# kelseyicotton/rawaudiovae_kelsey

Measured on NVIDIA B200. Metric: train frames/sec (fwd+bwd+Adam), higher is better.
Workload: dtype bf16

## Files before the change

rawaudiovae_kelsey_b200/csrc/capi.cu:

```cuda
#include <cmath>
#include <cstdlib>
#include <dlfcn.h>
#include <cstring>
#include <map>
#include <new>
#include <utility>
#include <vector>

#include "../../include/rvae_b200.h"
#include "common.h"

namespace rvae {
const char* last_error();
}

using namespace rvae;

struct NcclId {
  char internal[128];
};
struct NcclApi {
  void* handle;
  int (*GetUniqueId)(NcclId*);
  int (*CommInitRank)(void** comm, int nranks, NcclId id, int rank);
// ... 243 lines not shown
}
int rvae_dp_status(rvae_ctx* ctx, unsigned int* status) {
  RVAE_REQUIRE(ctx && status, RVAE_ERR_INVALID, "dp_status: null argument");
  *status = 0;
  if (!ctx->p2p_ready) return RVAE_OK;
  RVAE_CUDA(cudaMemcpy(status, ctx->p2p.status, sizeof(unsigned int), cudaMemcpyDeviceToHost));
  return RVAE_OK;
}
int rvae_ctx_num_sms(const rvae_ctx* ctx) { return ctx ? ctx->c.num_sms : 0; }
uint64_t rvae_ctx_launch_count(const rvae_ctx* ctx) { return ctx ? ctx->c.launches : 0; }

#define CTX_OR_FAIL(ctx) RVAE_REQUIRE((ctx) != nullptr, RVAE_ERR_INVALID, "null rvae_ctx")

int rvae_debug_set_aux_trace(rvae_ctx* ctx, void* buf, int launches) {
  CTX_OR_FAIL(ctx);
  ctx->c.aux_trace = reinterpret_cast<unsigned long long*>(buf);
  ctx->c.aux_cap = buf ? launches : 0;
  ctx->c.aux_seq = 0;
  return RVAE_OK;
}

int rvae_debug_set_trace(rvae_ctx* ctx, void* buf, int launches) {
  CTX_OR_FAIL(ctx);
  RVAE_REQUIRE(launches >= 1, RVAE_ERR_INVALID, "debug_set_trace: launches=%d", launches);
  ctx->c.trace_launches = launches;
  ctx->c.trace_seq = 0;
  static_assert(RVAE_TRACE_WORDS_PER_CTA == kTraceCtaWords && RVAE_TRACE_HEADER_WORDS == kTraceHeader &&
                    RVAE_TRACE_TILES == kTraceTiles && RVAE_TRACE_EVENTS == kTraceEvents,
                "trace layout");
  ctx->c.trace = reinterpret_cast<unsigned long long*>(buf);
  return RVAE_OK;
}

int rvae_frame_gather(rvae_ctx* ctx, const void* audio, int audio_is_i16, int64_t n_samples,
                      const int64_t* frame_idx, int64_t first_frame, int64_t n_frames, int hop, int S, void* out_hi,
                      void* out_lo, float* out_f32, void* stream) {
  CTX_OR_FAIL(ctx);
  return launch_frame_gather(&ctx->c, audio, audio_is_i16, n_samples, frame_idx, first_frame, n_frames, hop, S, S,
                             BF(out_hi), BF(out_lo), out_f32, S_(stream));
}
int rvae_overlap_add(rvae_ctx* ctx, const float* frames, int64_t n_frames, int S, int hop, float* out, int64_t t_begin,
                     int64_t n_out, void* stream) {
  CTX_OR_FAIL(ctx);
  return launch_overlap_add(&ctx->c, frames, n_frames, S, hop, out, t_begin, n_out, S_(stream));
}
int rvae_randn(rvae_ctx* ctx, float* out, int64_t n, uint64_t seed, uint64_t offset, int64_t elem_base,
               void* stream) {
  CTX_OR_FAIL(ctx);
  RVAE_REQUIRE(elem_base >= 0, RVAE_ERR_INVALID, "randn: elem_base %lld", (long long)elem_base);
  if (elem_base % 4 != 0) return launch_randn_rows(&ctx->c, out, 1, n, n, seed, offset, nullptr, elem_base, S_(stream));
  return launch_randn(&ctx->c, out, n, seed, offset, nullptr, elem_base, S_(stream));
}
int rvae_lerp_reparameterize(rvae_ctx* ctx, const float* mu_a, const float* logvar_a, const float* mu_b,
                             const float* logvar_b, const void* alpha, int alpha_is_f64, const float* eps,
                             int64_t rows, int L, float* z, float* mu_out, float* logvar_out, void* stream) {
  CTX_OR_FAIL(ctx);
  return launch_lerp_reparam(&ctx->c, mu_a, logvar_a, mu_b, logvar_b, alpha, alpha_is_f64, eps, rows, L, L, z, nullptr,
                             nullptr, mu_out, logvar_out, S_(stream));
}
int rvae_split_bf16(rvae_ctx* ctx, const float* src, int64_t n, void* hi, void* lo, void* stream) {
  CTX_OR_FAIL(ctx);
  return launch_split_bf16(&ctx->c, src, n, BF(hi), BF(lo), S_(stream));
}
int rvae_reparameterize(rvae_ctx* ctx, const float* mu, const float* logvar, const float* eps, int64_t n, float* z,
                        void* stream) {
  CTX_OR_FAIL(ctx);
  return launch_reparam(&ctx->c, mu, logvar, eps, n, z, S_(stream));
}
int rvae_loss_fwd(rvae_ctx* ctx, const float* xhat, const float* x, const float* mu, const float* logvar, int64_t B,
                  int S, int L, float beta, double* acc, float* loss_out, void* stream) {
  CTX_OR_FAIL(ctx);
  return launch_loss_fwd(&ctx->c, xhat, x, mu, logvar, B, S, L, beta, acc, loss_out, S_(stream));
}
int rvae_frame_loss(rvae_ctx* ctx, const float* xhat, int ld_xhat, const float* mu, const float* logvar, int ld_lat,
                    int64_t rows, int S, int L, const void* audio, int audio_is_i16, int64_t n_samples,
                    int64_t first_frame, int hop, float* rec_out, float* kl_out, void* stream) {
  RVAE_REQUIRE(xhat && mu && logvar && audio && rec_out && kl_out, RVAE_ERR_INVALID, "frame_loss: null buffer");
  RVAE_REQUIRE(rows > 0 && S > 0 && L > 0, RVAE_ERR_INVALID, "frame_loss: rows %lld, S %d, L %d (need > 0)",
               (long long)rows, S, L);
  RVAE_REQUIRE(ld_xhat >= S && ld_lat >= L, RVAE_ERR_INVALID, "frame_loss: row pitch ld_xhat %d < S %d or ld_lat %d < L %d",
               ld_xhat, S, ld_lat, L);
  RVAE_REQUIRE(hop > 0 && n_samples >= 0 && first_frame >= 0, RVAE_ERR_INVALID,
               "frame_loss: hop %d, n_samples %lld, first_frame %lld (need hop > 0, n_samples >= 0, first_frame >= 0)",
               hop, (long long)n_samples, (long long)first_frame);
  CTX_OR_FAIL(ctx);
  return launch_frame_loss(&ctx->c, xhat, ld_xhat, mu, logvar, ld_lat, rows, S, L, audio, audio_is_i16, n_samples,
                           first_frame, hop, rec_out, kl_out, S_(stream));
}
int rvae_loss_bwd(rvae_ctx* ctx, const float* xhat, const float* x, const float* mu, const float* logvar, int64_t B,
                  int S, int L, float beta, const float* grad_out, float* g_xhat, float* g_mu, float* g_logvar,
                  void* stream) {
  CTX_OR_FAIL(ctx);
  return launch_loss_bwd(&ctx->c, xhat, x, mu, logvar, B, S, L, beta, grad_out, g_xhat, g_mu, g_logvar, S_(stream));
}
int rvae_tanh_bwd(rvae_ctx* ctx, const float* g_xhat, const float* xhat, int64_t n, void* da_hi, void* da_lo,
                  void* stream) {
  CTX_OR_FAIL(ctx);
  return launch_tanh_bwd(&ctx->c, g_xhat, xhat, n, BF(da_hi), BF(da_lo), S_(stream));
}
int rvae_colsum(rvae_ctx* ctx, const void* hi, const void* lo, int64_t M, int N, int ld, float* out, int accumulate,
                void* stream) {
  CTX_OR_FAIL(ctx);
  return launch_colsum(&ctx->c, BF(hi), BF(lo), M, N, ld, out, accumulate, S_(stream));
}
int rvae_step_inc(rvae_ctx* ctx, float* step, void* stream) {
  CTX_OR_FAIL(ctx);
  return launch_step_inc(&ctx->c, step, S_(stream));
}
int rvae_adam_step(rvae_ctx* ctx, float* p, const float* g, float* m, float* v, int64_t n, double lr, double beta1,
                   double beta2, double eps, double weight_decay, float grad_scale, const float* step, void* shadow_hi,
                   void* shadow_lo, void* stream) {
  CTX_OR_FAIL(ctx);
  return launch_adam(&ctx->c, p, const_cast<float*>(g), m, v, n, lr, beta1, beta2, eps, weight_decay, grad_scale, step,
                     BF(shadow_hi), BF(shadow_lo), 0, S_(stream));
}
size_t rvae_param_histogram_bytes(int n_segs, int n_edges) { return param_histogram_bytes(n_segs, n_edges); }
int rvae_param_histogram(rvae_ctx* ctx, const float* params, const int64_t* seg_offsets_host,
                         const int64_t* seg_lengths_host, int n_segs, const double* edges_host, int n_edges,
                         void* record, void* stream) {
  CTX_OR_FAIL(ctx);
  return launch_param_histogram(&ctx->c, params, seg_offsets_host, seg_lengths_host, n_segs, edges_host, n_edges,
                                record, S_(stream));
}
int rvae_param_histogram_rows(rvae_ctx* ctx, const float* params, const int64_t* seg_offsets_host,
                              const int64_t* seg_rows_host, const int64_t* seg_cols_host, const int64_t* seg_pitch_host,
                              int n_segs, const double* edges_host, int n_edges, void* record, void* stream) {
  CTX_OR_FAIL(ctx);
  return launch_param_histogram_rows(&ctx->c, params, seg_offsets_host, seg_rows_host, seg_cols_host, seg_pitch_host,
                                     n_segs, edges_host, n_edges, record, S_(stream));
}

static GemmDesc desc_base(int epi, int M, int N, int K) {
  GemmDesc d;
  memset(&d, 0, sizeof(d));
  d.epi = epi; d.M = M; d.N = N; d.K = K;
  return d;
}
static Operand op(const void* hi, const void* lo, int major, int ld) {
  Operand o;
  o.hi = BF(hi); o.lo = BF(lo); o.major = major; o.ld = ld; o.cols = 0;
  return o;
}

int rvae_linear_act_fwd(rvae_ctx* ctx, const void* x_hi, const void* x_lo, const void* w_hi, const void* w_lo,
                        const float* bias, int M, int N, int K, int act, void* y_hi, void* y_lo, float* y_f32,
                        void* stream) {
  CTX_OR_FAIL(ctx);
  RVAE_REQUIRE(y_hi || y_f32, RVAE_ERR_INVALID, "linear_act_fwd: no output buffer");
  GemmDesc d = desc_base(EPI_LINEAR, M, N, K);
  d.A = op(x_hi, x_lo, MAJOR_K, K);
  d.B = op(w_hi, w_lo, MAJOR_K, K);
  d.args.bias = bias; d.args.act = act; d.args.ldo = N;
  d.args.out_hi = BF(y_hi); d.args.out_lo = BF(y_lo); d.args.out_f32 = y_f32;
  return gemm_launch(&ctx->c, d, S_(stream));
}

int rvae_encode_head_fwd(rvae_ctx* ctx, const void* h_hi, const void* h_lo, const void* w2_hi, const void* w2_lo,
                         const float* b2, int M, int L, int K, const float* eps, float* mu, float* logvar, void* z_hi,
                         void* z_lo, double* kl_acc, void* stream) {
  CTX_OR_FAIL(ctx);
  RVAE_REQUIRE(b2 && mu && logvar, RVAE_ERR_INVALID, "encode_head_fwd: null buffer");
  GemmDesc d = desc_base(EPI_HEAD, M, 2 * L, K);
  d.head_L = L;
  d.A = op(h_hi, h_lo, MAJOR_K, K);
  d.B = op(w2_hi, w2_lo, MAJOR_K, K);
  d.args.bias = b2; d.args.in0 = eps; d.args.out_f32 = mu; d.args.out_f32_b = logvar;
  d.args.out_hi = BF(z_hi); d.args.out_lo = BF(z_lo);
  d.args.loss_acc = kl_acc; d.args.L = L; d.args.ldo = L;
  return gemm_launch(&ctx->c, d, S_(stream));
}

int rvae_out_tanh_mse_fwd(rvae_ctx* ctx, const void* h_hi, const void* h_lo, const void* w4_hi, const void* w4_lo,
                          const float* b4, int M, int S, int K, const void* x_hi, const void* x_lo, int tanh_approx,
                          float* xhat, void* da_hi, void* da_lo, float grad_scale, double* mse_acc, float* bias_grad,
                          void* stream) {
  CTX_OR_FAIL(ctx);
  RVAE_REQUIRE(b4 && x_hi, RVAE_ERR_INVALID, "out_tanh_mse_fwd: null buffer");
  GemmDesc d = desc_base(EPI_OUT, M, S, K);
  d.A = op(h_hi, h_lo, MAJOR_K, K);
  d.B = op(w4_hi, w4_lo, MAJOR_K, K);
  d.args.bias = b4; d.args.in0 = x_hi; d.args.in1 = x_lo; d.args.out_f32 = xhat;
  d.args.out_hi = BF(da_hi); d.args.out_lo = BF(da_lo);
  d.args.act = tanh_approx ? ACT_TANH_APPROX : ACT_TANH;
  d.args.c0 = grad_scale; d.args.loss_acc = mse_acc; d.args.ldo = S; d.args.colsum = bias_grad;
  return gemm_launch(&ctx->c, d, S_(stream));
}

int rvae_dgrad_relu(rvae_ctx* ctx, const void* dy_hi, const void* dy_lo, const void* w_hi, const void* w_lo, int M,
                    int N, int Kd, const void* mask, void* dx_hi, void* dx_lo, float* bias_grad, void* stream) {
  CTX_OR_FAIL(ctx);
  RVAE_REQUIRE(dx_hi, RVAE_ERR_INVALID, "dgrad_relu: null output");
  GemmDesc d = desc_base(EPI_DRELU, M, N, Kd);
  d.A = op(dy_hi, dy_lo, MAJOR_K, Kd);
  d.B = op(w_hi, w_lo, MAJOR_MN, N);
  d.args.in0 = mask; d.args.out_hi = BF(dx_hi); d.args.out_lo = BF(dx_lo); d.args.ldo = N;
  d.args.colsum = bias_grad;
  return gemm_launch(&ctx->c, d, S_(stream));
}

int rvae_dgrad_latent(rvae_ctx* ctx, const void* da3_hi, const void* da3_lo, const void* w3_hi, const void* w3_lo,
                      int M, int L, int H, const float* eps, const float* logvar, const float* mu,
                      const float* g_mu_ext, const float* g_logvar_ext, float kl_grad_scale, float* dz_scratch,
                      void* dml_hi, void* dml_lo, float* bias_grad, void* stream) {
  CTX_OR_FAIL(ctx);
  RVAE_REQUIRE(eps && logvar && dz_scratch && dml_hi, RVAE_ERR_INVALID, "dgrad_latent: null buffer");
  RVAE_CUDA(cudaMemsetAsync(dz_scratch, 0, sizeof(float) * (size_t)M * L, S_(stream)));
  GemmDesc d = desc_base(EPI_REDUCE, M, L, H);
  d.A = op(da3_hi, da3_lo, MAJOR_K, H);
  d.B = op(w3_hi, w3_lo, MAJOR_MN, L);
  d.args.out_f32 = dz_scratch; d.args.ldo = L; d.args.accumulate = 1;
  RVAE_CHECK(gemm_launch(&ctx->c, d, S_(stream)));
  return launch_latent_bwd(&ctx->c, dz_scratch, eps, logvar, mu, g_mu_ext, g_logvar_ext, kl_grad_value(kl_grad_scale), M, L,
                           BF(dml_hi), BF(dml_lo), bias_grad, 0, nullptr, S_(stream));
}

int rvae_wgrad(rvae_ctx* ctx, const void* dy_hi, const void* dy_lo, const void* x_hi, const void* x_lo, int B, int M,
               int N, float* dW, int accumulate, int k_splits, void* stream) {
  CTX_OR_FAIL(ctx);
  RVAE_REQUIRE(dW, RVAE_ERR_INVALID, "wgrad: null output");
  RVAE_REQUIRE(M % 64 == 0, RVAE_ERR_UNSUPPORTED, "wgrad: M=%d must be a multiple of 64", M);
  GemmDesc d = desc_base(EPI_REDUCE, M, N, B);
  d.A = op(dy_hi, dy_lo, MAJOR_MN, M);
  d.B = op(x_hi, x_lo, MAJOR_MN, N);
  d.args.out_f32 = dW; d.args.ldo = N; d.args.accumulate = accumulate;
  d.k_splits = accumulate ? k_splits : 1;
  return gemm_launch(&ctx->c, d, S_(stream));
}

int rvae_param_layout(int S, int H, int L, rvae_layout* out) {
  RVAE_REQUIRE(out, RVAE_ERR_INVALID, "param_layout: null out");
  RVAE_REQUIRE(S > 0 && H > 0 && L > 0 && S % 64 == 0 && H % 64 == 0 && L % 64 == 0, RVAE_ERR_UNSUPPORTED,
               "segment_length=%d, n_units=%d, latent_dim=%d must be positive multiples of 64", S, H, L);
  int64_t o = 0;
  out->w1 = o; o += (int64_t)H * S;
  out->w2 = o; o += (int64_t)2 * L * H;
  out->w3 = o; o += (int64_t)H * L;
  out->w4 = o; o += (int64_t)S * H;
  out->b1 = o; o += H;
  out->b2 = o; o += 2 * L;
  out->b3 = o; o += H;
  out->b4 = o; o += S;
  out->total = o;
  return RVAE_OK;
}

int rvae_param_layout_padded(int S, int H, int L, rvae_layout* out, int* Sp, int* Hp, int* Lp) {
  RVAE_REQUIRE(out && Sp && Hp && Lp, RVAE_ERR_INVALID, "param_layout_padded: null out");
  RVAE_REQUIRE(S > 0 && H > 0 && L > 0 && S <= (1 << 24) && H <= (1 << 24) && L <= (1 << 24), RVAE_ERR_UNSUPPORTED,
               "segment_length=%d, n_units=%d, latent_dim=%d must be in 1..%d", S, H, L, 1 << 24);
  const int sp = (S + 63) / 64 * 64, hp = (H + 63) / 64 * 64, lp = (L + 63) / 64 * 64;
  RVAE_CHECK(rvae_param_layout(sp, hp, lp, out));
  *Sp = sp; *Hp = hp; *Lp = lp;
  return RVAE_OK;
}

}

namespace {

struct Planes {
  __nv_bfloat16* hi = nullptr;
  __nv_bfloat16* lo = nullptr;
};

constexpr int kNormGroups = 4;
constexpr int kNormMaxBlocks = 1024;

enum GemmId { G_F1, G_F2, G_F3, G_F4_OUT, G_F4_LIN, G_B4W, G_B4D, G_B3W, G_B3D, G_B2W, G_B2D, G_B1W, G_COUNT };
enum AuxSlot { T_LOAD = G_COUNT, T_EPS, T_FINALIZE, T_COLSUM, T_ADAM, T_TANHBWD, T_LATENT, T_COUNT };

constexpr int G_B3D_LAT = G_COUNT;
constexpr int kGemmSlots = G_COUNT + 1;

struct GemmSet {
  PreparedGemm g[kGemmSlots];
  bool ready[kGemmSlots];
  PreparedChain dual[3];
  int dual_state[3];
  PreparedChain dual_lat;
  int dual_lat_state;
  PreparedChain tri;
  int tri_state;
  PreparedChain fwd;
  int fwd_state;
};

}

struct rvae_plan {
  rvae_ctx* ctx;
  int S, H, L, max_batch, precision;
  int s_true, h_true, l_true;
  rvae_layout lay;
  rvae_plan_buffers bufs;
  bool bound;
  size_t ws_bytes;
  Planes x, h1, z, h3, da4, da3, dml, da1;
  float *mu, *lv, *eps, *dz, *xhat;
  float *ext_gx, *ext_gmu, *ext_glv, *ext_lv;
  Planes x_alt;
  float* eps_alt;
  int cur;
  int x_pitch, x_pitch_alt;
  int* sched_dev;
  int sched_batch;
  unsigned int* dep_flags;
  bool fuse_forward;
  bool fuse_latent;
  int dual_pairs;
  unsigned int* ticket;
  bool ticket_zeroed;
  bool norm_ticket_zeroed;
  const double* clip_max;
  float* clip_norm_out;
  int clip_ring;
  double* norm_parts;
  float* clip_coef;
  struct Prefetch {
    bool registered;
    int ready_batch;
    const void* audio; int audio_is_i16; int64_t n_samples; const int64_t* frame_idx; int64_t first_frame;
    int count, hop; uint64_t seed, offset; int add_step;
    bool span;
    int64_t noise_row0;
  } pf;
  double* loss_acc;
  float *out_mu, *out_lv, *out_xhat;
  int batch;
  int64_t global_batch;
  int64_t noise_row0;
  bool dp_enabled;
  float kl_c0;
  double kl_bl;
  const rvae_hparams* hp_dev;
  int hp_early;
  bool dz_zeroed;
  bool grads_zeroed[5];
  bool streams_ready;
  cudaEvent_t ev_fork;
  bool two_streams;
  bool have_eps;
  cudaEvent_t ev_eps;
  bool eps_pending;
  cudaStream_t adam_stream;
  cudaEvent_t ev_adam_fork, ev_adam_join;
  cudaStream_t hp;
  cudaEvent_t ev_hp_fork, ev_hp_join;
  cudaStream_t hp2;
  cudaEvent_t ev_s1_fork, ev_s1_join;
  bool split_stage1;
  int s1_wgrad_ctas, s1_order;
  bool merge_b3w;
  bool allow_defer;
  bool b3w_deferred;
  int adam_bg_blocks;
  cudaStream_t comm_stream;
  cudaStream_t comm_stream2;
  cudaEvent_t ev_comm_fork, ev_comm_done[5];
  LossFinalize fin;
  bool fin_pending;
  std::map<int64_t, GemmSet> sets;
  bool timing;
  std::vector<std::pair<cudaEvent_t, cudaEvent_t>> ev_pool;
  std::vector<std::pair<int, int>> ev_used;
  double t_ms[T_COUNT];
  int64_t t_n[T_COUNT];
  double t_flops[T_COUNT];
};

namespace {

size_t align_up(size_t v, size_t a) { return (v + a - 1) / a * a; }

size_t carve(rvae_plan* p, uint8_t* base) {
  const size_t B = p->max_batch, S = p->S, H = p->H, L = p->L;
  const bool lo = p->precision == RVAE_PRECISION_FP32;
  size_t off = 0;
  auto take = [&](size_t bytes) -> uint8_t* {
    uint8_t* r = base ? base + off : nullptr;
    off += align_up(bytes, 256);
    return r;
  };
  auto planes = [&](Planes& pl, size_t elems) {
    pl.hi = reinterpret_cast<__nv_bfloat16*>(take(elems * 2));
    pl.lo = lo ? reinterpret_cast<__nv_bfloat16*>(take(elems * 2)) : nullptr;
  };
  planes(p->x, B * S);
  planes(p->x_alt, B * S);
  planes(p->h1, B * H);
  planes(p->z, B * L);
  planes(p->h3, B * H);
  planes(p->da4, B * S);
  planes(p->da3, B * H);
  planes(p->dml, B * 2 * L);
  planes(p->da1, B * H);
  p->mu = reinterpret_cast<float*>(take(B * L * 4));
  p->lv = reinterpret_cast<float*>(take(B * L * 4));
  p->eps = reinterpret_cast<float*>(take(B * L * 4));
  p->eps_alt = reinterpret_cast<float*>(take(B * L * 4));
  p->ticket = reinterpret_cast<unsigned int*>(take(256));
  p->sched_dev = reinterpret_cast<int*>(take(sizeof(int) * 2 * 6 * 128 * kSchedMax));
  p->dep_flags = reinterpret_cast<unsigned int*>(take(sizeof(unsigned int) * 3 * 256));
  p->norm_parts = reinterpret_cast<double*>(take(sizeof(double) * kNormGroups * kNormMaxBlocks));
  p->clip_coef = reinterpret_cast<float*>(take(sizeof(float)));
  p->dz = reinterpret_cast<float*>(take(B * L * 4));
  p->xhat = reinterpret_cast<float*>(take(B * S * 4));
  p->loss_acc = reinterpret_cast<double*>(take(2 * sizeof(double)));
  p->ext_gx = p->ext_gmu = p->ext_glv = p->ext_lv = nullptr;
  if (p->S != (size_t)p->s_true) p->ext_gx = reinterpret_cast<float*>(take(B * S * 4));
  if (p->L != (size_t)p->l_true) {
    p->ext_gmu = reinterpret_cast<float*>(take(B * L * 4));
    p->ext_glv = reinterpret_cast<float*>(take(B * L * 4));
    p->ext_lv = reinterpret_cast<float*>(take(B * L * 4));
  }
  return off;
}

Operand opnd(const Planes& pl, int major, int ld) {
  Operand o;
  o.hi = pl.hi; o.lo = pl.lo; o.major = major; o.ld = ld; o.cols = 0;
  return o;
}
Operand wopnd(const rvae_plan* p, int64_t off, int major, int ld) {
  Operand o;
  o.hi = BF(p->bufs.shadow_hi) + off;
  o.lo = p->bufs.shadow_lo ? BF(p->bufs.shadow_lo) + off : nullptr;
  o.major = major; o.ld = ld; o.cols = 0;
  return o;
}

int prepare(rvae_plan* p, GemmSet& gs, int id) {
  if (gs.ready[id]) return RVAE_OK;
  const int B = p->batch, S = p->S, H = p->H, L = p->L;
  const int ldx = p->x_pitch > 0 ? p->x_pitch : S;
  const rvae_layout& ly = p->lay;
  float* params = p->bufs.params;
  float* grads = p->bufs.grads;
  GemmDesc d;
  memset(&d, 0, sizeof(d));
  const bool bf16_mode = p->precision == RVAE_PRECISION_BF16;
  switch (id) {
    case G_F1:
      d.epi = EPI_LINEAR; d.M = B; d.N = H; d.K = S;
      d.A = opnd(p->x, MAJOR_K, ldx); d.B = wopnd(p, ly.w1, MAJOR_K, S);
      d.A.cols = p->s_true;
      d.args.bias = params + ly.b1; d.args.act = ACT_RELU; d.args.ldo = H;
      d.args.out_hi = p->h1.hi; d.args.out_lo = p->h1.lo;
      break;
    case G_F2:
      d.epi = EPI_HEAD; d.M = B; d.N = 2 * L; d.K = H; d.head_L = L;
      d.A = opnd(p->h1, MAJOR_K, H); d.B = wopnd(p, ly.w2, MAJOR_K, H);
      d.args.bias = params + ly.b2; d.args.in0 = p->eps; d.args.out_f32 = p->mu; d.args.out_f32_b = p->lv;
      d.args.out_hi = p->z.hi; d.args.out_lo = p->z.lo;
      d.args.loss_acc = p->loss_acc + 1; d.args.L = L; d.args.ldo = L;
      break;
    case G_F3:
      d.epi = EPI_LINEAR; d.M = B; d.N = H; d.K = L;
      d.A = opnd(p->z, MAJOR_K, L); d.B = wopnd(p, ly.w3, MAJOR_K, L);
      d.args.bias = params + ly.b3; d.args.act = ACT_RELU; d.args.ldo = H;
      d.args.out_hi = p->h3.hi; d.args.out_lo = p->h3.lo;
      break;
    case G_F4_OUT:
      d.epi = EPI_OUT; d.M = B; d.N = S; d.K = H;
      d.A = opnd(p->h3, MAJOR_K, H); d.B = wopnd(p, ly.w4, MAJOR_K, H);
      d.args.bias = params + ly.b4; d.args.in0 = p->x.hi; d.args.in1 = p->x.lo; d.args.out_f32 = p->xhat;
      d.args.out_hi = p->da4.hi; d.args.out_lo = p->da4.lo;
      d.args.act = bf16_mode ? ACT_TANH_APPROX : ACT_TANH;
      d.args.loss_acc = p->loss_acc; d.args.ldo = S; d.args.ldi = ldx; d.side_cols = p->s_true;
      d.args.colsum = grads ? grads + ly.b4 : nullptr;
      break;
    case G_F4_LIN:
      d.epi = EPI_LINEAR; d.M = B; d.N = S; d.K = H;
      d.A = opnd(p->h3, MAJOR_K, H); d.B = wopnd(p, ly.w4, MAJOR_K, H);
      d.args.bias = params + ly.b4; d.args.act = bf16_mode ? ACT_TANH_APPROX : ACT_TANH; d.args.ldo = S;
      d.args.out_f32 = p->xhat;
      break;
    case G_B4W:
      d.epi = EPI_REDUCE; d.M = S; d.N = H; d.K = B;
      d.A = opnd(p->da4, MAJOR_MN, S); d.B = opnd(p->h3, MAJOR_MN, H);
      d.args.out_f32 = grads + ly.w4; d.args.ldo = H; d.args.accumulate = 1;
      break;
    case G_B4D:
      d.epi = EPI_DRELU; d.M = B; d.N = H; d.K = S;
      d.A = opnd(p->da4, MAJOR_K, S); d.B = wopnd(p, ly.w4, MAJOR_MN, H);
      d.args.in0 = p->h3.hi; d.args.out_hi = p->da3.hi; d.args.out_lo = p->da3.lo; d.args.ldo = H;
      d.args.colsum = grads + ly.b3;
      break;
    case G_B3W:
      d.epi = EPI_REDUCE; d.M = H; d.N = L; d.K = B;
      d.A = opnd(p->da3, MAJOR_MN, H); d.B = opnd(p->z, MAJOR_MN, L);
      d.args.out_f32 = grads + ly.w3; d.args.ldo = L; d.args.accumulate = 1;
      break;
    case G_B3D:
      d.epi = EPI_REDUCE; d.M = B; d.N = L; d.K = H;
      d.A = opnd(p->da3, MAJOR_K, H); d.B = wopnd(p, ly.w3, MAJOR_MN, L);
      d.args.out_f32 = p->dz; d.args.ldo = L; d.args.accumulate = 1;
      break;
    case G_B3D_LAT:
      d.epi = EPI_DLATENT; d.M = B; d.N = L; d.K = H;
      d.A = opnd(p->da3, MAJOR_K, H); d.B = wopnd(p, ly.w3, MAJOR_MN, L);
      d.args.in0 = p->eps; d.args.in1 = p->lv; d.args.in2 = p->mu;
      d.args.out_hi = p->dml.hi; d.args.ldo = 2 * L; d.args.L = L;
      d.args.colsum = grads + ly.b2;
      break;
    case G_B2W:
      d.epi = EPI_REDUCE; d.M = 2 * L; d.N = H; d.K = B;
      d.A = opnd(p->dml, MAJOR_MN, 2 * L); d.B = opnd(p->h1, MAJOR_MN, H);
      d.args.out_f32 = grads + ly.w2; d.args.ldo = H; d.args.accumulate = 1;
      break;
    case G_B2D:
      d.epi = EPI_DRELU; d.M = B; d.N = H; d.K = 2 * L;
      d.A = opnd(p->dml, MAJOR_K, 2 * L); d.B = wopnd(p, ly.w2, MAJOR_MN, H);
      d.args.in0 = p->h1.hi; d.args.out_hi = p->da1.hi; d.args.out_lo = p->da1.lo; d.args.ldo = H;
      d.args.colsum = grads + ly.b1;
      break;
    case G_B1W:
      d.epi = EPI_REDUCE; d.M = H; d.N = S; d.K = B;
      d.A = opnd(p->da1, MAJOR_MN, H); d.B = opnd(p->x, MAJOR_MN, ldx); d.B.cols = p->s_true;
      d.args.out_f32 = grads + ly.w1; d.args.ldo = S; d.args.accumulate = 1;
      break;
    default:
      return set_error(RVAE_ERR_INVALID, "plan: bad gemm id %d", id);
  }
  RVAE_CHECK(gemm_prepare(&p->ctx->c, d, &gs.g[id]));
  gs.ready[id] = true;
  return RVAE_OK;
}

int get_set(rvae_plan* p, GemmSet** out) {
  const int64_t key = ((int64_t)p->batch * 2 + p->cur) * 65536 + p->x_pitch;
  auto it = p->sets.find(key);
  if (it == p->sets.end()) {
    GemmSet gs;
    memset(&gs, 0, sizeof(gs));
    it = p->sets.emplace(key, gs).first;
  }
  *out = &it->second;
  return RVAE_OK;
}

int run_untimed(rvae_plan* p, GemmSet* gs, int id, cudaStream_t st, const EpiArgs* override_args) {
  if (override_args) {
    PreparedGemm g = gs->g[id];
    EpiArgs a = *override_args;
    if (a.L == 0) a.L = g.params.epi.L;
    RVAE_CHECK(gemm_bind_outputs(&g, a, false));
    return gemm_run(&p->ctx->c, g, st);
  }
  return gemm_run(&p->ctx->c, gs->g[id], st);
}

struct TimedScope {
  rvae_plan* p; int slot; cudaStream_t st; int idx;
  TimedScope(rvae_plan* p_, int slot_, cudaStream_t st_) : p(p_), slot(slot_), st(st_), idx(-1) {
    if (!p->timing) return;
    const size_t k = p->ev_used.size();
    if (k >= p->ev_pool.size()) {
      cudaEvent_t a, b;
      if (cudaEventCreate(&a) != cudaSuccess || cudaEventCreate(&b) != cudaSuccess) return;
      p->ev_pool.emplace_back(a, b);
    }
    idx = (int)k;
    cudaEventRecord(p->ev_pool[k].first, st);
  }
  ~TimedScope() {
    if (idx < 0) return;
    cudaEventRecord(p->ev_pool[idx].second, st);
    p->ev_used.emplace_back(slot, idx);
  }
};

int run(rvae_plan* p, int id, cudaStream_t st, const EpiArgs* override_args = nullptr) {
  GemmSet* gs;
  RVAE_CHECK(get_set(p, &gs));
  RVAE_CHECK(prepare(p, *gs, id));
  if (!p->timing) return run_untimed(p, gs, id, st, override_args);
  const size_t slot = p->ev_used.size();
  if (slot >= p->ev_pool.size()) {
    cudaEvent_t a, b;
    RVAE_CUDA(cudaEventCreate(&a));
    RVAE_CUDA(cudaEventCreate(&b));
    p->ev_pool.emplace_back(a, b);
  }
  RVAE_CUDA(cudaEventRecord(p->ev_pool[slot].first, st));
  RVAE_CHECK(run_untimed(p, gs, id, st, override_args));
  RVAE_CUDA(cudaEventRecord(p->ev_pool[slot].second, st));
  const int tid = id == G_B3D_LAT ? G_B3D : id;
  p->ev_used.emplace_back(tid, (int)slot);
  const GemmParams& gp = gs->g[id].params;
  p->t_flops[tid] = 2.0 * gp.M * gp.N * gp.K;
  return RVAE_OK;
}

int pad_rows(float* dst, const float* src, int rows, int cols, int ld, cudaStream_t st) {
  RVAE_CUDA(cudaMemcpy2DAsync(dst, sizeof(float) * ld, src, sizeof(float) * cols, sizeof(float) * cols, rows,
                              cudaMemcpyDeviceToDevice, st));
  RVAE_CUDA(cudaMemset2DAsync(dst + cols, sizeof(float) * ld, 0, sizeof(float) * (ld - cols), rows, st));
  return RVAE_OK;
}
int strip_rows(float* dst, const float* src, int rows, int cols, int ld, cudaStream_t st) {
  RVAE_CUDA(cudaMemcpy2DAsync(dst, sizeof(float) * cols, src, sizeof(float) * ld, sizeof(float) * cols, rows,
                              cudaMemcpyDeviceToDevice, st));
  return RVAE_OK;
}
int copy_latents_out(rvae_plan* p, cudaStream_t st) {
  if (p->out_mu) RVAE_CHECK(strip_rows(p->out_mu, p->mu, p->batch, p->l_true, p->L, st));
  if (p->out_lv) RVAE_CHECK(strip_rows(p->out_lv, p->lv, p->batch, p->l_true, p->L, st));
  return RVAE_OK;
}

int draw_eps(rvae_plan* p, float* out, int rows, uint64_t seed, uint64_t offset, const float* offset_src, int64_t row0,
             cudaStream_t st) {
  if (p->l_true == p->L)
    return launch_randn(&p->ctx->c, out, (int64_t)rows * p->L, seed, offset, offset_src, row0 * p->L, st);
  return launch_randn_rows(&p->ctx->c, out, rows, p->l_true, p->L, seed, offset, offset_src, row0 * p->l_true, st);
}

int decode_tail(rvae_plan* p, float* xhat_out, cudaStream_t st) {
  RVAE_CHECK(run(p, G_F3, st));
  GemmSet* gs;
  RVAE_CHECK(get_set(p, &gs));
  RVAE_CHECK(prepare(p, *gs, G_F4_LIN));
  EpiArgs a = gs->g[G_F4_LIN].params.epi;
  const bool rec_direct = p->S == p->s_true;
  a.out_f32 = rec_direct ? xhat_out : p->xhat;
  RVAE_CHECK(run(p, G_F4_LIN, st, &a));
  return rec_direct ? RVAE_OK : strip_rows(xhat_out, p->xhat, p->batch, p->s_true, p->S, st);
}

int check_ready(const rvae_plan* p, bool need_batch) {
  RVAE_REQUIRE(p != nullptr, RVAE_ERR_INVALID, "null rvae_plan");
  RVAE_REQUIRE(p->bound, RVAE_ERR_STATE, "plan: rvae_plan_bind has not been called");
  if (need_batch) RVAE_REQUIRE(p->batch > 0, RVAE_ERR_STATE, "plan: no batch loaded");
  return RVAE_OK;
}

int ensure_bias_zeroed(rvae_plan* p, cudaStream_t st) {
  if (p->grads_zeroed[4]) return RVAE_OK;
  const rvae_layout& ly = p->lay;
  RVAE_CUDA(cudaMemsetAsync(p->bufs.grads + ly.b1, 0, sizeof(float) * (size_t)(ly.total - ly.b1), st));
  p->grads_zeroed[4] = true;
  return RVAE_OK;
}

int ensure_side_stream(rvae_plan* p) {
  if (p->streams_ready) return RVAE_OK;
  int least = 0, greatest = 0;
  RVAE_CUDA(cudaDeviceGetStreamPriorityRange(&least, &greatest));
  RVAE_CUDA(cudaStreamCreateWithPriority(&p->hp, cudaStreamNonBlocking, greatest));
  RVAE_CUDA(cudaStreamCreateWithPriority(&p->adam_stream, cudaStreamNonBlocking, least));
  RVAE_CUDA(cudaStreamCreateWithPriority(&p->hp2, cudaStreamNonBlocking, greatest));
  RVAE_CUDA(cudaEventCreateWithFlags(&p->ev_s1_fork, cudaEventDisableTiming));
  RVAE_CUDA(cudaEventCreateWithFlags(&p->ev_s1_join, cudaEventDisableTiming));
  RVAE_CUDA(cudaEventCreateWithFlags(&p->ev_hp_fork, cudaEventDisableTiming));
  RVAE_CUDA(cudaEventCreateWithFlags(&p->ev_hp_join, cudaEventDisableTiming));
  RVAE_CUDA(cudaStreamCreateWithPriority(&p->comm_stream, cudaStreamNonBlocking, greatest));
  RVAE_CUDA(cudaStreamCreateWithPriority(&p->comm_stream2, cudaStreamNonBlocking, greatest));
  RVAE_CUDA(cudaEventCreateWithFlags(&p->ev_comm_fork, cudaEventDisableTiming));
  for (int i = 0; i < 5; ++i) RVAE_CUDA(cudaEventCreateWithFlags(&p->ev_comm_done[i], cudaEventDisableTiming));
  RVAE_CUDA(cudaEventCreateWithFlags(&p->ev_fork, cudaEventDisableTiming));
  RVAE_CUDA(cudaEventCreateWithFlags(&p->ev_eps, cudaEventDisableTiming));
  RVAE_CUDA(cudaEventCreateWithFlags(&p->ev_adam_fork, cudaEventDisableTiming));
  RVAE_CUDA(cudaEventCreateWithFlags(&p->ev_adam_join, cudaEventDisableTiming));
  p->streams_ready = true;
  return RVAE_OK;
}

int adam_buckets(rvae_plan* p, unsigned mask, const HpArg& hp, float grad_scale, int zero_grads, int step_bias,
                 bool advance_step, cudaStream_t st, const float* coef = nullptr) {
  const rvae_layout& ly = p->lay;
  const rvae_plan_buffers& b = p->bufs;
  const int order[5] = {3, 2, 1, 0, 4};
  const int64_t begin[6] = {ly.w1, ly.w2, ly.w3, ly.w4, ly.b1, ly.total};
  int64_t seg_off[5], seg_n[5];
  int nseg = 0;
  for (int i = 0; i < 5; ++i) {
    if (!(mask & (1u << order[i]))) continue;
    if (nseg > 0 && seg_off[nseg - 1] + seg_n[nseg - 1] == begin[i]) seg_n[nseg - 1] += begin[i + 1] - begin[i];
    else { seg_off[nseg] = begin[i]; seg_n[nseg] = begin[i + 1] - begin[i]; ++nseg; }
  }
  if (advance_step && !p->ticket_zeroed) {
    RVAE_CUDA(cudaMemsetAsync(p->ticket, 0, sizeof(unsigned int), st));
    p->ticket_zeroed = true;
  }
  for (int i = 0; i < nseg; i += 2) {
    const int64_t o = seg_off[i];
    const bool pair = i + 1 < nseg;
    const bool last = i + 2 >= nseg;
    RVAE_CHECK(launch_adam2(&p->ctx->c, b.params + o, b.grads + o, b.exp_avg + o, b.exp_avg_sq + o, seg_n[i],
                            pair ? seg_off[i + 1] - o : 0, pair ? seg_n[i + 1] : 0, hp, grad_scale, coef, b.step, step_bias, (advance_step && last) ? p->ticket : nullptr,
                            BF(b.shadow_hi) + o, b.shadow_lo ? BF(b.shadow_lo) + o : nullptr, zero_grads, st));
  }
  for (int s = 0; s < 5; ++s)
    if (mask & (1u << s)) p->grads_zeroed[s] = zero_grads != 0;
  return RVAE_OK;
}

int grad_norm_group(rvae_plan* p, int k, NormFinalize* fin, cudaStream_t st) {
  const rvae_layout& ly = p->lay;
  const int64_t off[kNormGroups][2] = {{ly.w4, 0}, {ly.w3, 0}, {ly.w2, ly.b1}, {ly.w1, 0}};
  const int64_t len[kNormGroups][2] = {{ly.b1 - ly.w4, 0}, {ly.w4 - ly.w3, 0}, {ly.w3 - ly.w2, ly.total - ly.b1},
                                       {ly.w2 - ly.w1, 0}};
  int base[kNormGroups + 1] = {0};
  for (int j = 0; j < kNormGroups; ++j) base[j + 1] = base[j] + grad_norm_blocks(&p->ctx->c, len[j][0] + len[j][1]);
  RVAE_REQUIRE(base[kNormGroups] <= kNormGroups * kNormMaxBlocks, RVAE_ERR_UNSUPPORTED, "grad_norm: %d blocks",
               base[kNormGroups]);
  if (fin != nullptr) {
    if (!p->norm_ticket_zeroed) {
      RVAE_CUDA(cudaMemsetAsync(p->ticket + 1, 0, sizeof(unsigned int), st));
      p->norm_ticket_zeroed = true;
    }
    fin->parts = p->norm_parts;
    fin->n_parts = base[kNormGroups];
    fin->ticket = p->ticket + 1;
  }
  NormFinalize none;
  memset(&none, 0, sizeof(none));
  return launch_grad_norm(&p->ctx->c, p->bufs.grads + off[k][0], len[k][0], off[k][1] - off[k][0], len[k][1],
                          p->norm_parts + base[k], fin ? *fin : none, st);
}

NormFinalize clip_finalize(rvae_plan* p) {
  NormFinalize f;
  memset(&f, 0, sizeof(f));
  f.step = p->bufs.step;
  f.norm_out = p->clip_norm_out;
  f.ring_size = p->clip_ring;
  f.max_norm = p->clip_max;
  f.coef_out = p->clip_coef;
  return f;
}

struct LatentExt {
  const float* g_mu;
  const float* g_lv;
  const float* lv;
};

KlGrad plan_kl(const rvae_plan* p) { return KlGrad{p->hp_dev, p->bufs.step, p->kl_bl, p->kl_c0, p->hp_early}; }

bool sched_usable(const rvae_plan* p) { return p->sched_batch == 0 || p->sched_batch == p->batch; }

bool latent_fused(const rvae_plan* p) {
  return p->fuse_latent && p->precision == RVAE_PRECISION_BF16 && p->batch > kBlockM;
}

int backward_stage_latent_fused(rvae_plan* p, cudaStream_t st) {
  GemmSet* gs;
  RVAE_CHECK(get_set(p, &gs));
  if (p->fin_pending) {
    RVAE_CHECK(launch_loss_finalize_prepared(&p->ctx->c, p->fin, st));
    p->fin_pending = false;
  }
  if (p->dual_pairs > 0 && !p->timing && sched_usable(p)) {
    int pairs = p->dual_pairs > 64 ? 64 : p->dual_pairs;
    if (const char* e = getenv("RVAE_DUAL_PAIRS_S1")) {
      const int v = atoi(e);
      if (v >= 1 && 2 * v <= p->ctx->c.num_sms_total) pairs = v;
    }
    if (gs->dual_lat_state == 0) {
      RVAE_CHECK(prepare(p, *gs, G_B3D_LAT));
      RVAE_CHECK(prepare(p, *gs, G_B3W));
      int* sched = p->sched_dev + ((size_t)p->cur * 6 + 4) * 128 * kSchedMax;
      const PreparedGemm* both[2] = {&gs->g[G_B3D_LAT], &gs->g[G_B3W]};
      const int rc = gemm_prepare_chain(&p->ctx->c, both, 2, pairs, sched, &gs->dual_lat);
      gs->dual_lat_state = rc == RVAE_OK ? 1 : -1;
      if (rc != RVAE_OK && rc != RVAE_ERR_UNSUPPORTED) return rc;
      if (rc == RVAE_OK) p->sched_batch = p->batch;
    }
    if (gs->dual_lat_state == 1) {
      PreparedChain d = gs->dual_lat;
      d.params.p[0].epi.c0 = p->kl_c0;
      return gemm_run_chain(&p->ctx->c, d, st);
    }
  }
  RVAE_CHECK(prepare(p, *gs, G_B3D_LAT));
  EpiArgs a = gs->g[G_B3D_LAT].params.epi;
  a.c0 = p->kl_c0;
  RVAE_CHECK(run(p, G_B3D_LAT, st, &a));
  return run(p, G_B3W, st);
}

int backward_stage(rvae_plan* p, int stage, const LatentExt* ext, cudaStream_t st) {
  const int S = p->S, H = p->H, L = p->L;
  const rvae_layout& ly = p->lay;
  float* grads = p->bufs.grads;
  static const int kWgrad[4] = {G_B4W, G_B3W, G_B2W, G_B1W};
  static const int kDgrad[4] = {G_B4D, G_B3D, G_B2D, -1};
  RVAE_REQUIRE(stage >= 0 && stage < 4, RVAE_ERR_INVALID, "plan_backward: stage %d not in -1..3", stage);
  float* wptr[4] = {grads + ly.w4, grads + ly.w3, grads + ly.w2, grads + ly.w1};
  const size_t wcount[4] = {(size_t)S * H, (size_t)H * L, (size_t)2 * L * H, (size_t)H * S};
  if (!p->grads_zeroed[stage]) RVAE_CUDA(cudaMemsetAsync(wptr[stage], 0, sizeof(float) * wcount[stage], st));
  p->grads_zeroed[stage] = false;
  if (stage == 1 && ext == nullptr && latent_fused(p)) return backward_stage_latent_fused(p, st);
  if (stage == 1 && !p->dz_zeroed)
    RVAE_CUDA(cudaMemsetAsync(p->dz, 0, sizeof(float) * (size_t)p->max_batch * L, st));
  auto stage_pairs = [&](int st_idx) {
    int pairs = (p->dp_enabled && p->ctx->dp_world > 1 && p->dual_pairs > 64) ? 64 : p->dual_pairs;
    const char* names[3] = {"RVAE_DUAL_PAIRS_S0", "RVAE_DUAL_PAIRS_S1", "RVAE_DUAL_PAIRS_S2"};
    if (const char* e = getenv(names[st_idx])) {
      const int v = atoi(e);
      if (v >= 1 && 2 * v <= p->ctx->c.num_sms_total) pairs = v;
    }
    return pairs;
  };
  if (stage == 1 && p->allow_defer && p->merge_b3w && p->dual_pairs > 0 && sched_usable(p) && p->batch > kBlockM) {
    GemmSet* gs;
    RVAE_CHECK(get_set(p, &gs));
    if (gs->tri_state == 0) {
      RVAE_CHECK(prepare(p, *gs, G_B2D));
      RVAE_CHECK(prepare(p, *gs, G_B2W));
      RVAE_CHECK(prepare(p, *gs, G_B3W));
      int* sched = p->sched_dev + ((size_t)p->cur * 6 + 5) * 128 * kSchedMax;
      const PreparedGemm* three[3] = {&gs->g[G_B2D], &gs->g[G_B2W], &gs->g[G_B3W]};
      const int rc = gemm_prepare_chain(&p->ctx->c, three, 3, stage_pairs(2), sched, &gs->tri);
      gs->tri_state = rc == RVAE_OK ? 1 : -1;
      if (rc != RVAE_OK && rc != RVAE_ERR_UNSUPPORTED) return rc;
      if (rc == RVAE_OK) p->sched_batch = p->batch;
    }
    if (gs->tri_state == 1) {
      RVAE_CHECK(run(p, G_B3D, st));
      {
        TimedScope ts(p, T_LATENT, st);
        RVAE_CHECK(launch_latent_bwd(&p->ctx->c, p->dz, p->eps, ext ? ext->lv : p->lv, p->mu, ext ? ext->g_mu : nullptr,
                                     ext ? ext->g_lv : nullptr, plan_kl(p), p->batch, L, p->dml.hi, p->dml.lo, grads + ly.b2,
                                     1, p->fin_pending ? &p->fin : nullptr, st));
      }
      p->fin_pending = false;
      p->dz_zeroed = true;
      p->b3w_deferred = true;
      return RVAE_OK;
    }
  }
  if (stage == 2 && p->b3w_deferred) {
    GemmSet* gs;
    RVAE_CHECK(get_set(p, &gs));
    RVAE_REQUIRE(gs->tri_state == 1, RVAE_ERR_STATE, "plan_backward: stage 1 deferred the fc3 weight gradient but the "
                 "three-problem launch is not prepared (batch or input set changed between the stages)");
    p->b3w_deferred = false;
    TimedScope ts(p, G_B2D, st);
    if (p->timing) {
      double f = 0.0;
      for (int id : {G_B2D, G_B2W, G_B3W}) { const GemmParams& q = gs->g[id].params; f += 2.0 * q.M * q.N * q.K; }
      p->t_flops[G_B2D] = f;
    }
    return gemm_run_chain(&p->ctx->c, gs->tri, st);
  }
  if (stage == 1 && p->split_stage1 && p->timing && p->batch > kBlockM) {
    GemmSet* gs;
    RVAE_CHECK(get_set(p, &gs));
    RVAE_CHECK(run(p, G_B3D, st));
    RVAE_CHECK(prepare(p, *gs, G_B3W));
    {
      TimedScope ts(p, G_B3W, st);
      PreparedGemm w = gs->g[G_B3W];
      p->t_flops[G_B3W] = 2.0 * w.params.M * w.params.N * w.params.K;
      if (w.grid > p->s1_wgrad_ctas) w.grid = p->s1_wgrad_ctas;
      RVAE_CHECK(gemm_run(&p->ctx->c, w, st));
    }
    TimedScope ts(p, T_LATENT, st);
    RVAE_CHECK(launch_latent_bwd(&p->ctx->c, p->dz, p->eps, ext ? ext->lv : p->lv, p->mu, ext ? ext->g_mu : nullptr,
                                 ext ? ext->g_lv : nullptr, plan_kl(p), p->batch, L, p->dml.hi, p->dml.lo, grads + ly.b2, 1,
                                 p->fin_pending ? &p->fin : nullptr, st));
    p->fin_pending = false;
    p->dz_zeroed = true;
    return RVAE_OK;
  }
  if (stage == 1 && p->split_stage1 && p->two_streams && !p->timing && p->batch > kBlockM) {
    RVAE_CHECK(ensure_side_stream(p));
    GemmSet* gs;
    RVAE_CHECK(get_set(p, &gs));
    RVAE_CHECK(prepare(p, *gs, G_B3D));
    RVAE_CHECK(prepare(p, *gs, G_B3W));
    RVAE_CHECK(gemm_run(&p->ctx->c, gs->g[G_B3D], st));
    RVAE_CUDA(cudaEventRecord(p->ev_s1_fork, st));
    RVAE_CUDA(cudaStreamWaitEvent(p->hp2, p->ev_s1_fork, 0));
    cudaStream_t s_w = p->s1_order == 0 ? st : p->hp2;
    cudaStream_t s_l = p->s1_order == 0 ? p->hp2 : st;
    auto run_wgrad = [&]() -> int {
      PreparedGemm w = gs->g[G_B3W];
      const int cap = (p->dp_enabled && p->ctx->dp_world > 1 && p->s1_wgrad_ctas > 64) ? 64 : p->s1_wgrad_ctas;
      if (w.grid > cap) w.grid = cap;
      return gemm_run(&p->ctx->c, w, s_w);
    };
    auto run_latent = [&]() -> int {
      return launch_latent_bwd(&p->ctx->c, p->dz, p->eps, ext ? ext->lv : p->lv, p->mu, ext ? ext->g_mu : nullptr,
                               ext ? ext->g_lv : nullptr, plan_kl(p), p->batch, L, p->dml.hi, p->dml.lo, grads + ly.b2, 1,
                               p->fin_pending ? &p->fin : nullptr, s_l);
    };
    if (p->s1_order == 0) { RVAE_CHECK(run_wgrad()); RVAE_CHECK(run_latent()); }
    else { RVAE_CHECK(run_latent()); RVAE_CHECK(run_wgrad()); }
    RVAE_CUDA(cudaEventRecord(p->ev_s1_join, p->hp2));
    p->fin_pending = false;
    p->dz_zeroed = true;
    RVAE_CUDA(cudaStreamWaitEvent(st, p->ev_s1_join, 0));
    return RVAE_OK;
  }
  bool fused = false;
  if (kDgrad[stage] >= 0 && p->dual_pairs > 0 && sched_usable(p)) {
    int pairs = stage_pairs(stage);
    if (stage == 1 && pairs > 64 && !getenv("RVAE_DUAL_PAIRS_S1")) pairs = 64;
    GemmSet* gs;
    RVAE_CHECK(get_set(p, &gs));
    if (gs->dual_state[stage] == 0) {
      RVAE_CHECK(prepare(p, *gs, kDgrad[stage]));
      RVAE_CHECK(prepare(p, *gs, kWgrad[stage]));
      int* sched = p->sched_dev + ((size_t)p->cur * 6 + stage) * 128 * kSchedMax;
      const PreparedGemm* both[2] = {&gs->g[kDgrad[stage]], &gs->g[kWgrad[stage]]};
      const int rc = gemm_prepare_chain(&p->ctx->c, both, 2, pairs, sched, &gs->dual[stage]);
      gs->dual_state[stage] = rc == RVAE_OK ? 1 : -1;
      if (rc != RVAE_OK && rc != RVAE_ERR_UNSUPPORTED) return rc;
      if (rc == RVAE_OK) p->sched_batch = p->batch;
    }
    if (gs->dual_state[stage] == 1) {
      TimedScope ts(p, kDgrad[stage], st);
      if (p->timing) {
        const GemmParams& a = gs->g[kDgrad[stage]].params;
        const GemmParams& b = gs->g[kWgrad[stage]].params;
        p->t_flops[kDgrad[stage]] = 2.0 * a.M * a.N * a.K + 2.0 * b.M * b.N * b.K;
      }
      RVAE_CHECK(gemm_run_chain(&p->ctx->c, gs->dual[stage], st));
      fused = true;
    }
  }
  if (!fused && kDgrad[stage] >= 0) RVAE_CHECK(run(p, kDgrad[stage], st));
  if (stage == 1) {
    TimedScope ts(p, T_LATENT, st);
    RVAE_CHECK(launch_latent_bwd(&p->ctx->c, p->dz, p->eps, ext ? ext->lv : p->lv, p->mu, ext ? ext->g_mu : nullptr,
                                 ext ? ext->g_lv : nullptr, plan_kl(p), p->batch, L, p->dml.hi, p->dml.lo, grads + ly.b2, 1,
                                 p->fin_pending ? &p->fin : nullptr, st));
    p->fin_pending = false;
    p->dz_zeroed = true;
  }
  return fused ? RVAE_OK : run(p, kWgrad[stage], st);
}

}

extern "C" {

int rvae_plan_create(rvae_ctx* ctx, int S, int H, int L, int max_batch, int precision, rvae_plan** out) {
  CTX_OR_FAIL(ctx);
  RVAE_REQUIRE(out, RVAE_ERR_INVALID, "plan_create: null out");
  RVAE_REQUIRE(max_batch > 0, RVAE_ERR_INVALID, "plan_create: max_batch=%d", max_batch);
  RVAE_REQUIRE(precision == RVAE_PRECISION_BF16 || precision == RVAE_PRECISION_FP32, RVAE_ERR_INVALID,
               "plan_create: precision %d", precision);
  rvae_layout lay;
  int Sp, Hp, Lp;
  RVAE_CHECK(rvae_param_layout_padded(S, H, L, &lay, &Sp, &Hp, &Lp));
  rvae_plan* p = new (std::nothrow) rvae_plan();
  RVAE_REQUIRE(p, RVAE_ERR_INVALID, "plan_create: out of host memory");
  p->ctx = ctx; p->S = Sp; p->H = Hp; p->L = Lp; p->max_batch = max_batch; p->precision = precision;
  p->s_true = S; p->h_true = H; p->l_true = L;
  p->lay = lay; p->bound = false; p->batch = 0; p->have_eps = false; p->global_batch = 0; p->noise_row0 = 0;
  p->timing = false;
  p->kl_c0 = 0.f; p->kl_bl = 0.0; p->hp_dev = nullptr; p->hp_early = 0; p->dz_zeroed = false; p->dp_enabled = false;
  p->cur = 0; p->ticket_zeroed = false; p->ticket = nullptr; p->norm_ticket_zeroed = false;
  p->clip_max = nullptr; p->clip_norm_out = nullptr; p->clip_ring = 1;
  p->x_pitch = 0; p->x_pitch_alt = 0;
  p->fuse_latent = false;
  p->sched_batch = 0;
  memset(&p->pf, 0, sizeof(p->pf));
  for (int i = 0; i < 5; ++i) p->grads_zeroed[i] = false;
  p->streams_ready = false; p->ev_fork = nullptr;
  p->hp = nullptr; p->ev_hp_fork = nullptr; p->ev_hp_join = nullptr;
  p->comm_stream = nullptr; p->comm_stream2 = nullptr; p->ev_comm_fork = nullptr;
  for (int i = 0; i < 5; ++i) p->ev_comm_done[i] = nullptr;
  p->adam_stream = nullptr; p->ev_eps = nullptr; p->ev_adam_fork = nullptr; p->ev_adam_join = nullptr;
  p->eps_pending = false; p->fin_pending = false;
  p->two_streams = true;
  p->hp2 = nullptr; p->ev_s1_fork = nullptr; p->ev_s1_join = nullptr;
  p->split_stage1 = true;
  p->s1_wgrad_ctas = 96;
  p->s1_order = 0;
  p->merge_b3w = false; p->allow_defer = false; p->b3w_deferred = false;
#if RVAE_EXPERIMENTS
  if (const char* e = getenv("RVAE_MERGE_B3W")) p->merge_b3w = atoi(e) != 0;
#endif
  p->adam_bg_blocks = 0;
  if (const char* e = getenv("RVAE_ADAM_BG_BLOCKS")) p->adam_bg_blocks = atoi(e) > 0 ? atoi(e) : 0;
  if (const char* e = getenv("RVAE_S1_ORDER")) p->s1_order = atoi(e) != 0;
  if (const char* e = getenv("RVAE_SPLIT_STAGE1")) p->split_stage1 = atoi(e) != 0;
  if (const char* e = getenv("RVAE_S1_WGRAD_CTAS")) {
    const int v = atoi(e);
    if (v >= 2 && v <= ctx->c.num_sms_total) p->s1_wgrad_ctas = v & ~1;
  }
  p->fuse_forward = false;
#if RVAE_EXPERIMENTS
  if (const char* e = getenv("RVAE_FUSE_LATENT")) p->fuse_latent = atoi(e) != 0;
  if (const char* e = getenv("RVAE_FUSE_FORWARD")) p->fuse_forward = atoi(e) != 0;
#endif
  p->dual_pairs = ctx->c.num_sms / 2;
  if (const char* e = getenv("RVAE_DUAL_PAIRS")) {
    const int v = atoi(e);
    if (v >= 0 && 2 * v <= ctx->c.num_sms_total) p->dual_pairs = v;
  }
  if (const char* e = getenv("RVAE_TWO_STREAMS")) p->two_streams = atoi(e) != 0;
  for (int i = 0; i < T_COUNT; ++i) { p->t_ms[i] = 0; p->t_n[i] = 0; p->t_flops[i] = 0; }
  p->out_mu = p->out_lv = p->out_xhat = nullptr;
  memset(&p->bufs, 0, sizeof(p->bufs));
  p->ws_bytes = carve(p, nullptr);
  *out = p;
  return RVAE_OK;
}

void rvae_plan_destroy(rvae_plan* plan) {
  if (!plan) return;
  for (auto& e : plan->ev_pool) {
    cudaEventDestroy(e.first);
    cudaEventDestroy(e.second);
  }
  if (plan->streams_ready) {
    cudaStreamSynchronize(plan->adam_stream);
    cudaStreamSynchronize(plan->hp);
    cudaStreamSynchronize(plan->comm_stream);
    cudaStreamSynchronize(plan->comm_stream2);
    cudaStreamDestroy(plan->comm_stream2);
    cudaEventDestroy(plan->ev_comm_fork);
    for (int i = 0; i < 5; ++i) cudaEventDestroy(plan->ev_comm_done[i]);
    cudaStreamDestroy(plan->comm_stream);
    cudaEventDestroy(plan->ev_hp_fork);
    cudaEventDestroy(plan->ev_hp_join);
    cudaStreamDestroy(plan->hp);
    cudaStreamSynchronize(plan->hp2);
    cudaStreamDestroy(plan->hp2);
    cudaEventDestroy(plan->ev_s1_fork);
    cudaEventDestroy(plan->ev_s1_join);
    cudaEventDestroy(plan->ev_fork);
    cudaEventDestroy(plan->ev_eps);
    cudaEventDestroy(plan->ev_adam_fork);
    cudaEventDestroy(plan->ev_adam_join);
    cudaStreamDestroy(plan->adam_stream);
  }
  delete plan;
}

int rvae_plan_enable_timing(rvae_plan* plan, int enable) {
  RVAE_REQUIRE(plan, RVAE_ERR_INVALID, "null rvae_plan");
  plan->timing = enable != 0;
  return RVAE_OK;
}

int rvae_plan_read_timing(rvae_plan* plan, float* ms, int64_t* launches, double* flops_per_launch) {
  RVAE_REQUIRE(plan && ms && launches && flops_per_launch, RVAE_ERR_INVALID, "plan_read_timing: null argument");
  static_assert(G_COUNT == RVAE_NUM_GEMM_SLOTS && T_COUNT == RVAE_NUM_TIMING_SLOTS, "slot count");
  for (auto& u : plan->ev_used) {
    auto& e = plan->ev_pool[u.second];
    RVAE_CUDA(cudaEventSynchronize(e.second));
    float t = 0.f;
    RVAE_CUDA(cudaEventElapsedTime(&t, e.first, e.second));
    plan->t_ms[u.first] += t;
    plan->t_n[u.first] += 1;
  }
  plan->ev_used.clear();
  for (int i = 0; i < T_COUNT; ++i) {
    ms[i] = (float)plan->t_ms[i];
    launches[i] = plan->t_n[i];
    flops_per_launch[i] = plan->t_flops[i];
    plan->t_ms[i] = 0; plan->t_n[i] = 0;
  }
  return RVAE_OK;
}

size_t rvae_plan_workspace_bytes(const rvae_plan* plan) { return plan ? plan->ws_bytes : 0; }

int rvae_plan_bind(rvae_plan* plan, const rvae_plan_buffers* b) {
  RVAE_REQUIRE(plan && b, RVAE_ERR_INVALID, "plan_bind: null argument");
  RVAE_REQUIRE(b->params && b->shadow_hi && b->workspace, RVAE_ERR_INVALID,
               "plan_bind: params, shadow_hi and workspace are required");
  RVAE_REQUIRE(plan->precision == RVAE_PRECISION_BF16 || b->shadow_lo, RVAE_ERR_INVALID,
               "plan_bind: fp32 mode needs shadow_lo");
  RVAE_REQUIRE((reinterpret_cast<uintptr_t>(b->workspace) & 255) == 0, RVAE_ERR_INVALID,
               "plan_bind: workspace must be 256-byte aligned");
  plan->bufs = *b;
  if (plan->precision == RVAE_PRECISION_BF16) plan->bufs.shadow_lo = nullptr;
  carve(plan, reinterpret_cast<uint8_t*>(b->workspace));
  plan->sets.clear();
  plan->sched_batch = 0;
  for (int i = 0; i < 5; ++i) plan->grads_zeroed[i] = false;
  plan->dz_zeroed = false;
  plan->cur = 0; plan->ticket_zeroed = false; plan->norm_ticket_zeroed = false;
  memset(&plan->pf, 0, sizeof(plan->pf));
  if (plan->two_streams) RVAE_CHECK(ensure_side_stream(plan));
  plan->bound = true;
  plan->batch = 0;
  return RVAE_OK;
}

int rvae_plan_sync_shadow(rvae_plan* plan, void* stream) {
  RVAE_CHECK(check_ready(plan, false));
  return launch_split_bf16(&plan->ctx->c, plan->bufs.params, plan->lay.total, BF(plan->bufs.shadow_hi),
                           BF(plan->bufs.shadow_lo), S_(stream));
}

int rvae_plan_load_frames(rvae_plan* plan, const void* audio, int audio_is_i16, int64_t n_samples,
                          const int64_t* frame_idx, int64_t first_frame, int count, int hop, int row_offset,
                          void* stream) {
  RVAE_CHECK(check_ready(plan, false));
  RVAE_REQUIRE(count > 0 && row_offset >= 0 && row_offset + count <= plan->max_batch, RVAE_ERR_INVALID,
               "plan_load_frames: rows %d..%d outside 0..%d", row_offset, row_offset + count, plan->max_batch);
  RVAE_REQUIRE(row_offset == 0 || row_offset == plan->batch, RVAE_ERR_STATE,
               "plan_load_frames: row_offset %d does not continue the loaded batch (%d rows)", row_offset,
               plan->batch);
  RVAE_REQUIRE(row_offset == 0 || plan->x_pitch == 0, RVAE_ERR_STATE,
               "plan_load_frames: cannot append rows to a batch that was loaded as a sample span");
  plan->batch = row_offset + count;
  plan->x_pitch = 0;
  plan->have_eps = false;
  const size_t off = (size_t)row_offset * plan->S;
  TimedScope ts(plan, T_LOAD, S_(stream));
  return launch_frame_gather(&plan->ctx->c, audio, audio_is_i16, n_samples, frame_idx, first_frame, count, hop,
                             plan->s_true, plan->S, plan->x.hi + off, plan->x.lo ? plan->x.lo + off : nullptr, nullptr,
                             S_(stream));
}

int rvae_plan_load_batch(rvae_plan* plan, const float* x, int batch, void* stream) {
  RVAE_CHECK(check_ready(plan, false));
  RVAE_REQUIRE(x, RVAE_ERR_INVALID, "plan_load_batch: null x");
  RVAE_REQUIRE(batch > 0 && batch <= plan->max_batch, RVAE_ERR_INVALID, "plan_load_batch: batch %d not in 1..%d",
               batch, plan->max_batch);
  plan->batch = batch;
  plan->x_pitch = 0;
  plan->have_eps = false;
  TimedScope ts(plan, T_LOAD, S_(stream));
  if (plan->s_true != plan->S)
    return launch_split_bf16_rows(&plan->ctx->c, x, batch, plan->s_true, plan->s_true, plan->S, plan->x.hi, plan->x.lo,
                                  S_(stream));
  return launch_split_bf16(&plan->ctx->c, x, (int64_t)batch * plan->S, plan->x.hi, plan->x.lo, S_(stream));
}

static int span_eligible(const rvae_plan* p, int count, int hop) {
  const int S = p->s_true;
  return hop > 0 && hop % 8 == 0 && hop <= S && S % 8 == 0 && count > 0 && count <= p->max_batch &&
         (S == p->S || p->precision == RVAE_PRECISION_BF16);
}
static int convert_span(rvae_plan* p, const void* audio, int audio_is_i16, int64_t n_samples,
                        const int64_t* first_frame_dev, int64_t first_frame, int count, int hop, Planes& dst,
                        cudaStream_t st) {
  const int64_t span = (int64_t)(count - 1) * hop + p->s_true;
  RVAE_REQUIRE(span <= (int64_t)INT32_MAX, RVAE_ERR_UNSUPPORTED, "plan span: %lld samples", (long long)span);
  return launch_frame_gather(&p->ctx->c, audio, audio_is_i16, n_samples, first_frame_dev, first_frame, 1, hop,
                             (int)span, (int)span, dst.hi, dst.lo, nullptr, st);
}

int rvae_plan_span_supported(const rvae_plan* plan, int count, int hop) {
  return plan ? span_eligible(plan, count, hop) : 0;
}

int rvae_plan_load_span(rvae_plan* plan, const void* audio, int audio_is_i16, int64_t n_samples,
                        const int64_t* first_frame_dev, int64_t first_frame, int count, int hop, void* stream) {
  RVAE_CHECK(check_ready(plan, false));
  RVAE_REQUIRE(audio && span_eligible(plan, count, hop), RVAE_ERR_UNSUPPORTED,
               "plan_load_span: count %d (max %d), hop %d (needs hop %% 8 == 0 and hop <= S = %d; S %% 8 == 0; bf16 "
               "mode if S %% 64 != 0)", count, plan->max_batch, hop, plan->s_true);
  RVAE_REQUIRE(first_frame_dev || first_frame >= 0, RVAE_ERR_INVALID, "plan_load_span: first_frame %lld",
               (long long)first_frame);
  plan->batch = count;
  plan->x_pitch = hop;
  plan->have_eps = false;
  TimedScope ts(plan, T_LOAD, S_(stream));
  return convert_span(plan, audio, audio_is_i16, n_samples, first_frame_dev, first_frame, count, hop, plan->x,
                      S_(stream));
}

int rvae_plan_set_eps(rvae_plan* plan, const float* eps, void* stream) {
  RVAE_CHECK(check_ready(plan, true));
  RVAE_REQUIRE(eps, RVAE_ERR_INVALID, "plan_set_eps: null eps");
  if (plan->l_true != plan->L)
    RVAE_CHECK(pad_rows(plan->eps, eps, plan->batch, plan->l_true, plan->L, S_(stream)));
  else
    RVAE_CUDA(cudaMemcpyAsync(plan->eps, eps, sizeof(float) * (size_t)plan->batch * plan->L, cudaMemcpyDeviceToDevice,
                              S_(stream)));
  plan->have_eps = true;
  return RVAE_OK;
}

int rvae_plan_gen_eps(rvae_plan* plan, uint64_t seed, uint64_t offset, int add_step, void* stream) {
  RVAE_CHECK(check_ready(plan, true));
  RVAE_REQUIRE(!add_step || plan->bufs.step, RVAE_ERR_STATE, "plan_gen_eps(add_step): no step counter bound");
  plan->have_eps = true;
  cudaStream_t st = S_(stream);
  if (plan->two_streams && !plan->timing) {
    RVAE_CHECK(ensure_side_stream(plan));
    RVAE_CUDA(cudaEventRecord(plan->ev_fork, st));
    RVAE_CUDA(cudaStreamWaitEvent(plan->adam_stream, plan->ev_fork, 0));
    RVAE_CHECK(draw_eps(plan, plan->eps, plan->batch, seed, offset, add_step ? plan->bufs.step : nullptr,
                        plan->noise_row0, plan->adam_stream));
    RVAE_CUDA(cudaEventRecord(plan->ev_eps, plan->adam_stream));
    plan->eps_pending = true;
    return RVAE_OK;
  }
  TimedScope ts(plan, T_EPS, st);
  return draw_eps(plan, plan->eps, plan->batch, seed, offset, add_step ? plan->bufs.step : nullptr, plan->noise_row0,
                  st);
}

int rvae_plan_set_outputs(rvae_plan* plan, float* mu, float* logvar, float* xhat) {
  RVAE_REQUIRE(plan, RVAE_ERR_INVALID, "null rvae_plan");
  plan->out_mu = mu; plan->out_lv = logvar; plan->out_xhat = xhat;
  return RVAE_OK;
}

int rvae_plan_enable_dp(rvae_plan* plan, int on) {
  RVAE_REQUIRE(plan, RVAE_ERR_INVALID, "null rvae_plan");
  RVAE_REQUIRE(!on || plan->ctx->comm != nullptr || plan->ctx->p2p_ready, RVAE_ERR_STATE,
               "plan_enable_dp: call rvae_dp_init / rvae_dp_sym_open first");
  if (plan->dp_enabled != (on != 0) && !plan->sets.empty()) {
    RVAE_CUDA(cudaDeviceSynchronize());
    plan->sets.clear();
    plan->sched_batch = 0;
  }
  plan->dp_enabled = on != 0;
  return RVAE_OK;
}

int rvae_plan_set_noise_rows(rvae_plan* plan, int64_t first_global_row) {
  RVAE_REQUIRE(plan && first_global_row >= 0, RVAE_ERR_INVALID, "plan_set_noise_rows: bad argument");
  plan->noise_row0 = first_global_row;
  return RVAE_OK;
}

int rvae_plan_set_global_batch(rvae_plan* plan, int64_t global_batch) {
  RVAE_REQUIRE(plan && global_batch >= 0, RVAE_ERR_INVALID, "plan_set_global_batch: bad argument");
  plan->global_batch = global_batch;
  return RVAE_OK;
}

int rvae_plan_forward(rvae_plan* plan, float kl_beta, int fused_loss, int want_xhat, void* stream) {
  RVAE_CHECK(check_ready(plan, true));
  RVAE_REQUIRE(plan->have_eps, RVAE_ERR_STATE, "plan_forward: call rvae_plan_set_eps / rvae_plan_gen_eps first");
  cudaStream_t st = S_(stream);
  rvae_plan* p = plan;
  const double nb = p->global_batch > 0 ? (double)p->global_batch : (double)p->batch;
  const double BL = nb * p->l_true, BS = nb * p->s_true;
  const bool lat_direct = p->L == p->l_true, rec_direct = p->S == p->s_true;
  GemmSet* gs;
  RVAE_CHECK(get_set(p, &gs));

  const bool chain = fused_loss && !want_xhat && p->fuse_forward && p->dual_pairs > 0 && !p->timing && sched_usable(p) && !p->out_mu &&
                     !p->out_lv && !p->out_xhat && p->bufs.grads != nullptr;
  if (chain) {
    if (gs->fwd_state == 0) {
      static const int kLayers[4] = {G_F1, G_F2, G_F3, G_F4_OUT};
      const PreparedGemm* layers[4];
      for (int k = 0; k < 4; ++k) {
        RVAE_CHECK(prepare(p, *gs, kLayers[k]));
        layers[k] = &gs->g[kLayers[k]];
      }
      int* sched = p->sched_dev + ((size_t)p->cur * 6 + 3) * 128 * kSchedMax;
      int fpairs = p->dual_pairs;
      if (const char* e = getenv("RVAE_DUAL_PAIRS_F")) {
        const int v = atoi(e);
        if (v >= 1 && 2 * v <= p->ctx->c.num_sms_total) fpairs = v;
      }
      const int rc = gemm_prepare_chain(&p->ctx->c, layers, 4, fpairs, sched, &gs->fwd, p->dep_flags);
      gs->fwd_state = rc == RVAE_OK ? 1 : -1;
      if (rc != RVAE_OK && rc != RVAE_ERR_UNSUPPORTED) return rc;
      if (rc == RVAE_OK) p->sched_batch = p->batch;
    }
    if (gs->fwd_state == 1) {
      p->kl_c0 = (float)((double)kl_beta / BL);
      p->kl_bl = BL;
      RVAE_CHECK(ensure_bias_zeroed(p, st));
      p->grads_zeroed[4] = false;
      RVAE_CUDA(cudaMemsetAsync(p->dep_flags, 0, sizeof(unsigned int) * 3 * 256, st));
      if (p->eps_pending) {
        RVAE_CUDA(cudaStreamWaitEvent(st, p->ev_eps, 0));
        p->eps_pending = false;
      }
      PreparedChain d = gs->fwd;
      d.params.p[3].epi.c0 = (float)(2.0 / BS);
      d.params.p[3].epi.out_f32 = nullptr;
      return gemm_run_chain(&p->ctx->c, d, st);
    }
  }
  RVAE_CHECK(run(p, G_F1, st));
  if (p->eps_pending) {
    RVAE_CUDA(cudaStreamWaitEvent(st, p->ev_eps, 0));
    p->eps_pending = false;
  }
  {
    RVAE_CHECK(prepare(p, *gs, G_F2));
    EpiArgs a = gs->g[G_F2].params.epi;
    if (p->out_mu && lat_direct) a.out_f32 = p->out_mu;
    if (p->out_lv && lat_direct) a.out_f32_b = p->out_lv;
    if (fused_loss) { p->kl_c0 = (float)((double)kl_beta / BL); p->kl_bl = BL; }
    else a.loss_acc = nullptr;
    RVAE_CHECK(run(p, G_F2, st, &a));
    if (!lat_direct) RVAE_CHECK(copy_latents_out(p, st));
  }
  RVAE_CHECK(run(p, G_F3, st));
  if (fused_loss) {
    RVAE_REQUIRE(p->bufs.grads, RVAE_ERR_STATE, "plan_forward(fused_loss): no grads buffer bound");
    RVAE_REQUIRE(!p->out_mu && !p->out_lv, RVAE_ERR_STATE,
                 "plan_forward(fused_loss): mu / logvar must stay in the workspace (the fused backward reads them)");
    RVAE_CHECK(ensure_bias_zeroed(p, st));
    p->grads_zeroed[4] = false;
    RVAE_CHECK(prepare(p, *gs, G_F4_OUT));
    EpiArgs a = gs->g[G_F4_OUT].params.epi;
    a.c0 = (float)(2.0 / BS);
    a.out_f32 = want_xhat ? (p->out_xhat && rec_direct ? p->out_xhat : p->xhat) : nullptr;
    RVAE_CHECK(run(p, G_F4_OUT, st, &a));
    if (want_xhat && p->out_xhat && !rec_direct) RVAE_CHECK(strip_rows(p->out_xhat, p->xhat, p->batch, p->s_true, p->S, st));
  } else {
    RVAE_CHECK(prepare(p, *gs, G_F4_LIN));
    EpiArgs a = gs->g[G_F4_LIN].params.epi;
    a.out_f32 = p->out_xhat && rec_direct ? p->out_xhat : p->xhat;
    RVAE_CHECK(run(p, G_F4_LIN, st, &a));
    if (p->out_xhat && !rec_direct) RVAE_CHECK(strip_rows(p->out_xhat, p->xhat, p->batch, p->s_true, p->S, st));
  }
  return RVAE_OK;
}

int rvae_plan_backward(rvae_plan* plan, int stage, void* stream) {
  RVAE_CHECK(check_ready(plan, true));
  RVAE_REQUIRE(plan->bufs.grads, RVAE_ERR_STATE, "plan_backward: no grads buffer bound");
  if (stage == -1) {
    plan->allow_defer = true;
    int rc = RVAE_OK;
    for (int s = 0; s < 4 && rc == RVAE_OK; ++s) rc = backward_stage(plan, s, nullptr, S_(stream));
    plan->allow_defer = false;
    return rc;
  }
  return backward_stage(plan, stage, nullptr, S_(stream));
}

int rvae_plan_backward_external(rvae_plan* plan, const float* g_xhat, const float* xhat, const float* g_mu,
                                const float* g_logvar, const float* logvar, void* stream) {
  RVAE_CHECK(check_ready(plan, true));
  RVAE_REQUIRE(plan->bufs.grads, RVAE_ERR_STATE, "plan_backward_external: no grads buffer bound");
  RVAE_REQUIRE(g_xhat && xhat && g_mu && g_logvar && logvar, RVAE_ERR_INVALID,
               "plan_backward_external: null argument");
  rvae_plan* p = plan;
  cudaStream_t st = S_(stream);
  if (p->S != p->s_true) {
    RVAE_CHECK(pad_rows(p->ext_gx, g_xhat, p->batch, p->s_true, p->S, st));
    RVAE_CHECK(pad_rows(p->xhat, xhat, p->batch, p->s_true, p->S, st));
    g_xhat = p->ext_gx;
    xhat = p->xhat;
  }
  if (p->L != p->l_true) {
    RVAE_CHECK(pad_rows(p->ext_gmu, g_mu, p->batch, p->l_true, p->L, st));
    RVAE_CHECK(pad_rows(p->ext_glv, g_logvar, p->batch, p->l_true, p->L, st));
    RVAE_CHECK(pad_rows(p->ext_lv, logvar, p->batch, p->l_true, p->L, st));
    g_mu = p->ext_gmu;
    g_logvar = p->ext_glv;
    logvar = p->ext_lv;
  }
  RVAE_CHECK(ensure_bias_zeroed(p, st));
  p->grads_zeroed[4] = false;
  { TimedScope ts(p, T_TANHBWD, st); RVAE_CHECK(launch_tanh_bwd(&p->ctx->c, g_xhat, xhat, (int64_t)p->batch * p->S, p->da4.hi, p->da4.lo, st)); }
  { TimedScope ts(p, T_COLSUM, st);
    RVAE_CHECK(launch_colsum(&p->ctx->c, p->da4.hi, p->da4.lo, p->batch, p->S, p->S, p->bufs.grads + p->lay.b4, 1, st)); }
  const LatentExt ext = {g_mu, g_logvar, logvar};
  p->allow_defer = true;
  int rc = RVAE_OK;
  for (int s = 0; s < 4 && rc == RVAE_OK; ++s) rc = backward_stage(p, s, &ext, st);
  p->allow_defer = false;
  return rc;
}

int rvae_plan_finish_loss(rvae_plan* plan, float kl_beta, float* loss_out, int ring_size, void* stream) {
  RVAE_CHECK(check_ready(plan, true));
  RVAE_REQUIRE(ring_size >= 1, RVAE_ERR_INVALID, "plan_finish_loss: ring_size %d", ring_size);
  TimedScope ts(plan, T_FINALIZE, S_(stream));
  return launch_loss_finalize(&plan->ctx->c, plan->loss_acc, plan->batch, plan->s_true, plan->l_true, kl_beta, loss_out,
                              ring_size, plan->bufs.step, S_(stream));
}

int rvae_plan_finish_loss_deferred(rvae_plan* plan, float kl_beta, float* loss_out, int ring_size) {
  RVAE_CHECK(check_ready(plan, true));
  RVAE_REQUIRE(ring_size >= 1, RVAE_ERR_INVALID, "plan_finish_loss_deferred: ring_size %d", ring_size);
  plan->fin = make_loss_finalize(plan->loss_acc, plan->batch, plan->s_true, plan->l_true, kl_beta, loss_out, ring_size,
                                 plan->bufs.step);
  plan->fin_pending = true;
  return RVAE_OK;
}

int rvae_plan_prefetch_frames(rvae_plan* plan, const void* audio, int audio_is_i16, int64_t n_samples,
                              const int64_t* frame_idx, int64_t first_frame, int count, int hop, uint64_t seed,
                              uint64_t offset, int add_step) {
  RVAE_CHECK(check_ready(plan, false));
  RVAE_REQUIRE(audio && count > 0 && count <= plan->max_batch && hop > 0, RVAE_ERR_INVALID,
               "plan_prefetch_frames: bad arguments (count %d of max %d)", count, plan->max_batch);
  rvae_plan::Prefetch& f = plan->pf;
  f.audio = audio; f.audio_is_i16 = audio_is_i16; f.n_samples = n_samples; f.frame_idx = frame_idx;
  f.first_frame = first_frame; f.count = count; f.hop = hop; f.seed = seed; f.offset = offset; f.add_step = add_step;
  f.noise_row0 = plan->noise_row0;
  f.span = false;
  f.registered = true;
  return RVAE_OK;
}

int rvae_plan_prefetch_span(rvae_plan* plan, const void* audio, int audio_is_i16, int64_t n_samples,
                            const int64_t* first_frame_dev, int64_t first_frame, int count, int hop, uint64_t seed,
                            uint64_t offset, int add_step) {
  RVAE_CHECK(check_ready(plan, false));
  RVAE_REQUIRE(audio && span_eligible(plan, count, hop), RVAE_ERR_UNSUPPORTED,
               "plan_prefetch_span: count %d (max %d), hop %d (needs hop %% 8 == 0 and hop <= S = %d; S %% 8 == 0; "
               "bf16 mode if S %% 64 != 0)", count, plan->max_batch, hop, plan->s_true);
  RVAE_REQUIRE(first_frame_dev || first_frame >= 0, RVAE_ERR_INVALID, "plan_prefetch_span: first_frame %lld",
               (long long)first_frame);
  RVAE_CHECK(rvae_plan_prefetch_frames(plan, audio, audio_is_i16, n_samples, first_frame_dev, first_frame, count, hop,
                                       seed, offset, add_step));
  plan->pf.span = true;
  return RVAE_OK;
}

int rvae_plan_swap_prefetched(rvae_plan* plan) {
  RVAE_CHECK(check_ready(plan, false));
  RVAE_REQUIRE(plan->pf.ready_batch > 0, RVAE_ERR_STATE, "plan_swap_prefetched: no prefetched batch");
  std::swap(plan->x, plan->x_alt);
  std::swap(plan->x_pitch, plan->x_pitch_alt);
  std::swap(plan->eps, plan->eps_alt);
  plan->cur ^= 1;
  plan->batch = plan->pf.ready_batch;
  plan->pf.ready_batch = 0;
  plan->have_eps = true;
  plan->eps_pending = false;
  return RVAE_OK;
}

int rvae_plan_prefetched_batch(const rvae_plan* plan) { return plan ? plan->pf.ready_batch : 0; }

int rvae_plan_join_background(rvae_plan* plan, void* stream) {
  RVAE_CHECK(check_ready(plan, false));
  if (plan->eps_pending) {
    RVAE_CUDA(cudaStreamWaitEvent(S_(stream), plan->ev_eps, 0));
    plan->eps_pending = false;
  }
  return RVAE_OK;
}

int rvae_plan_note_prefetched(rvae_plan* plan, int count, int span_hop) {
  RVAE_CHECK(check_ready(plan, false));
  RVAE_REQUIRE(count > 0 && count <= plan->max_batch && span_hop >= 0, RVAE_ERR_INVALID,
               "plan_note_prefetched: count %d span_hop %d", count, span_hop);
  plan->pf.ready_batch = count;
  plan->x_pitch_alt = span_hop;
  return RVAE_OK;
}

int rvae_plan_adam(rvae_plan* plan, double lr, double beta1, double beta2, double eps, double weight_decay,
                   float grad_scale, int zero_grads, void* stream) {
  return rvae_plan_adam_buckets(plan, 0x1f, lr, beta1, beta2, eps, weight_decay, grad_scale, zero_grads, stream);
}

int rvae_plan_adam_buckets(rvae_plan* plan, unsigned bucket_mask, double lr, double beta1, double beta2, double eps,
                           double weight_decay, float grad_scale, int zero_grads, void* stream) {
  RVAE_CHECK(check_ready(plan, false));
  const rvae_plan_buffers& b = plan->bufs;
  RVAE_REQUIRE(b.grads && b.exp_avg && b.exp_avg_sq && b.step, RVAE_ERR_STATE,
               "plan_adam: grads / exp_avg / exp_avg_sq / step not bound");
  RVAE_REQUIRE(bucket_mask != 0 && bucket_mask <= 0x1f, RVAE_ERR_INVALID, "plan_adam_buckets: mask %#x", bucket_mask);
  TimedScope ts(plan, T_ADAM, S_(stream));
  return adam_buckets(plan, bucket_mask, hp_value(lr, beta1, beta2, eps, weight_decay), grad_scale, zero_grads, 0,
                      false, S_(stream));
}

static int train_step(rvae_plan* plan, float kl_beta, const HpArg& hp, int zero_grads, float* loss_out, int ring_size,
               void* stream) {
  RVAE_CHECK(check_ready(plan, true));
  const rvae_plan_buffers& b = plan->bufs;
  RVAE_REQUIRE(b.grads && b.exp_avg && b.exp_avg_sq && b.step, RVAE_ERR_STATE,
               "plan_train_step: grads / exp_avg / exp_avg_sq / step not bound");
  rvae_plan* p = plan;
  const bool fork = plan->two_streams && !plan->timing;
  const bool clip = plan->clip_max != nullptr;
  plan->hp_early = fork && plan->hp_dev != nullptr;
  if (!fork) {
    RVAE_CHECK(rvae_plan_forward(plan, kl_beta, 1, 0, stream));
    RVAE_CHECK(rvae_plan_finish_loss_deferred(plan, kl_beta, loss_out, ring_size));
    plan->fin.inc_step = 0;
    plan->fin.hp = hp.dev;
    RVAE_CHECK(rvae_plan_backward(plan, -1, stream));
    TimedScope ts(plan, T_ADAM, S_(stream));
    if (clip) {
      NormFinalize fin = clip_finalize(plan);
      for (int k = 0; k < kNormGroups; ++k)
        RVAE_CHECK(grad_norm_group(plan, k, k == kNormGroups - 1 ? &fin : nullptr, S_(stream)));
    }
    return adam_buckets(plan, 0x1f, hp, 1.0f, zero_grads, 1, true, S_(stream), clip ? plan->clip_coef : nullptr);
  }
  RVAE_CHECK(ensure_side_stream(plan));
  cudaStream_t st = plan->hp, bg = plan->adam_stream;
  RVAE_CUDA(cudaEventRecord(plan->ev_hp_fork, S_(stream)));
  RVAE_CUDA(cudaStreamWaitEvent(st, plan->ev_hp_fork, 0));
  auto enqueue_prefetch = [&]() -> int {
    if (!p->pf.registered) return RVAE_OK;
    const rvae_plan::Prefetch& f = p->pf;
    RVAE_CUDA(cudaStreamWaitEvent(bg, plan->ev_hp_fork, 0));
    if (f.span) {
      RVAE_CHECK(convert_span(p, f.audio, f.audio_is_i16, f.n_samples, f.frame_idx, f.first_frame, f.count, f.hop,
                              p->x_alt, bg));
      p->x_pitch_alt = f.hop;
    } else {
      RVAE_CHECK(launch_frame_gather(&p->ctx->c, f.audio, f.audio_is_i16, f.n_samples, f.frame_idx, f.first_frame,
                                     f.count, f.hop, p->s_true, p->S, p->x_alt.hi, p->x_alt.lo, nullptr, bg));
      p->x_pitch_alt = 0;
    }
    RVAE_CHECK(draw_eps(p, p->eps_alt, f.count, f.seed, f.offset + (f.add_step ? 1 : 0), f.add_step ? b.step : nullptr,
                        f.noise_row0, bg));
    p->pf.ready_batch = f.count;
    p->pf.registered = false;
    return RVAE_OK;
  };
  static const bool pf_late = getenv("RVAE_PF_LATE") ? atoi(getenv("RVAE_PF_LATE")) != 0 : false;
  if (!pf_late) RVAE_CHECK(enqueue_prefetch());
  RVAE_CHECK(rvae_plan_forward(plan, kl_beta, 1, 0, st));
  if (pf_late) {
    RVAE_CUDA(cudaEventRecord(plan->ev_hp_fork, st));
    RVAE_CHECK(enqueue_prefetch());
  }
  RVAE_CHECK(rvae_plan_finish_loss_deferred(plan, kl_beta, loss_out, ring_size));
  plan->fin.inc_step = 0;
  plan->fin.hp = hp.dev;
  rvae_ctx* cx = plan->ctx;
  const bool dp = plan->dp_enabled && (cx->comm != nullptr || cx->p2p_ready) && cx->dp_world > 1;
  cudaStream_t cs = plan->comm_stream;
  const uint8_t* g0 = reinterpret_cast<const uint8_t*>(b.grads);
  const bool use_p2p = cx->p2p_ready && cx->sym_base != nullptr && g0 >= cx->sym_base + kP2PFlagBytes &&
                       g0 + sizeof(float) * (size_t)plan->lay.total <= cx->sym_base + kP2PFlagBytes + cx->sym_data_bytes;
  RVAE_REQUIRE(!dp || use_p2p || cx->comm != nullptr, RVAE_ERR_STATE, "plan_train_step: no communicator for these gradients");
  auto allreduce_buckets = [&](unsigned mask, int flag_set, int ctas, cudaStream_t cs) -> int {
    P2PSegs sg;
    memset(&sg, 0, sizeof(sg));
    int ns = 0;
    for (int bucket = 0; bucket < 5; ++bucket) {
      if (!(mask & (1u << bucket))) continue;
      float* ptr; int64_t cnt;
      RVAE_CHECK(rvae_plan_bucket(plan, bucket, &ptr, &cnt));
      if (use_p2p) {
        RVAE_REQUIRE(ns < 3, RVAE_ERR_INVALID, "plan_train_step: too many segments in one all-reduce");
        sg.off[ns] = ptr - cx->p2p.data[cx->p2p.rank];
        sg.n[ns] = cnt;
        ++ns;
      } else {
        RVAE_NCCL(cx, cx->nccl.AllReduce(ptr, ptr, (size_t)cnt,  7,  0, cx->comm, cs));
      }
    }
    if (use_p2p) return launch_allreduce_p2p(&cx->c, cx->p2p, sg, flag_set, ctas, cs);
    return RVAE_OK;
  };
  static const unsigned kBucketMask[3] = {0x1, 0x2, 0x4};
  auto finalize_on_bg = [&]() -> int {
    if (!(plan->fin_pending && latent_fused(plan))) return RVAE_OK;
    RVAE_CHECK(launch_loss_finalize_prepared(&cx->c, plan->fin, bg));
    plan->fin_pending = false;
    return RVAE_OK;
  };
  struct DeferGuard {
    rvae_plan* p;
// ... 227 lines not shown
```

rawaudiovae_kelsey_b200/csrc/common.h:

```cpp
#pragma once
#include <cstdarg>
#include <cstdint>
#include <cstdio>
#include <cuda.h>
#include <cuda_bf16.h>
#include <cuda_runtime.h>

#include "../../include/rvae_b200.h"
#include "gemm.cuh"

namespace rvae {

enum : int {
  RVAE_OK = 0,
  RVAE_ERR_INVALID = 1,
  RVAE_ERR_UNSUPPORTED = 2,
  RVAE_ERR_DRIVER = 3,
  RVAE_ERR_STATE = 4,
  RVAE_ERR_CUDA_BASE = 1000,
};

int set_error(int code, const char* fmt, ...);
int cuda_error(cudaError_t err, const char* what);

#define RVAE_CUDA(expr)                                       \
  do {                                                        \
    cudaError_t _e = (expr);                                  \
    if (_e != cudaSuccess) return ::rvae::cuda_error(_e, #expr); \
  } while (0)

#define RVAE_CHECK(expr)           \
  do {                             \
    int _rc = (expr);              \
    if (_rc != RVAE_OK) return _rc; \
  } while (0)

#define RVAE_REQUIRE(cond, code, ...)                        \
  do {                                                       \
    if (!(cond)) return ::rvae::set_error(code, __VA_ARGS__); \
  } while (0)

struct Ctx {
  int device;
  int num_sms;
  int num_sms_total;
  int force_block_n;
  int force_cta_group;
  int debug;
  int use_pdl;
  unsigned long long* trace;
  int trace_launches;
  uint64_t trace_seq;
  unsigned long long* aux_trace;
  int aux_cap;
  uint64_t aux_seq;
  uint64_t launches;
  int aux_grid_cap;
};

template <typename... KArgs, typename... Args>
inline cudaError_t launch_kernel(const Ctx* ctx, void (*kernel)(KArgs...), dim3 grid, dim3 block, size_t smem,
                                 cudaStream_t stream, Args&&... args) {
  cudaLaunchConfig_t cfg = {};
  cfg.gridDim = grid;
  cfg.blockDim = block;
  cfg.dynamicSmemBytes = smem;
  cfg.stream = stream;
  cudaLaunchAttribute attr[1];
  attr[0].id = cudaLaunchAttributeProgrammaticStreamSerialization;
  attr[0].val.programmaticStreamSerializationAllowed = 1;
  cfg.attrs = attr;
  cfg.numAttrs = ctx->use_pdl ? 1 : 0;
  return cudaLaunchKernelEx(&cfg, kernel, static_cast<KArgs>(args)...);
}

struct AuxTrace {
  unsigned long long* slot;
};
inline AuxTrace next_aux(Ctx* ctx, int kind) {
  AuxTrace t;
  t.slot = nullptr;
  if (ctx->aux_trace != nullptr && ctx->aux_cap > 0) {
    t.slot = ctx->aux_trace + (ctx->aux_seq % (uint64_t)ctx->aux_cap) * 8;
    ctx->aux_seq++;
    (void)kind;
  }
  return t;
}

struct Operand {
  const __nv_bfloat16* hi;
  const __nv_bfloat16* lo;
  int major;
  int ld;
  int cols;
};

struct GemmDesc {
  int epi;
  int M, N, K;
  Operand A, B;
  EpiArgs args;
  int head_L;
  int k_splits;
  int side_cols;
};

struct PreparedGemm {
  GemmParams params;
  int block_n;
  int variant;
  int grid;
  int smem_bytes;
  int epi;
  int a_major, b_major, cg;
  int out_rows, out_cols_bf16, out_ld_bf16, out_cols_f32, out_ld_f32;
  int side_cols;
};

int gemm_bind_outputs(PreparedGemm* g, const EpiArgs& args, bool force);

struct PreparedChain {
  ChainParams params;
  int count;
  int variant;
  int grid;
  int smem_bytes;
};
int gemm_prepare_chain(const Ctx* ctx, const PreparedGemm* const* g, int count, int pairs, int* sched_dev,
                       PreparedChain* out, unsigned int* dep_flags = nullptr);
int gemm_run_chain(Ctx* ctx, const PreparedChain& g, cudaStream_t stream);

int gemm_prepare(const Ctx* ctx, const GemmDesc& d, PreparedGemm* out);
int gemm_run(Ctx* ctx, const PreparedGemm& g, cudaStream_t stream);
int gemm_launch(Ctx* ctx, const GemmDesc& d, cudaStream_t stream);

int launch_frame_gather(Ctx* ctx, const void* audio, int audio_is_i16, int64_t n_samples, const int64_t* frame_idx,
                        int64_t first_frame, int64_t n_frames, int hop, int S, int W, __nv_bfloat16* out_hi,
                        __nv_bfloat16* out_lo, float* out_f32, cudaStream_t stream);
int launch_overlap_add(Ctx* ctx, const float* frames, int64_t n_frames, int S, int hop, float* out, int64_t t_begin,
                       int64_t n_out, cudaStream_t stream);
int launch_randn(Ctx* ctx, float* out, int64_t n, uint64_t seed, uint64_t offset, const float* offset_src,
                 int64_t elem_base, cudaStream_t stream);
int launch_randn_rows(Ctx* ctx, float* out, int64_t rows, int64_t cols, int64_t ld, uint64_t seed, uint64_t offset,
                      const float* offset_src, int64_t elem_base, cudaStream_t stream);
int launch_split_bf16_rows(Ctx* ctx, const float* src, int64_t rows, int cols, int ld_src, int ld_dst,
                           __nv_bfloat16* hi, __nv_bfloat16* lo, cudaStream_t stream);
int launch_split_bf16(Ctx* ctx, const float* src, int64_t n, __nv_bfloat16* hi, __nv_bfloat16* lo,
                      cudaStream_t stream);
int launch_colsum(Ctx* ctx, const __nv_bfloat16* hi, const __nv_bfloat16* lo, int64_t M, int N, int ld, float* out,
                  int accumulate, cudaStream_t stream);
int launch_loss_fwd(Ctx* ctx, const float* xhat, const float* x, const float* mu, const float* lv, int64_t B, int S,
                    int L, float beta, double* acc, float* loss_out, cudaStream_t stream);
int launch_frame_loss(Ctx* ctx, const float* xhat, int ld_xhat, const float* mu, const float* lv, int ld_lat,
                      int64_t rows, int S, int L, const void* audio, int audio_is_i16, int64_t n_samples,
                      int64_t first_frame, int hop, float* rec_out, float* kl_out, cudaStream_t stream);
int launch_loss_bwd(Ctx* ctx, const float* xhat, const float* x, const float* mu, const float* lv, int64_t B, int S,
                    int L, float beta, const float* grad_out, float* g_xhat, float* g_mu, float* g_lv,
                    cudaStream_t stream);
int launch_tanh_bwd(Ctx* ctx, const float* g_xhat, const float* xhat, int64_t n, __nv_bfloat16* da_hi,
                    __nv_bfloat16* da_lo, cudaStream_t stream);
int launch_reparam(Ctx* ctx, const float* mu, const float* lv, const float* eps, int64_t n, float* z,
                   cudaStream_t stream);
int launch_lerp_reparam(Ctx* ctx, const float* mu_a, const float* lv_a, const float* mu_b, const float* lv_b,
                        const void* alpha, int alpha_is_f64, const float* eps, int64_t rows, int L, int ld_z,
                        float* z_f32, __nv_bfloat16* z_hi, __nv_bfloat16* z_lo, float* mu_out, float* lv_out,
                        cudaStream_t stream);
int launch_loss_finalize(Ctx* ctx, double* acc, int64_t B, int S, int L, float beta, float* loss_out, int ring_size,
                         float* step, cudaStream_t stream);
struct HpArg {
  const rvae_hparams* dev;
  rvae_hparams val;
};
HpArg hp_value(double lr, double beta1, double beta2, double eps, double weight_decay);
inline HpArg hp_device(const rvae_hparams* dev) { HpArg a = hp_value(0.0, 0.0, 0.0, 0.0, 0.0); a.dev = dev; return a; }
int launch_adam(Ctx* ctx, float* p, float* g, float* m, float* v, int64_t n, double lr, double beta1, double beta2,
                double eps, double weight_decay, float grad_scale, const float* step, __nv_bfloat16* shadow_hi,
                __nv_bfloat16* shadow_lo, int zero_grads, cudaStream_t stream);
int launch_adam2(Ctx* ctx, float* p, float* g, float* m, float* v, int64_t n, int64_t off_b, int64_t n_b,
                 const HpArg& hp, float grad_scale, const float* coef, float* step, int step_bias, unsigned int* ticket,
                 __nv_bfloat16* shadow_hi, __nv_bfloat16* shadow_lo, int zero_grads, cudaStream_t stream);
struct NormFinalize {
  const double* parts;
  int n_parts;
  unsigned int* ticket;
  const float* step;
  float* norm_out;
  int ring_size;
  const double* max_norm;
  float* coef_out;
};
int grad_norm_blocks(const Ctx* ctx, int64_t n);
int launch_grad_norm(Ctx* ctx, const float* g, int64_t n, int64_t off_b, int64_t n_b, double* part,
                     const NormFinalize& f, cudaStream_t stream);
int launch_hparams_eval(Ctx* ctx, const rvae_hparams* hp, const int64_t* k, int n, double* lr_out, float* beta_out,
                        cudaStream_t stream);
int launch_step_inc(Ctx* ctx, float* step, cudaStream_t stream);
size_t param_histogram_bytes(int n_segs, int n_edges);
int launch_param_histogram(Ctx* ctx, const float* params, const int64_t* seg_offsets, const int64_t* seg_lengths,
                           int n_segs, const double* edges, int n_edges, void* record, cudaStream_t stream);
int launch_param_histogram_rows(Ctx* ctx, const float* params, const int64_t* seg_offsets, const int64_t* seg_rows,
                                const int64_t* seg_cols, const int64_t* seg_pitch, int n_segs, const double* edges,
                                int n_edges, void* record, cudaStream_t stream);

constexpr int kP2PMaxWorld = 8;
constexpr int kP2PMaxBuckets = 8;
constexpr int kP2PMaxCtas = 64;
constexpr int kP2PFlagStride = 32;
constexpr size_t kP2PFlagBytes = 1024 * 1024;
struct P2PArgs {
  float* data[kP2PMaxWorld];
  float* mc_data;
  uint32_t* flags[kP2PMaxWorld];
  uint32_t* epoch;
  unsigned int* ticket;
  uint32_t* status;
  long long timeout_cycles;
  int rank, world;
  int mode;
};
struct P2PSegs {
  int64_t off[3];
  int64_t n[3];
};
int launch_allreduce_p2p(Ctx* ctx, const P2PArgs& a, const P2PSegs& sg, int bucket, int ctas, cudaStream_t stream);
struct LossFinalize {
  double* acc;
  double inv_rec, kl_scale;
  float* loss_out;
  int ring_size;
  float* step;
  int inc_step;
  const rvae_hparams* hp;
  double kl_bl;
};
struct KlGrad {
  const rvae_hparams* hp;
  const float* step;
  double bl;
  float c;
  int early;
};
inline KlGrad kl_grad_value(float c) { return KlGrad{nullptr, nullptr, 0.0, c, 0}; }
LossFinalize make_loss_finalize(double* acc, int64_t B, int S, int L, float beta, float* loss_out, int ring_size,
                                float* step);
int launch_loss_finalize_prepared(Ctx* ctx, const LossFinalize& f, cudaStream_t stream);
int launch_latent_bwd(Ctx* ctx, float* dz, const float* eps, const float* lv, const float* mu, const float* g_mu_ext,
                      const float* g_lv_ext, const KlGrad& kl, int64_t M, int L, __nv_bfloat16* dml_hi,
                      __nv_bfloat16* dml_lo, float* bias_grad, int clear_dz, const LossFinalize* fin,
                      cudaStream_t stream);

}
```

rawaudiovae_kelsey_b200/csrc/gemm.cuh:

```cuda
#pragma once
#include <cstdint>
#include <cstdio>
#include <cuda.h>
#include <cuda_bf16.h>
#include <cuda_runtime.h>

#include "ptx.cuh"

#ifndef RVAE_EXPERIMENTS
#define RVAE_EXPERIMENTS 0
#endif

namespace rvae {

constexpr int kBlockM = 128;
constexpr int kBlockK = 64;
constexpr int kUmmaK = 16;
constexpr int kGemmThreads = 320;
constexpr int kEpiTeams = 2;
constexpr int kMaxPasses = 3;
constexpr int kSlotBytes = 128 * 128;
constexpr int kSlotsPerTeam = 3;

enum : int { MAJOR_K = 0, MAJOR_MN = 1 };
enum : int { EPI_LINEAR = 0, EPI_HEAD = 1, EPI_OUT = 2, EPI_DRELU = 3, EPI_REDUCE = 5, EPI_DLATENT = 6 };
enum : int { ACT_NONE = 0, ACT_RELU = 1, ACT_TANH = 2, ACT_TANH_APPROX = 3 };

struct EpiArgs {
  const float* bias;
  __nv_bfloat16* out_hi;
  __nv_bfloat16* out_lo;
  float* out_f32;
  float* out_f32_b;
  const void* in0;
  const void* in1;
  const void* in2;
  double* loss_acc;
  float* colsum;
  int ldo;
  int ldi;
  int act;
  int L;
  int accumulate;
  float c0;
};

struct alignas(64) GemmParams {
  CUtensorMap tmA[kMaxPasses];
  CUtensorMap tmB[kMaxPasses];
  CUtensorMap tmOutHi;
  CUtensorMap tmOutLo;
  CUtensorMap tmOutF32;
  CUtensorMap tmOutF32b;
  CUtensorMap tmSide;
  int M, N, K;
  int num_passes;
  int m_blocks, n_blocks;
  int k_splits, kb_per_split, kb_total;
  int b_tile_stride;
  int b_half_stride;
  int debug;
  unsigned long long* trace;
  unsigned int* dep_signal;
  const unsigned int* dep_wait;
  unsigned int dep_target;
  EpiArgs epi;
};

template <int BLOCK_N, int CG>
struct GemmCfg {
  static constexpr int kABytes = kBlockM * kBlockK * 2;
  static constexpr int kBBytes = (BLOCK_N / CG) * kBlockK * 2;
  static constexpr int kStageBytes = kABytes + kBBytes;
  static constexpr int kSlotRegion = kEpiTeams * kSlotsPerTeam * kSlotBytes;
  static constexpr int kBiasFloats = BLOCK_N / 2 > 128 ? BLOCK_N / 2 : 128;
  static constexpr int kBiasBytes = kEpiTeams * kBiasFloats * 4;
  static constexpr int kCsumBytes = kEpiTeams * 2 * 64 * 4;
  static constexpr int kBarrierBytes = 256;
  static constexpr int kBudget = 232448 - kSlotRegion - kBiasBytes - kCsumBytes - kBarrierBytes;
  static constexpr int kStages = kBudget / kStageBytes > 8 ? 8 : kBudget / kStageBytes;
  static constexpr int kAccStages = 2;
  static constexpr int kTmemCols = (kAccStages * BLOCK_N <= 256) ? 256 : 512;
  static constexpr int kSmemBytes = kStages * kStageBytes + kSlotRegion + kBiasBytes + kCsumBytes + kBarrierBytes;
  static_assert(kStages >= 2, "pipeline too shallow");
};

constexpr int kTraceHeader = 16;
constexpr int kTraceTiles = 24;
constexpr int kTraceEvents = 16;
constexpr int kTraceCtaWords = kTraceHeader + kTraceTiles * kTraceEvents;
__device__ __forceinline__ unsigned long long global_timer() {
  unsigned long long t;
  asm volatile("mov.u64 %0, %%globaltimer;" : "=l"(t));
  return t;
}
__device__ __forceinline__ void trace_hdr(const unsigned long long* trace, int word, unsigned long long v) {
  if (trace) const_cast<unsigned long long*>(trace)[static_cast<size_t>(blockIdx.x) * kTraceCtaWords + word] = v;
}
__device__ __forceinline__ void trace_ev(const unsigned long long* trace, int tile_iter, int ev) {
  if (trace && tile_iter < kTraceTiles)
    const_cast<unsigned long long*>(trace)[static_cast<size_t>(blockIdx.x) * kTraceCtaWords + kTraceHeader +
                                           tile_iter * kTraceEvents + ev] = clock64();
}

__device__ __forceinline__ float warp_sum(float v) {
#pragma unroll
  for (int o = 16; o > 0; o >>= 1) v += __shfl_xor_sync(0xffffffffu, v, o);
  return v;
}

template <int COUNT>
__device__ __forceinline__ void load_row_bf16(const __nv_bfloat16* row, float (&v)[COUNT]) {
  const uint4* s = reinterpret_cast<const uint4*>(row);
#pragma unroll
  for (int i = 0; i < COUNT / 8; ++i) {
    uint4 t = __ldg(s + i);
    const __nv_bfloat162* h = reinterpret_cast<const __nv_bfloat162*>(&t);
#pragma unroll
    for (int j = 0; j < 4; ++j) {
      float2 f = __bfloat1622float2(h[j]);
      v[8 * i + 2 * j] = f.x;
      v[8 * i + 2 * j + 1] = f.y;
    }
  }
}

__device__ __forceinline__ void team_bar_sync(int team) {
  asm volatile("bar.sync %0, 128;" ::"r"(team + 1) : "memory");
}
__device__ __forceinline__ uint4* slot_chunk(uint8_t* slot, int r, int c) {
  return reinterpret_cast<uint4*>(slot + r * 128 + ((c ^ (r & 7)) << 4));
}
__device__ __forceinline__ void stage_bf16(uint8_t* slot, int r, const float* v) {
#pragma unroll
  for (int i = 0; i < 8; ++i)
    *slot_chunk(slot, r, i) =
        make_uint4(ptx::pack_bf16x2(v[8 * i + 0], v[8 * i + 1]), ptx::pack_bf16x2(v[8 * i + 2], v[8 * i + 3]),
                   ptx::pack_bf16x2(v[8 * i + 4], v[8 * i + 5]), ptx::pack_bf16x2(v[8 * i + 6], v[8 * i + 7]));
}
__device__ __forceinline__ float bf16_residual(float v) { return v - __bfloat162float(__float2bfloat16_rn(v)); }
__device__ __forceinline__ void stage_bf16_residual(uint8_t* slot, int r, const float* v) {
#pragma unroll
  for (int i = 0; i < 8; ++i) {
    float q[8];
#pragma unroll
    for (int j = 0; j < 8; ++j) q[j] = bf16_residual(v[8 * i + j]);
    *slot_chunk(slot, r, i) = make_uint4(ptx::pack_bf16x2(q[0], q[1]), ptx::pack_bf16x2(q[2], q[3]),
                                         ptx::pack_bf16x2(q[4], q[5]), ptx::pack_bf16x2(q[6], q[7]));
  }
}
__device__ __forceinline__ void stage_f32(uint8_t* slot, int r, const float* v) {
#pragma unroll
  for (int i = 0; i < 8; ++i)
    *slot_chunk(slot, r, i) = make_uint4(__float_as_uint(v[4 * i]), __float_as_uint(v[4 * i + 1]),
                                         __float_as_uint(v[4 * i + 2]), __float_as_uint(v[4 * i + 3]));
}
__device__ __forceinline__ void unstage_bf16(uint8_t* slot, int r, float* v) {
#pragma unroll
  for (int i = 0; i < 8; ++i) {
    const uint4 t = *slot_chunk(slot, r, i);
    const __nv_bfloat162* h = reinterpret_cast<const __nv_bfloat162*>(&t);
#pragma unroll
    for (int j = 0; j < 4; ++j) {
      const float2 f = __bfloat1622float2(h[j]);
      v[8 * i + 2 * j] = f.x;
      v[8 * i + 2 * j + 1] = f.y;
    }
  }
}
__device__ __forceinline__ void unstage_f32(uint8_t* slot, int r, float* v) {
#pragma unroll
  for (int i = 0; i < 8; ++i) {
    const uint4 t = *slot_chunk(slot, r, i);
    v[4 * i] = __uint_as_float(t.x); v[4 * i + 1] = __uint_as_float(t.y);
    v[4 * i + 2] = __uint_as_float(t.z); v[4 * i + 3] = __uint_as_float(t.w);
  }
}

__device__ __forceinline__ void warp_colsum64(float* v, int lane) {
#pragma unroll
  for (int step = 0; step < 5; ++step) {
    const int half = 32 >> step;
    const int mask = 16 >> step;
    const bool upper = (lane & mask) != 0;
#pragma unroll
    for (int j = 0; j < 32; ++j) {
      if (j < half) {
        const float send = upper ? v[j] : v[j + half];
        const float keep = upper ? v[j + half] : v[j];
        v[j] = keep + __shfl_xor_sync(0xffffffffu, send, mask);
      }
    }
  }
}

__device__ __forceinline__ void warp_colsum16(float* v, int lane) {
#pragma unroll
  for (int step = 0; step < 4; ++step) {
    const int half = 8 >> step;
    const int mask = 16 >> step;
    const bool upper = (lane & mask) != 0;
#pragma unroll
    for (int j = 0; j < 8; ++j) {
      if (j < half) {
        const float send = upper ? v[j] : v[j + half];
        const float keep = upper ? v[j + half] : v[j];
        v[j] = keep + __shfl_xor_sync(0xffffffffu, send, mask);
      }
    }
  }
  v[0] += __shfl_xor_sync(0xffffffffu, v[0], 1);
}

static __device__ __noinline__ float tanh_accurate(float x) { return tanhf(x); }

template <int COUNT>
__device__ __forceinline__ void apply_act(float (&v)[COUNT], int act) {
  if (act == ACT_RELU) {
#pragma unroll
    for (int q = 0; q < COUNT; ++q) v[q] = fmaxf(v[q], 0.f);
  } else if (act == ACT_TANH_APPROX) {
#pragma unroll
    for (int q = 0; q < COUNT; ++q) v[q] = ptx::tanh_approx(v[q]);
  } else if (act == ACT_TANH) {
#pragma unroll
    for (int q = 0; q < COUNT; ++q) v[q] = tanh_accurate(v[q]);
  }
}

struct Team {
  uint8_t* slots;
  uint64_t* in_bar;
  float* bias_s;
  float* csum_s;
  uint32_t use;
  uint32_t in_phase;
  uint32_t cs_par;
  int team;
  bool issuer;

  __device__ __forceinline__ uint8_t* slot(uint32_t u) const { return slots + (u % kSlotsPerTeam) * kSlotBytes; }
  __device__ __forceinline__ void sync() const { team_bar_sync(team); }
  __device__ __forceinline__ void load(uint32_t u, const CUtensorMap* tm, int c0, int c1) const {
    uint64_t* bar = &in_bar[u % kSlotsPerTeam];
    ptx::mbar_arrive_expect_tx(bar, kSlotBytes);
    ptx::tma_load_2d(slot(u), tm, bar, c0, c1);
  }
  __device__ __forceinline__ void wait_load(uint32_t u) {
    const uint32_t s = u % kSlotsPerTeam;
    ptx::mbar_wait(&in_bar[s], (in_phase >> s) & 1u);
    in_phase ^= 1u << s;
  }
  __device__ __forceinline__ void store(uint32_t u, const CUtensorMap* tm, int c0, int c1, bool reduce) const {
    ptx::fence_proxy_async_smem();
    sync();
    if (issuer) {
      if (reduce) ptx::tma_reduce_add_2d(tm, slot(u), c0, c1);
      else ptx::tma_store_2d(tm, slot(u), c0, c1);
      ptx::tma_store_commit();
      ptx::tma_store_wait_read<1>();
    }
  }
  __device__ __forceinline__ void drain() const {
    if (issuer) ptx::tma_store_wait_read<0>();
    sync();
  }
};

template <int A_MAJOR_, int B_MAJOR_, int EPI_>
struct Kind {
  static constexpr int A = A_MAJOR_, B = B_MAJOR_, EPI = EPI_;
};

constexpr int kSchedMax = 16;

constexpr int kMaxChain = 4;
struct alignas(64) ChainParams {
  GemmParams p[kMaxChain];
  const int* sched;
  int base[kMaxChain + 1];
};

struct UnitIter {
  const int* sched;
  int pos, u, stride, total;
  __device__ __forceinline__ UnitIter(const int* sched_, int group_id, int num_groups, int total_)
      : sched(sched_ ? sched_ + group_id * kSchedMax : nullptr), pos(0), u(group_id), stride(num_groups), total(total_) {}
  __device__ __forceinline__ bool next(int& unit) {
    if (sched) {
      if (pos >= kSchedMax) return false;
      unit = __ldg(sched + pos);
      ++pos;
      return unit >= 0;
    }
    if (u >= total) return false;
    unit = u;
    u += stride;
    return true;
  }
};

struct Shared {
  uint8_t* smem;
  uint8_t* slot_base;
  float* bias_strips;
  float* csum_strips;
  uint64_t* full_bar;
  uint64_t* empty_bar;
  uint64_t* tmem_full_bar;
  uint64_t* tmem_empty_bar;
  uint64_t* in_bars;
  uint32_t tmem_base;
  uint32_t cta_rank;
  bool leader;
};

struct TileCoord {
  int ks, n_blk, m_blk, m0, kb_begin, kb_count;
};
template <int CG>
__device__ __forceinline__ TileCoord decode_unit(const GemmParams& p, int u, uint32_t cta_rank) {
  TileCoord t;
  const int tiles = p.m_blocks * p.n_blocks;
  t.ks = u / tiles;
  const int tile = u - t.ks * tiles;
  t.n_blk = tile / p.m_blocks;
  t.m_blk = tile - t.n_blk * p.m_blocks;
  t.m0 = (t.m_blk * CG + static_cast<int>(cta_rank)) * kBlockM;
  t.kb_begin = t.ks * p.kb_per_split;
  t.kb_count = min(p.kb_per_split, p.kb_total - t.kb_begin);
  return t;
}

struct ProdState {
  uint32_t stage, phase;
  bool slot_free;
};

template <class KD, int BLOCK_N, int CG>
__device__ __forceinline__ void produce_unit(const GemmParams& p, int u, ProdState& ps, const Shared& sh, int titer) {
  using Cfg = GemmCfg<BLOCK_N, CG>;
  constexpr int kStages = Cfg::kStages;
  constexpr int A_MAJOR = KD::A, B_MAJOR = KD::B;
  trace_ev(p.trace, titer, 0);
  const TileCoord t = decode_unit<CG>(p, u, sh.cta_rank);
  uint32_t stage = ps.stage, phase = ps.phase;
  bool slot_free = ps.slot_free;
#if RVAE_EXPERIMENTS
  if (p.dep_wait != nullptr) {
    const unsigned int* flag = p.dep_wait + t.m_blk;
    const long long t0 = clock64();
    while (ptx::ld_acquire_gpu(flag) < p.dep_target) {
      __nanosleep(64);
      if (clock64() - t0 > 2000000000ll) {
        printf("rvae: tile dependency timeout block %d row block %d (%u of %u)\n", (int)blockIdx.x, t.m_blk,
               ptx::ld_acquire_gpu(flag), p.dep_target);
        __trap();
      }
    }
    ptx::fence_proxy_async_all();
  }
#endif
  for (int pass = 0; pass < p.num_passes; ++pass) {
    const CUtensorMap* tmA = &p.tmA[pass];
    const CUtensorMap* tmB = &p.tmB[pass];
    for (int kb = t.kb_begin; kb < t.kb_begin + t.kb_count; ++kb) {
      ptx::mbar_wait_probed(slot_free, &sh.empty_bar[stage], phase ^ 1);
      {
        const uint32_t ns = (stage + 1 == kStages) ? 0u : stage + 1;
        const uint32_t np = (stage + 1 == kStages) ? phase ^ 1u : phase;
        slot_free = ptx::mbar_try_wait(&sh.empty_bar[ns], np ^ 1);
      }
      uint64_t* fb = &sh.full_bar[stage];
#if RVAE_EXPERIMENTS
      if (CG == 1 && (p.debug & 2)) {
        ptx::mbar_arrive(fb);
        if (++stage == kStages) { stage = 0; phase ^= 1; }
        continue;
      }
#endif
      if constexpr (CG == 1) {
        ptx::mbar_arrive_expect_tx(fb, Cfg::kStageBytes);
      } else {
        if (sh.leader) ptx::mbar_arrive_expect_tx(fb, 2 * Cfg::kStageBytes);
      }
      uint8_t* sA = sh.smem + stage * Cfg::kStageBytes;
      uint8_t* sB = sA + Cfg::kABytes;
      const int k0 = kb * kBlockK;
      if constexpr (A_MAJOR == MAJOR_K) {
        ptx::tma_load_2d_cg<CG>(sA, tmA, fb, k0, t.m0);
      } else {
#pragma unroll
        for (int i = 0; i < kBlockM / 64; ++i)
          ptx::tma_load_2d_cg<CG>(sA + i * (kBlockK * 128), tmA, fb, t.m0 + i * 64, k0);
      }
      if constexpr (B_MAJOR == MAJOR_K) {
        const int r0 = t.n_blk * p.b_tile_stride;
        if constexpr (CG == 1) {
#pragma unroll
          for (int h = 0; h < 2; ++h)
            ptx::tma_load_2d_cg<1>(sB + h * (Cfg::kBBytes / 2), tmB, fb, k0, r0 + h * p.b_half_stride);
        } else {
          ptx::tma_load_2d_cg<2>(sB, tmB, fb, k0, r0 + static_cast<int>(sh.cta_rank) * p.b_half_stride);
        }
      } else {
        const int n0 = t.n_blk * BLOCK_N + static_cast<int>(sh.cta_rank) * (BLOCK_N / CG);
#pragma unroll
        for (int i = 0; i < BLOCK_N / CG / 64; ++i)
          ptx::tma_load_2d_cg<CG>(sB + i * (kBlockK * 128), tmB, fb, n0 + i * 64, k0);
      }
      if (++stage == kStages) { stage = 0; phase ^= 1; }
    }
  }
  ps.stage = stage; ps.phase = phase; ps.slot_free = slot_free;
  trace_ev(p.trace, titer, 1);
}

struct MmaState {
  uint32_t stage, phase, as, aphase;
  bool data_ready;
};

template <class KD, int BLOCK_N, int CG>
__device__ __forceinline__ void mma_unit(const GemmParams& p, int u, MmaState& ms, const Shared& sh, int titer) {
  using Cfg = GemmCfg<BLOCK_N, CG>;
  constexpr int kStages = Cfg::kStages;
  constexpr int A_MAJOR = KD::A, B_MAJOR = KD::B;
  constexpr uint32_t kIdesc = ptx::umma_idesc_bf16(kBlockM * CG, BLOCK_N, A_MAJOR, B_MAJOR);
  const TileCoord t = decode_unit<CG>(p, u, sh.cta_rank);
  const int iters = t.kb_count * p.num_passes;
  uint32_t stage = ms.stage, phase = ms.phase;
  bool data_ready = ms.data_ready;
  trace_ev(p.trace, titer, 2);
  ptx::mbar_wait(&sh.tmem_empty_bar[ms.as], ms.aphase ^ 1);
  ptx::tc_fence_after();
  trace_ev(p.trace, titer, 3);
  const uint32_t d_tmem = sh.tmem_base + ms.as * BLOCK_N;
  for (int it = 0; it < iters; ++it) {
    ptx::mbar_wait_probed(data_ready, &sh.full_bar[stage], phase);
    {
      const uint32_t ns = (stage + 1 == kStages) ? 0u : stage + 1;
      const uint32_t np = (stage + 1 == kStages) ? phase ^ 1u : phase;
      data_ready = ptx::mbar_try_wait(&sh.full_bar[ns], np);
    }
    ptx::tc_fence_after();
    if (it == 0) trace_ev(p.trace, titer, 4);
#if RVAE_EXPERIMENTS
    if (CG == 1 && (p.debug & 1)) {
      ptx::mbar_arrive(&sh.empty_bar[stage]);
      if (++stage == kStages) { stage = 0; phase ^= 1; }
      continue;
    }
#endif
    const uint32_t a_addr = ptx::smem_u32(sh.smem + stage * Cfg::kStageBytes);
    const uint32_t b_addr = a_addr + Cfg::kABytes;
#pragma unroll
    for (int k = 0; k < kBlockK / kUmmaK; ++k) {
      const uint64_t adesc = (A_MAJOR == MAJOR_K) ? ptx::umma_desc_sw128(a_addr + k * (kUmmaK * 2), 0, 1024)
                                                  : ptx::umma_desc_sw128(a_addr + k * (kUmmaK * 128), kBlockK * 128, 1024);
      const uint64_t bdesc = (B_MAJOR == MAJOR_K) ? ptx::umma_desc_sw128(b_addr + k * (kUmmaK * 2), 0, 1024)
                                                  : ptx::umma_desc_sw128(b_addr + k * (kUmmaK * 128), kBlockK * 128, 1024);
      ptx::umma_bf16<CG>(d_tmem, adesc, bdesc, kIdesc, (it > 0 || k > 0) ? 1u : 0u);
    }
    ptx::umma_commit<CG>(&sh.empty_bar[stage]);
    if (++stage == kStages) { stage = 0; phase ^= 1; }
  }
#if RVAE_EXPERIMENTS
  if (CG == 1 && (p.debug & 1)) ptx::mbar_arrive(&sh.tmem_full_bar[ms.as]);
  else
#endif
  ptx::umma_commit<CG>(&sh.tmem_full_bar[ms.as]);
  trace_ev(p.trace, titer, 5);
  if (++ms.as == Cfg::kAccStages) { ms.as = 0; ms.aphase ^= 1; }
  ms.stage = stage; ms.phase = phase; ms.data_ready = data_ready;
}

struct EpiState {
  Team tm;
  uint32_t as, aphase;
  float loss_local;
  int team, quarter, row, team_tid, lane;
  uint32_t lane_base;
};

template <class KD, int BLOCK_N, int CG>
__device__ __forceinline__ void epilogue_unit(const GemmParams& p, int u, EpiState& es, const Shared& sh, int titer) {
  using Cfg = GemmCfg<BLOCK_N, CG>;
  constexpr int EPI = KD::EPI;
  const EpiArgs& e = p.epi;
  Team& tm = es.tm;
  const int team = es.team, row = es.row, team_tid = es.team_tid, lane = es.lane;
  uint64_t* tmem_full_bar = sh.tmem_full_bar;
  uint32_t& as = es.as;
  uint32_t& aphase = es.aphase;
  float& loss_local = es.loss_local;
  const bool dual = e.out_lo != nullptr;
  const bool tr = team_tid == 0 && team == 0;
  const TileCoord tc = decode_unit<CG>(p, u, sh.cta_rank);
  const int n_blk = tc.n_blk, m0 = tc.m0;
  const int m = m0 + row;
  const bool row_ok = m < p.M;
  const uint32_t t_acc = sh.tmem_base + es.lane_base + as * BLOCK_N;
  (void)lane; (void)tr; (void)dual; (void)row_ok; (void)m;

      if constexpr (EPI == EPI_HEAD) {
        constexpr int kHalf = BLOCK_N / 2;
        static_assert(kHalf / 64 <= kEpiTeams, "one HEAD unit per team per tile");
        const int L = e.L;
        const bool active = team < kHalf / 64;
        const int col0 = n_blk * kHalf + team * 64;
        const bool has_eps = e.in0 != nullptr;
        if (active && team_tid < 128) {
          const int i = team_tid;
          tm.bias_s[i] = (i < 64) ? __ldg(e.bias + col0 + i) : __ldg(e.bias + L + col0 + i - 64);
        }
        if (tm.issuer && active) {
          ptx::tma_store_wait_read<0>();
          if (has_eps) {
            tm.load(0, &p.tmSide, col0, m0);
            tm.load(1, &p.tmSide, col0 + 32, m0);
          }
        }
        ptx::mbar_wait(&tmem_full_bar[as], aphase);
        ptx::tc_fence_after();
        if (team_tid == 0) trace_ev(p.trace, titer, 6 + 2 * team);
        tm.sync();
        if (active) {
          float z[64];
          float lv1[32];
#pragma unroll
          for (int h = 0; h < 2; ++h) {
            const int c = team * 64 + h * 32;
            uint32_t rm[32], rl[32];
            ptx::tmem_ld_32x32(t_acc + c, rm);
            ptx::tmem_ld_32x32(t_acc + kHalf + c, rl);
            if (has_eps) tm.wait_load(h);
            ptx::tmem_ld_wait();
            uint8_t* s_mu = tm.slot(h);
            uint8_t* s_lv = tm.slot(2);
#pragma unroll
            for (int i = 0; i < 8; ++i) {
              float eps[4] = {0.f, 0.f, 0.f, 0.f};
              if (has_eps) {
                const uint4 t = *slot_chunk(s_mu, row, i);
                eps[0] = __uint_as_float(t.x); eps[1] = __uint_as_float(t.y);
                eps[2] = __uint_as_float(t.z); eps[3] = __uint_as_float(t.w);
              }
              float mu[4], lv[4];
#pragma unroll
              for (int q = 0; q < 4; ++q) {
                const int jj = 4 * i + q;
                mu[q] = __uint_as_float(rm[jj]) + tm.bias_s[h * 32 + jj];
                lv[q] = __uint_as_float(rl[jj]) + tm.bias_s[64 + h * 32 + jj];
                const float sig = expf(0.5f * lv[q]);
                z[h * 32 + jj] = fmaf(eps[q], sig, mu[q]);
                if (row_ok) loss_local += (1.f + lv[q]) - fmaf(mu[q], mu[q], sig * sig);
                if (h == 1) lv1[jj] = lv[q];
              }
              *slot_chunk(s_mu, row, i) = make_uint4(__float_as_uint(mu[0]), __float_as_uint(mu[1]),
                                                     __float_as_uint(mu[2]), __float_as_uint(mu[3]));
              if (h == 0)
                *slot_chunk(s_lv, row, i) = make_uint4(__float_as_uint(lv[0]), __float_as_uint(lv[1]),
                                                       __float_as_uint(lv[2]), __float_as_uint(lv[3]));
            }
            ptx::fence_proxy_async_smem();
            if (h == 0) {
              tm.sync();
              if (tm.issuer) {
                ptx::tma_store_2d(&p.tmOutF32, tm.slot(0), col0, m0);
                ptx::tma_store_2d(&p.tmOutF32b, tm.slot(2), col0, m0);
                ptx::tma_store_commit();
              }
            } else {
              if (tm.issuer) ptx::tma_store_wait_read<0>();
              tm.sync();
              if (tm.issuer) {
                ptx::tma_store_2d(&p.tmOutF32, tm.slot(1), col0 + 32, m0);
                ptx::tma_store_commit();
              }
              stage_f32(tm.slot(0), row, lv1);
              if (e.out_hi) stage_bf16(tm.slot(2), row, z);
              ptx::fence_proxy_async_smem();
              tm.sync();
              if (tm.issuer) {
                ptx::tma_store_2d(&p.tmOutF32b, tm.slot(0), col0 + 32, m0);
                if (e.out_hi) ptx::tma_store_2d(&p.tmOutHi, tm.slot(2), col0, m0);
                ptx::tma_store_commit();
              }
            }
          }
          if (e.out_hi && dual) {
            tm.drain();
            stage_bf16_residual(tm.slot(0), row, z);
            ptx::fence_proxy_async_smem();
            tm.sync();
            if (tm.issuer) {
              ptx::tma_store_2d(&p.tmOutLo, tm.slot(0), col0, m0);
              ptx::tma_store_commit();
            }
          }
        }
      } else if constexpr (EPI == EPI_DLATENT) {
        constexpr int kSubs = BLOCK_N / 64;
        constexpr int kUnitsPerTeam = (kSubs + kEpiTeams - 1) / kEpiTeams;
        constexpr int kPieces = kUnitsPerTeam * 8;
        const int L = e.L;
        const float* src[3] = {reinterpret_cast<const float*>(e.in2), reinterpret_cast<const float*>(e.in1),
                               reinterpret_cast<const float*>(e.in0)};
        const size_t row_off = static_cast<size_t>(m) * L;
        auto piece_col = [&](int pc) { return n_blk * BLOCK_N + (team + (pc >> 3) * kEpiTeams) * 64 + (pc & 7) * 8; };
        float4 nx[6];
        auto load_piece = [&](int pc) {
          const int col = pc < kPieces ? piece_col(pc) : p.N;
          if (row_ok && col < p.N) {
#pragma unroll
            for (int a = 0; a < 3; ++a) {
              const float4* g4 = reinterpret_cast<const float4*>(src[a] + row_off + col);
              nx[2 * a] = __ldg(g4);
              nx[2 * a + 1] = __ldg(g4 + 1);
            }
          } else {
#pragma unroll
            for (int a = 0; a < 6; ++a) nx[a] = make_float4(0.f, 0.f, 0.f, 0.f);
          }
        };
        if (row_ok && !(p.debug & 4)) {
#pragma unroll
          for (int j = 0; j < kUnitsPerTeam; ++j) {
            const int n0 = n_blk * BLOCK_N + (team + j * kEpiTeams) * 64;
            if (team + j * kEpiTeams < kSubs && n0 < p.N) {
#pragma unroll
              for (int a = 0; a < 3; ++a) ptx::prefetch_l2_bulk(src[a] + row_off + n0, 256u);
            }
          }
        }
        ptx::mbar_wait(&tmem_full_bar[as], aphase);
        ptx::tc_fence_after();
        if (team_tid == 0) trace_ev(p.trace, titer, 6 + 2 * team);
        load_piece(0);
        float* cs_mu = tm.csum_s;
        float* cs_lv = tm.csum_s + 64;
        __nv_bfloat16* out_row = e.out_hi + static_cast<size_t>(m) * e.ldo;
#pragma unroll 1
        for (int pc = 0; pc < kPieces; ++pc) {
          const int col = piece_col(pc);
          if (col >= p.N) break;
          uint32_t r[8];
          ptx::tmem_ld_32x8(t_acc + (col - n_blk * BLOCK_N), r);
          float in[24];
#pragma unroll
          for (int a = 0; a < 6; ++a) {
            in[4 * a] = nx[a].x; in[4 * a + 1] = nx[a].y; in[4 * a + 2] = nx[a].z; in[4 * a + 3] = nx[a].w;
          }
          load_piece(pc + 1);
          ptx::tmem_ld_wait();
          float o[16];
#pragma unroll
          for (int q = 0; q < 8; ++q) {
            const float d = __uint_as_float(r[q]);
            const float sig = expf(0.5f * in[8 + q]);
            const float gl = 0.5f * e.c0 * (sig * sig - 1.f);
            o[q] = row_ok ? d + e.c0 * in[q] : 0.f;
            o[8 + q] = row_ok ? fmaf(d, 0.5f * in[16 + q] * sig, gl) : 0.f;
          }
          if (row_ok) {
            *reinterpret_cast<uint4*>(out_row + col) =
                make_uint4(ptx::pack_bf16x2(o[0], o[1]), ptx::pack_bf16x2(o[2], o[3]), ptx::pack_bf16x2(o[4], o[5]),
                           ptx::pack_bf16x2(o[6], o[7]));
            *reinterpret_cast<uint4*>(out_row + L + col) =
                make_uint4(ptx::pack_bf16x2(o[8], o[9]), ptx::pack_bf16x2(o[10], o[11]),
                           ptx::pack_bf16x2(o[12], o[13]), ptx::pack_bf16x2(o[14], o[15]));
          }
          if (e.colsum) {
            warp_colsum16(o, lane);
            if ((lane & 1) == 0) {
              const int idx = lane >> 1;
              atomicAdd((idx < 8 ? cs_mu : cs_lv - 8) + (pc & 7) * 8 + idx, o[0]);
            }
            if ((pc & 7) == 7) {
              const int n0 = col - 56;
              tm.sync();
              if (team_tid < 64) {
                atomicAdd(e.colsum + n0 + team_tid, cs_mu[team_tid]);
                atomicAdd(e.colsum + L + n0 + team_tid, cs_lv[team_tid]);
                cs_mu[team_tid] = 0.f;
                cs_lv[team_tid] = 0.f;
              }
              tm.sync();
            }
          }
          if (tr && (pc & 7) == 7) trace_ev(p.trace, titer, 14 + (pc >> 3));
        }
      } else if constexpr (EPI == EPI_REDUCE) {
        ptx::mbar_wait(&tmem_full_bar[as], aphase);
        ptx::tc_fence_after();
        if (team_tid == 0) trace_ev(p.trace, titer, 6 + 2 * team);
        for (int piece = team; piece < BLOCK_N / 32; piece += kEpiTeams) {
          const int n = n_blk * BLOCK_N + piece * 32;
          if (n >= p.N) continue;
          uint32_t r[32];
          ptx::tmem_ld_32x32(t_acc + piece * 32, r);
          ptx::tmem_ld_wait();
          uint8_t* sl = tm.slot(tm.use);
#pragma unroll
          for (int i = 0; i < 8; ++i) *slot_chunk(sl, row, i) = make_uint4(r[4 * i], r[4 * i + 1], r[4 * i + 2], r[4 * i + 3]);
          tm.store(tm.use, &p.tmOutF32, n, m0, e.accumulate != 0);
          ++tm.use;
        }
      } else {
        constexpr int kSubs = BLOCK_N / 64;
        constexpr int kUnitsPerTeam = (kSubs + kEpiTeams - 1) / kEpiTeams;
        static_assert(kUnitsPerTeam <= 2, "side-input prefetch covers at most two units per team and tile");
        constexpr bool kSide = (EPI == EPI_OUT || EPI == EPI_DRELU);
        constexpr bool kBias = (EPI == EPI_LINEAR || EPI == EPI_OUT);
        const bool side = kSide && e.in0 != nullptr && e.out_hi != nullptr;
        const bool do_colsum = kSide && e.colsum != nullptr;
        if constexpr (kBias) {
          if (team_tid < kUnitsPerTeam * 64) {
            const int n = n_blk * BLOCK_N + (team + (team_tid >> 6) * kEpiTeams) * 64 + (team_tid & 63);
            tm.bias_s[team_tid] = (e.bias && n < p.N) ? __ldg(e.bias + n) : 0.f;
          }
        }
        if (side && !dual && tm.issuer) {
#pragma unroll
          for (int j = 0; j < kUnitsPerTeam; ++j) {
            const int sub = team + j * kEpiTeams;
            const int n0 = n_blk * BLOCK_N + sub * 64;
            if (sub < kSubs && n0 < p.N) tm.load(tm.use + j, &p.tmSide, n0, m0);
          }
        }
        ptx::mbar_wait(&tmem_full_bar[as], aphase);
        ptx::tc_fence_after();
        if (team_tid == 0) trace_ev(p.trace, titer, 6 + 2 * team);
        if constexpr (kBias) tm.sync();
        if (e.out_hi) {
#pragma unroll 1
          for (int j = 0; j < kUnitsPerTeam; ++j) {
            const int sub = team + j * kEpiTeams;
            const int n0 = n_blk * BLOCK_N + sub * 64;
            if (sub >= kSubs || n0 >= p.N) continue;
            uint32_t r[64];
            ptx::tmem_ld_32x32(t_acc + sub * 64, *reinterpret_cast<uint32_t(*)[32]>(&r[0]));
            ptx::tmem_ld_32x32(t_acc + sub * 64 + 32, *reinterpret_cast<uint32_t(*)[32]>(&r[32]));
            if (dual) {
              tm.drain();
              tm.use = 0;
              if (side && tm.issuer) tm.load(0, &p.tmSide, n0, m0);
            }
            if (side) tm.wait_load(tm.use);
            if (tr) trace_ev(p.trace, titer, j == 0 ? 10 : 14);
            ptx::tmem_ld_wait();
            if (tr && j == 0) trace_ev(p.trace, titer, 11);
            uint8_t* sl = tm.slot(tm.use);
            float v[64];
#pragma unroll
            for (int q = 0; q < 64; ++q) v[q] = __uint_as_float(r[q]);
            if constexpr (kBias) {
#pragma unroll
              for (int q = 0; q < 64; q += 4) {
                const float4 b = *reinterpret_cast<const float4*>(tm.bias_s + j * 64 + q);
                v[q] += b.x; v[q + 1] += b.y; v[q + 2] += b.z; v[q + 3] += b.w;
              }
            }
            if constexpr (EPI == EPI_LINEAR) {
              apply_act<64>(v, e.act);
            } else if constexpr (EPI == EPI_DRELU) {
              if (side) {
#pragma unroll
                for (int i = 0; i < 8; ++i) {
                  const uint4 t = *slot_chunk(sl, row, i);
                  const uint32_t w[4] = {t.x, t.y, t.z, t.w};
#pragma unroll
                  for (int q = 0; q < 4; ++q) {
                    const uint32_t lo16 = w[q] & 0xffffu, hi16 = w[q] >> 16;
                    if (!(lo16 != 0u && lo16 < 0x8000u)) v[8 * i + 2 * q] = 0.f;
                    if (!(hi16 != 0u && hi16 < 0x8000u)) v[8 * i + 2 * q + 1] = 0.f;
                  }
                }
              }
            } else {
              apply_act<64>(v, e.act == ACT_TANH_APPROX ? ACT_TANH_APPROX : ACT_TANH);
#pragma unroll
              for (int i = 0; i < 8; ++i) {
                float x[8];
                if (side) {
                  const uint4 t = *slot_chunk(sl, row, i);
                  const __nv_bfloat162* hh = reinterpret_cast<const __nv_bfloat162*>(&t);
#pragma unroll
                  for (int q = 0; q < 4; ++q) {
                    const float2 f = __bfloat1622float2(hh[q]);
                    x[2 * q] = f.x; x[2 * q + 1] = f.y;
                  }
                  if (e.in1 && row_ok) {
                    const uint4 t2 = __ldg(reinterpret_cast<const uint4*>(
                        reinterpret_cast<const __nv_bfloat16*>(e.in1) + static_cast<size_t>(m) * (e.ldi ? e.ldi : e.ldo) + n0 + 8 * i));
                    const __nv_bfloat162* h2 = reinterpret_cast<const __nv_bfloat162*>(&t2);
#pragma unroll
                    for (int q = 0; q < 4; ++q) {
                      const float2 f = __bfloat1622float2(h2[q]);
                      x[2 * q] += f.x; x[2 * q + 1] += f.y;
                    }
                  }
                } else {
#pragma unroll
                  for (int q = 0; q < 8; ++q) x[q] = 0.f;
                }
#pragma unroll
                for (int q = 0; q < 8; ++q) {
                  const float xh = v[8 * i + q];
                  const float d = xh - x[q];
                  if (row_ok) loss_local = fmaf(d, d, loss_local);
                  v[8 * i + q] = row_ok ? e.c0 * d * (1.f - xh * xh) : 0.f;
                }
              }
            }
            stage_bf16(sl, row, v);
            if (dual) stage_bf16_residual(tm.slot(tm.use + 1), row, v);
            if (tr && j == 0) trace_ev(p.trace, titer, 12);
            float* cs = tm.csum_s + (tm.cs_par << 6);
            if (do_colsum) {
              warp_colsum64(v, lane);
              atomicAdd(cs + 2 * lane, v[0]);
              atomicAdd(cs + 2 * lane + 1, v[1]);
            }
            tm.store(tm.use, &p.tmOutHi, n0, m0, false);
            if (dual && tm.issuer) {
              ptx::tma_store_2d(&p.tmOutLo, tm.slot(tm.use + 1), n0, m0);
              ptx::tma_store_commit();
            }
            if (tr) trace_ev(p.trace, titer, j == 0 ? 13 : 15);
            if (do_colsum) {
              if (team_tid < 64) {
                atomicAdd(e.colsum + n0 + team_tid, cs[team_tid]);
                cs[team_tid] = 0.f;
              }
              tm.cs_par ^= 1u;
            }
            ++tm.use;
          }
        }
        if constexpr (kBias) {
          if (e.out_f32) {
            if (dual) { tm.drain(); tm.use = 0; }
#pragma unroll 1
            for (int jp = 0; jp < 2 * kUnitsPerTeam; ++jp) {
              const int j = jp >> 1, hf = jp & 1;
              const int sub = team + j * kEpiTeams;
              const int n = n_blk * BLOCK_N + sub * 64 + hf * 32;
              if (sub >= kSubs || n >= p.N) continue;
              uint32_t r[32];
              ptx::tmem_ld_32x32(t_acc + sub * 64 + hf * 32, r);
              ptx::tmem_ld_wait();
              float v[32];
#pragma unroll
              for (int q = 0; q < 32; ++q) v[q] = __uint_as_float(r[q]) + tm.bias_s[j * 64 + hf * 32 + q];
              apply_act<32>(v, (EPI == EPI_OUT && e.act != ACT_TANH_APPROX) ? ACT_TANH : e.act);
              if constexpr (EPI == EPI_OUT) {
                if (!e.out_hi && row_ok) {
                  const size_t off = static_cast<size_t>(m) * (e.ldi ? e.ldi : e.ldo) + n;
                  float x[32];
                  load_row_bf16<32>(reinterpret_cast<const __nv_bfloat16*>(e.in0) + off, x);
                  if (e.in1) {
                    float xl[32];
                    load_row_bf16<32>(reinterpret_cast<const __nv_bfloat16*>(e.in1) + off, xl);
#pragma unroll
                    for (int q = 0; q < 32; ++q) x[q] += xl[q];
                  }
#pragma unroll
                  for (int q = 0; q < 32; ++q) loss_local = fmaf(v[q] - x[q], v[q] - x[q], loss_local);
                }
              }
              stage_f32(tm.slot(tm.use), row, v);
              tm.store(tm.use, &p.tmOutF32, n, m0, false);
              ++tm.use;
            }
          }
        }
      }
  ptx::tc_fence_before();
  __syncwarp();
  if (lane == 0) {
    if (CG == 1 || sh.leader) ptx::mbar_arrive(&sh.tmem_empty_bar[as]);
    else ptx::mbar_arrive_remote(&sh.tmem_empty_bar[as], 0);
  }
#if RVAE_EXPERIMENTS
  if (p.dep_signal != nullptr && tm.issuer) {
    ptx::tma_store_wait<0>();
    __threadfence();
    atomicAdd(p.dep_signal + tc.m_blk, 1u);
  }
#endif
  if (team_tid == 0) trace_ev(p.trace, titer, 7 + 2 * team);
  if (++as == Cfg::kAccStages) { as = 0; aphase ^= 1; }
}

struct NoKind {
  static constexpr int A = 0, B = 0, EPI = -1;
};
template <class K>
struct is_kind { static constexpr bool value = true; };
template <>
struct is_kind<NoKind> { static constexpr bool value = false; };

struct ProblemSet {
  const GemmParams* p[kMaxChain];
  int base[kMaxChain + 1];
  const int* sched;
};

#define RVAE_DISPATCH(FN, STATE)                                                                                  \
  do {                                                                                                            \
    if (u < ps.base[1]) {                                                                                         \
      FN<K0, BLOCK_N, CG>(*ps.p[0], u, STATE, sh, titer);                                                         \
    } else if (u < ps.base[2]) {                                                                                  \
      if constexpr (is_kind<K1>::value) FN<K1, BLOCK_N, CG>(*ps.p[1], u - ps.base[1], STATE, sh, titer);          \
    } else if (u < ps.base[3]) {                                                                                  \
      if constexpr (is_kind<K2>::value) FN<K2, BLOCK_N, CG>(*ps.p[2], u - ps.base[2], STATE, sh, titer);          \
    } else {                                                                                                      \
      if constexpr (is_kind<K3>::value) FN<K3, BLOCK_N, CG>(*ps.p[3], u - ps.base[3], STATE, sh, titer);          \
    }                                                                                                             \
  } while (0)

template <int BLOCK_N, int CG, class K0, class K1, class K2, class K3>
__device__ __forceinline__ void gemm_body(const ProblemSet& ps) {
  using Cfg = GemmCfg<BLOCK_N, CG>;
  constexpr int kStages = Cfg::kStages;
  const GemmParams& p = *ps.p[0];

  extern __shared__ __align__(1024) uint8_t smem[];
  Shared sh;
  sh.smem = smem;
  sh.slot_base = smem + kStages * Cfg::kStageBytes;
  sh.bias_strips = reinterpret_cast<float*>(sh.slot_base + Cfg::kSlotRegion);
  sh.csum_strips = sh.bias_strips + kEpiTeams * Cfg::kBiasFloats;
  sh.full_bar = reinterpret_cast<uint64_t*>(sh.csum_strips + kEpiTeams * 128);
  sh.empty_bar = sh.full_bar + kStages;
  sh.tmem_full_bar = sh.empty_bar + kStages;
  sh.tmem_empty_bar = sh.tmem_full_bar + Cfg::kAccStages;
  sh.in_bars = sh.tmem_empty_bar + Cfg::kAccStages;
  uint32_t* tmem_slot = reinterpret_cast<uint32_t*>(sh.in_bars + kEpiTeams * kSlotsPerTeam);
  static_assert((2 * 8 + 2 * 2 + kEpiTeams * kSlotsPerTeam) * 8 + 4 <= Cfg::kBarrierBytes, "barrier region");

  const int warp = threadIdx.x >> 5;
  const int lane = threadIdx.x & 31;
  sh.cta_rank = (CG == 2) ? ptx::cluster_ctarank() : 0u;
  sh.leader = sh.cta_rank == 0;
  const int group_id = (CG == 2) ? (blockIdx.x >> 1) : blockIdx.x;
  const int num_groups = (CG == 2) ? (gridDim.x >> 1) : gridDim.x;

  if (threadIdx.x == 0) {
    if ((ptx::smem_u32(smem) & 1023u) != 0) {
      printf("rvae: dynamic shared memory base is not 1024-byte aligned\n");
      __trap();
    }
    trace_hdr(p.trace, 0, global_timer());
    trace_hdr(p.trace, 1, clock64());
  }
  if (warp == 0 && lane == 0) {
#pragma unroll
    for (int q = 0; q < kMaxChain; ++q) {
      if (ps.base[q + 1] == ps.base[q]) continue;
      const GemmParams& pq = *ps.p[q];
      for (int i = 0; i < pq.num_passes; ++i) {
        ptx::prefetch_tensormap(&pq.tmA[i]);
        ptx::prefetch_tensormap(&pq.tmB[i]);
      }
      ptx::prefetch_tensormap(&pq.tmOutHi);
      ptx::prefetch_tensormap(&pq.tmOutLo);
      ptx::prefetch_tensormap(&pq.tmOutF32);
      ptx::prefetch_tensormap(&pq.tmOutF32b);
      ptx::prefetch_tensormap(&pq.tmSide);
    }
    for (int i = 0; i < kStages; ++i) {
      ptx::mbar_init(&sh.full_bar[i], 1);
      ptx::mbar_init(&sh.empty_bar[i], 1);
    }
    for (int i = 0; i < Cfg::kAccStages; ++i) {
      ptx::mbar_init(&sh.tmem_full_bar[i], 1);
      ptx::mbar_init(&sh.tmem_empty_bar[i], 8 * CG);
    }
    for (int i = 0; i < kEpiTeams * kSlotsPerTeam; ++i) ptx::mbar_init(&sh.in_bars[i], 1);
    ptx::fence_barrier_init();
  }
  if (warp == 1) ptx::tmem_alloc<CG>(tmem_slot, Cfg::kTmemCols);
  if (threadIdx.x >= 64 && threadIdx.x < 64 + kEpiTeams * 128) sh.csum_strips[threadIdx.x - 64] = 0.f;
  ptx::tc_fence_before();
  if constexpr (CG == 2) ptx::cluster_sync(); else __syncthreads();
  ptx::tc_fence_after();
  sh.tmem_base = *tmem_slot;
  if (threadIdx.x == 0) trace_hdr(p.trace, 2, clock64());
  ptx::pdl_wait();
  if (threadIdx.x == 0) trace_hdr(p.trace, 3, clock64());

  UnitIter it(ps.sched, group_id, num_groups, ps.base[1]);

  if (warp == 0) {
    if (lane == 0) {
      ProdState st{0u, 0u, ptx::mbar_try_wait(&sh.empty_bar[0], 1)};
      int titer = 0, u;
      while (it.next(u)) {
        RVAE_DISPATCH(produce_unit, st);
        ++titer;
      }
      trace_hdr(p.trace, 4, clock64());
    }
  } else if (warp == 1) {
    if (lane == 0 && sh.leader) {
      MmaState st{0u, 0u, 0u, 0u, false};
      int titer = 0, u;
      while (it.next(u)) {
        RVAE_DISPATCH(mma_unit, st);
        ++titer;
      }
    }
  } else {
    EpiState es;
    es.team = (warp - 2) >> 2;
    es.quarter = warp & 3;
    es.lane = lane;
    es.row = es.quarter * 32 + lane;
    es.team_tid = (((warp - 2) & 3) << 5) | lane;
    es.lane_base = static_cast<uint32_t>(es.quarter * 32) << 16;
    es.tm = Team{sh.slot_base + es.team * (kSlotsPerTeam * kSlotBytes), sh.in_bars + es.team * kSlotsPerTeam,
                 sh.bias_strips + es.team * Cfg::kBiasFloats, sh.csum_strips + es.team * 128, 0u, 0u, 0u, es.team,
                 es.team_tid == 0};
    es.as = 0; es.aphase = 0; es.loss_local = 0.f;
    float loss[kMaxChain] = {0.f, 0.f, 0.f, 0.f};
    int titer = 0, u;
    while (it.next(u)) {
      RVAE_DISPATCH(epilogue_unit, es);
      const int q = (u >= ps.base[1]) + (u >= ps.base[2]) + (u >= ps.base[3]);
#pragma unroll
      for (int i = 0; i < kMaxChain; ++i)
        if (i == q) loss[i] += es.loss_local;
      es.loss_local = 0.f;
      ++titer;
    }
    ptx::pdl_launch_dependents();
    if (es.tm.issuer) ptx::tma_store_wait<0>();
    auto flush_loss = [&](int i, int epi) {
      if (epi == EPI_HEAD || epi == EPI_OUT) {
        const float s = warp_sum(loss[i]);
        if (lane == 0 && ps.p[i]->epi.loss_acc) atomicAdd(ps.p[i]->epi.loss_acc, static_cast<double>(s));
      }
    };
    flush_loss(0, K0::EPI);
    if constexpr (is_kind<K1>::value) flush_loss(1, K1::EPI);
    if constexpr (is_kind<K2>::value) flush_loss(2, K2::EPI);
    if constexpr (is_kind<K3>::value) flush_loss(3, K3::EPI);
  }

  ptx::tc_fence_before();
  if constexpr (CG == 2) ptx::cluster_sync(); else __syncthreads();
  if (warp == 1) {
    __syncwarp();
    ptx::tc_fence_after();
    ptx::tmem_dealloc<CG>(sh.tmem_base, Cfg::kTmemCols);
  }
  if (threadIdx.x == 0) {
    trace_hdr(p.trace, 5, clock64());
    trace_hdr(p.trace, 6, global_timer());
  }
}

__device__ __forceinline__ ProblemSet single_problem(const GemmParams& p) {
  ProblemSet ps;
  const int total = p.m_blocks * p.n_blocks * p.k_splits;
  ps.p[0] = ps.p[1] = ps.p[2] = ps.p[3] = &p;
  ps.base[0] = 0;
  ps.base[1] = ps.base[2] = ps.base[3] = ps.base[4] = total;
  ps.sched = nullptr;
  return ps;
}

template <int BLOCK_N, int A_MAJOR, int B_MAJOR, int EPI>
__global__ void __launch_bounds__(kGemmThreads, 1) gemm_kernel(const __grid_constant__ GemmParams p) {
  gemm_body<BLOCK_N, 1, Kind<A_MAJOR, B_MAJOR, EPI>, NoKind, NoKind, NoKind>(single_problem(p));
}

template <int BLOCK_N, int A_MAJOR, int B_MAJOR, int EPI>
__global__ void __cluster_dims__(2, 1, 1) __launch_bounds__(kGemmThreads, 1)
gemm_kernel_2cta(const __grid_constant__ GemmParams p) {
  gemm_body<BLOCK_N, 2, Kind<A_MAJOR, B_MAJOR, EPI>, NoKind, NoKind, NoKind>(single_problem(p));
}

template <int BLOCK_N, class K0, class K1, class K2, class K3>
__global__ void __cluster_dims__(2, 1, 1) __launch_bounds__(kGemmThreads, 1)
gemm_chain_kernel_2cta(const __grid_constant__ ChainParams cp) {
  ProblemSet ps;
#pragma unroll
  for (int i = 0; i < kMaxChain; ++i) ps.p[i] = &cp.p[i];
#pragma unroll
  for (int i = 0; i <= kMaxChain; ++i) ps.base[i] = cp.base[i];
  ps.sched = cp.sched;
  gemm_body<BLOCK_N, 2, K0, K1, K2, K3>(ps);
}

}
```

rawaudiovae_kelsey_b200/csrc/gemm_host.cu:

```cuda
#include <cstdlib>
#include <cstring>
#include <algorithm>
#include <mutex>
#include <vector>

#include "common.h"

namespace rvae {

static thread_local char g_last_error[512] = "";

int set_error(int code, const char* fmt, ...) {
  va_list ap;
  va_start(ap, fmt);
  vsnprintf(g_last_error, sizeof(g_last_error), fmt, ap);
  va_end(ap);
  return code;
}
int cuda_error(cudaError_t err, const char* what) {
  snprintf(g_last_error, sizeof(g_last_error), "CUDA error %d (%s) in %s", (int)err, cudaGetErrorString(err), what);
  return RVAE_ERR_CUDA_BASE + (int)err;
}
const char* last_error() { return g_last_error; }

typedef CUresult (*EncodeTiledFn)(CUtensorMap*, CUtensorMapDataType, cuuint32_t, void*, const cuuint64_t*,
                                  const cuuint64_t*, const cuuint32_t*, const cuuint32_t*, CUtensorMapInterleave,
                                  CUtensorMapSwizzle, CUtensorMapL2promotion, CUtensorMapFloatOOBfill);

static EncodeTiledFn get_encode_fn() {
  static EncodeTiledFn fn = nullptr;
  static std::once_flag once;
  std::call_once(once, [] {
    void* p = nullptr;
    cudaDriverEntryPointQueryResult q;
    if (cudaGetDriverEntryPoint("cuTensorMapEncodeTiled", &p, cudaEnableDefault, &q) == cudaSuccess &&
        q == cudaDriverEntryPointSuccess)
      fn = reinterpret_cast<EncodeTiledFn>(p);
  });
  return fn;
}

static int encode_2d(CUtensorMap* tm, const void* base, bool f32, uint64_t dim0, uint64_t dim1, uint64_t ld,
                     uint32_t box0, uint32_t box1) {
  EncodeTiledFn fn = get_encode_fn();
  const uint64_t esz = f32 ? 4 : 2;
  RVAE_REQUIRE(fn != nullptr, RVAE_ERR_DRIVER, "cuTensorMapEncodeTiled entry point unavailable");
  RVAE_REQUIRE((reinterpret_cast<uintptr_t>(base) & 15) == 0, RVAE_ERR_INVALID, "tensor base %p not 16-byte aligned",
               base);
  RVAE_REQUIRE((ld * esz) % 16 == 0, RVAE_ERR_UNSUPPORTED, "row pitch %llu elements is not a multiple of 16 bytes",
               (unsigned long long)ld);
  cuuint64_t gdim[2] = {dim0, dim1};
  cuuint64_t gstride[1] = {ld * esz};
  cuuint32_t box[2] = {box0, box1};
  cuuint32_t estr[2] = {1, 1};
  CUresult r = fn(tm, f32 ? CU_TENSOR_MAP_DATA_TYPE_FLOAT32 : CU_TENSOR_MAP_DATA_TYPE_BFLOAT16, 2,
                  const_cast<void*>(base), gdim, gstride, box, estr, CU_TENSOR_MAP_INTERLEAVE_NONE,
                  CU_TENSOR_MAP_SWIZZLE_128B, CU_TENSOR_MAP_L2_PROMOTION_L2_256B, CU_TENSOR_MAP_FLOAT_OOB_FILL_NONE);
  RVAE_REQUIRE(r == CUDA_SUCCESS, RVAE_ERR_DRIVER,
               "cuTensorMapEncodeTiled failed (%d): dims %llu x %llu ld %llu box %u x %u", (int)r,
               (unsigned long long)dim0, (unsigned long long)dim1, (unsigned long long)ld, box0, box1);
  return RVAE_OK;
}
static int encode_bf16_2d(CUtensorMap* tm, const void* base, uint64_t dim0, uint64_t dim1, uint64_t ld,
                          uint32_t box0, uint32_t box1) {
  return encode_2d(tm, base, false, dim0, dim1, ld, box0, box1);
}

int gemm_bind_outputs(PreparedGemm* g, const EpiArgs& a, bool force) {
  GemmParams& p = g->params;
  const EpiArgs old = p.epi;
  p.epi = a;
  if (a.out_hi && (force || a.out_hi != old.out_hi))
    RVAE_CHECK(encode_2d(&p.tmOutHi, a.out_hi, false, g->out_cols_bf16, g->out_rows, g->out_ld_bf16, 64, 128));
  if (a.out_lo && (force || a.out_lo != old.out_lo))
    RVAE_CHECK(encode_2d(&p.tmOutLo, a.out_lo, false, g->out_cols_bf16, g->out_rows, g->out_ld_bf16, 64, 128));
  if (a.out_f32 && (force || a.out_f32 != old.out_f32))
    RVAE_CHECK(encode_2d(&p.tmOutF32, a.out_f32, true, g->out_cols_f32, g->out_rows, g->out_ld_f32, 32, 128));
  if (a.out_f32_b && g->epi == EPI_HEAD && (force || a.out_f32_b != old.out_f32_b))
    RVAE_CHECK(encode_2d(&p.tmOutF32b, a.out_f32_b, true, g->out_cols_f32, g->out_rows, g->out_ld_f32, 32, 128));
  if (a.in0 && (force || a.in0 != old.in0 || a.ldi != old.ldi)) {
    if (g->epi == EPI_HEAD)
      RVAE_CHECK(encode_2d(&p.tmSide, a.in0, true, g->out_cols_f32, g->out_rows, g->out_ld_f32, 32, 128));
    else if (g->epi == EPI_OUT || g->epi == EPI_DRELU)
      RVAE_CHECK(encode_2d(&p.tmSide, a.in0, false, g->side_cols > 0 ? g->side_cols : g->out_cols_bf16, g->out_rows,
                           (g->epi == EPI_OUT && a.ldi > 0) ? a.ldi : g->out_ld_bf16, 64, 128));
  }
  return RVAE_OK;
}

typedef void (*GemmKernel)(const GemmParams);

struct Variant {
  int block_n, a_major, b_major, epi, cg;
  GemmKernel fn;
  int smem;
};

#define RVAE_VARIANT(BN, AM, BM, EP)                                                          \
  { BN, AM, BM, EP, 1, gemm_kernel<BN, AM, BM, EP>, GemmCfg<BN, 1>::kSmemBytes },             \
  { BN, AM, BM, EP, 2, gemm_kernel_2cta<BN, AM, BM, EP>, GemmCfg<BN, 2>::kSmemBytes }

static const Variant kVariants[] = {
    RVAE_VARIANT(256, MAJOR_K, MAJOR_K, EPI_LINEAR),  RVAE_VARIANT(128, MAJOR_K, MAJOR_K, EPI_LINEAR),
    RVAE_VARIANT(256, MAJOR_K, MAJOR_K, EPI_HEAD),    RVAE_VARIANT(128, MAJOR_K, MAJOR_K, EPI_HEAD),
    RVAE_VARIANT(256, MAJOR_K, MAJOR_K, EPI_OUT),     RVAE_VARIANT(128, MAJOR_K, MAJOR_K, EPI_OUT),
    RVAE_VARIANT(256, MAJOR_K, MAJOR_MN, EPI_DRELU),  RVAE_VARIANT(128, MAJOR_K, MAJOR_MN, EPI_DRELU),
    RVAE_VARIANT(256, MAJOR_K, MAJOR_MN, EPI_REDUCE),  RVAE_VARIANT(128, MAJOR_K, MAJOR_MN, EPI_REDUCE),
    RVAE_VARIANT(256, MAJOR_MN, MAJOR_MN, EPI_REDUCE), RVAE_VARIANT(128, MAJOR_MN, MAJOR_MN, EPI_REDUCE),
#if RVAE_EXPERIMENTS
    {256, MAJOR_K, MAJOR_MN, EPI_DLATENT, 2, gemm_kernel_2cta<256, MAJOR_K, MAJOR_MN, EPI_DLATENT>,
     GemmCfg<256, 2>::kSmemBytes},
#endif
};
static const int kNumVariants = sizeof(kVariants) / sizeof(kVariants[0]);

static int find_variant(int block_n, int a_major, int b_major, int epi, int cg) {
  for (int i = 0; i < kNumVariants; ++i)
    if (kVariants[i].block_n == block_n && kVariants[i].a_major == a_major && kVariants[i].b_major == b_major &&
        kVariants[i].epi == epi && kVariants[i].cg == cg)
      return i;
  return -1;
}

static int configure_variants() {
  static int rc = -1;
  static std::once_flag once;
  std::call_once(once, [] {
    rc = RVAE_OK;
    for (int i = 0; i < kNumVariants; ++i) {
      cudaError_t e = cudaFuncSetAttribute(reinterpret_cast<const void*>(kVariants[i].fn),
                                           cudaFuncAttributeMaxDynamicSharedMemorySize, kVariants[i].smem);
      if (e != cudaSuccess) {
        rc = cuda_error(e, "cudaFuncSetAttribute(MaxDynamicSharedMemorySize)");
        break;
      }
    }
  });
  return rc;
}

static inline int ceil_div(int a, int b) { return (a + b - 1) / b; }

static void choose_tile(const Ctx* ctx, int M, int N, bool allow128, bool allow256, int* block_n, int* cg) {
  int g = (M > kBlockM) ? 2 : 1;
  if (ctx->force_cta_group == 1 || ctx->force_cta_group == 2) g = ctx->force_cta_group;
  *cg = g;
  const int slots = ctx->num_sms / g;
  const int mb = ceil_div(M, kBlockM * g);
  if (ctx->force_block_n == 128 && allow128) { *block_n = 128; return; }
  if (ctx->force_block_n == 256 && allow256) { *block_n = 256; return; }
  if (!allow256) { *block_n = 128; return; }
  if (!allow128) { *block_n = 256; return; }
  if (N % 256 != 0) { *block_n = 128; return; }
  const double c256 = 1.0 * ceil_div(mb * ceil_div(N, 256), slots);
  const double c128 = 0.6 * ceil_div(mb * ceil_div(N, 128), slots);
  *block_n = (c128 < c256) ? 128 : 256;
}

int gemm_prepare(const Ctx* ctx, const GemmDesc& d, PreparedGemm* out) {
  RVAE_REQUIRE(d.M > 0 && d.N > 0 && d.K > 0, RVAE_ERR_INVALID, "gemm: empty problem %d x %d x %d", d.M, d.N, d.K);
  RVAE_REQUIRE(d.A.hi && d.B.hi, RVAE_ERR_INVALID, "gemm: null operand");
  RVAE_REQUIRE(d.N % 64 == 0, RVAE_ERR_UNSUPPORTED, "gemm: N=%d must be a multiple of 64", d.N);
  RVAE_CHECK(configure_variants());

  PreparedGemm& g = *out;
  memset(&g, 0, sizeof(g));
  GemmParams& p = g.params;
  p.M = d.M; p.N = d.N; p.K = d.K;
  p.epi = d.args;
  p.debug = ctx->debug;
  p.trace = nullptr;

  int block_n, cg;
  if (d.epi == EPI_HEAD) {
    const int L = d.head_L;
    RVAE_REQUIRE(d.N == 2 * L && L % 64 == 0, RVAE_ERR_UNSUPPORTED, "head gemm: N=%d must be 2*L, L=%d %% 64 == 0",
                 d.N, L);
    choose_tile(ctx, d.M, d.N, true, L % 128 == 0, &block_n, &cg);
    p.n_blocks = L / (block_n / 2);
    p.b_tile_stride = block_n / 2;
    p.b_half_stride = L;
    p.epi.L = L;
  } else {
    choose_tile(ctx, d.M, d.N, d.epi != EPI_DLATENT && (d.epi != EPI_REDUCE || d.N % 256 != 0), true, &block_n, &cg);
    if (d.epi == EPI_DLATENT)
      RVAE_REQUIRE(d.args.in0 && d.args.in1 && d.args.in2 && d.args.out_hi && !d.args.out_lo && !d.A.lo && !d.B.lo &&
                       d.args.L == d.N && d.args.ldo == 2 * d.N,
                   RVAE_ERR_UNSUPPORTED, "latent dgrad gemm: bf16 mode with eps, logvar, mu and d_ml [M, 2L] only");
    p.n_blocks = ceil_div(d.N, block_n);
    p.b_tile_stride = block_n;
    p.b_half_stride = block_n / 2;
  }
  p.m_blocks = ceil_div(d.M, kBlockM * cg);
  const int slots = ctx->num_sms / cg;
  p.kb_total = ceil_div(d.K, kBlockK);

  int splits = 1;
  if (d.epi == EPI_REDUCE) {
    const int tiles = p.m_blocks * p.n_blocks;
    static const int env_splits = getenv("RVAE_WGRAD_SPLITS") ? atoi(getenv("RVAE_WGRAD_SPLITS")) : 0;
    if (d.k_splits > 0) {
      splits = d.k_splits;
    } else if (env_splits > 0 && d.A.major == MAJOR_MN) {
      splits = env_splits;
    } else {
      double best = 0.0;
      for (int s = 1; s <= 8 && p.kb_total / s >= 8; ++s) {
        const int units = tiles * s;
        const double eff = (double)units / (ceil_div(units, slots) * (double)slots);
        if (eff > best + 1e-9) { best = eff; splits = s; }
        if (eff >= 0.90) break;
      }
    }
    if (splits > p.kb_total) splits = p.kb_total;
    RVAE_REQUIRE(splits == 1 || d.args.accumulate, RVAE_ERR_INVALID, "reduce gemm: split-K needs accumulate=1");
  }
  p.kb_per_split = ceil_div(p.kb_total, splits);
  p.k_splits = ceil_div(p.kb_total, p.kb_per_split);

  const Operand* pa[kMaxPasses];
  const void* a_ptr[kMaxPasses];
  const void* b_ptr[kMaxPasses];
  (void)pa;
  int np = 0;
  if (d.A.lo && d.B.lo) {
    a_ptr[np] = d.A.lo; b_ptr[np] = d.B.hi; ++np;
    a_ptr[np] = d.A.hi; b_ptr[np] = d.B.lo; ++np;
  } else if (d.A.lo) {
    a_ptr[np] = d.A.lo; b_ptr[np] = d.B.hi; ++np;
  } else if (d.B.lo) {
    a_ptr[np] = d.A.hi; b_ptr[np] = d.B.lo; ++np;
  }
  a_ptr[np] = d.A.hi; b_ptr[np] = d.B.hi; ++np;
  p.num_passes = np;

  const int b_rows = (d.epi == EPI_HEAD) ? d.N : d.N;
  auto dim0 = [](const Operand& o, int extent) { return (uint64_t)(o.cols > 0 && o.cols < extent ? o.cols : extent); };
  for (int i = 0; i < np; ++i) {
    if (d.A.major == MAJOR_K)
      RVAE_CHECK(encode_bf16_2d(&p.tmA[i], a_ptr[i], dim0(d.A, d.K), d.M, d.A.ld, kBlockK, kBlockM));
    else
      RVAE_CHECK(encode_bf16_2d(&p.tmA[i], a_ptr[i], dim0(d.A, d.M), d.K, d.A.ld, 64, kBlockK));
    if (d.B.major == MAJOR_K)
      RVAE_CHECK(encode_bf16_2d(&p.tmB[i], b_ptr[i], dim0(d.B, d.K), b_rows, d.B.ld, kBlockK, block_n / 2));
    else
      RVAE_CHECK(encode_bf16_2d(&p.tmB[i], b_ptr[i], dim0(d.B, d.N), d.K, d.B.ld, 64, kBlockK));
  }

  g.epi = d.epi;
  g.out_rows = d.M;
  g.side_cols = d.epi == EPI_OUT ? d.side_cols : 0;
  if (d.epi == EPI_HEAD) {
    g.out_cols_bf16 = d.head_L; g.out_ld_bf16 = d.head_L;
    g.out_cols_f32 = d.head_L; g.out_ld_f32 = d.head_L;
  } else if (d.epi == EPI_DLATENT) {
    g.out_cols_bf16 = 2 * d.N; g.out_ld_bf16 = d.args.ldo;
    g.out_cols_f32 = d.N; g.out_ld_f32 = d.N;
  } else {
    g.out_cols_bf16 = d.N; g.out_ld_bf16 = d.args.ldo;
    g.out_cols_f32 = d.N; g.out_ld_f32 = d.args.ldo;
  }
  RVAE_CHECK(gemm_bind_outputs(&g, p.epi, true));

  g.block_n = block_n;
  g.a_major = d.A.major; g.b_major = d.B.major; g.cg = cg;
  g.variant = find_variant(block_n, d.A.major, d.B.major, d.epi, cg);
  RVAE_REQUIRE(g.variant >= 0, RVAE_ERR_UNSUPPORTED, "gemm: no kernel for block_n=%d majors (%d,%d) epilogue %d",
               block_n, d.A.major, d.B.major, d.epi);
  const int units = p.m_blocks * p.n_blocks * p.k_splits;
  const int waves = ceil_div(units, slots);
  const int slots_eff = ceil_div(units, waves);
  g.grid = cg * (units < slots_eff ? units : slots_eff);
  g.smem_bytes = kVariants[g.variant].smem;
  return RVAE_OK;
}

int gemm_run(Ctx* ctx, const PreparedGemm& g, cudaStream_t stream) {
  if (ctx->trace != nullptr) {
    GemmParams p = g.params;
    const uint64_t slab = ctx->trace_launches > 1 ? ctx->trace_seq % (uint64_t)ctx->trace_launches : 0;
    p.trace = ctx->trace + slab * (uint64_t)ctx->num_sms_total * kTraceCtaWords;
    ctx->trace_seq++;
    RVAE_CUDA(launch_kernel(ctx, kVariants[g.variant].fn, dim3(g.grid), dim3(kGemmThreads), (size_t)g.smem_bytes,
                            stream, p));
    ctx->launches++;
    return RVAE_OK;
  }
  RVAE_CUDA(launch_kernel(ctx, kVariants[g.variant].fn, dim3(g.grid), dim3(kGemmThreads), (size_t)g.smem_bytes, stream,
                          g.params));
  ctx->launches++;
  return RVAE_OK;
}

typedef void (*ChainKernel)(const ChainParams);
struct KindId {
  int a, b, e;
};
struct ChainVariant {
  int count;
  KindId k[kMaxChain];
  ChainKernel fn;
};
using KDrelu = Kind<MAJOR_K, MAJOR_MN, EPI_DRELU>;
using KWgrad = Kind<MAJOR_MN, MAJOR_MN, EPI_REDUCE>;
using KDz = Kind<MAJOR_K, MAJOR_MN, EPI_REDUCE>;
using KDlat = Kind<MAJOR_K, MAJOR_MN, EPI_DLATENT>;
using KLinear = Kind<MAJOR_K, MAJOR_K, EPI_LINEAR>;
using KHead = Kind<MAJOR_K, MAJOR_K, EPI_HEAD>;
using KOut = Kind<MAJOR_K, MAJOR_K, EPI_OUT>;
#define RVAE_KID(K) {K::A, K::B, K::EPI}
static const ChainVariant kChainVariants[] = {
    {2, {RVAE_KID(KDrelu), RVAE_KID(KWgrad)}, gemm_chain_kernel_2cta<256, KDrelu, KWgrad, NoKind, NoKind>},
    {2, {RVAE_KID(KDz), RVAE_KID(KWgrad)}, gemm_chain_kernel_2cta<256, KDz, KWgrad, NoKind, NoKind>},

#if RVAE_EXPERIMENTS
    {3, {RVAE_KID(KDrelu), RVAE_KID(KWgrad), RVAE_KID(KWgrad)}, gemm_chain_kernel_2cta<256, KDrelu, KWgrad, KWgrad, NoKind>},
    {2, {RVAE_KID(KDlat), RVAE_KID(KWgrad)}, gemm_chain_kernel_2cta<256, KDlat, KWgrad, NoKind, NoKind>},
    {2, {RVAE_KID(KLinear), RVAE_KID(KHead)}, gemm_chain_kernel_2cta<256, KLinear, KHead, NoKind, NoKind>},
    {2, {RVAE_KID(KLinear), RVAE_KID(KOut)}, gemm_chain_kernel_2cta<256, KLinear, KOut, NoKind, NoKind>},
    {4, {RVAE_KID(KLinear), RVAE_KID(KHead), RVAE_KID(KLinear), RVAE_KID(KOut)},
     gemm_chain_kernel_2cta<256, KLinear, KHead, KLinear, KOut>},
#endif
};
static const int kNumChainVariants = sizeof(kChainVariants) / sizeof(kChainVariants[0]);

static int configure_chain_variants() {
  static int rc = -1;
  static std::once_flag once;
  std::call_once(once, [] {
    rc = RVAE_OK;
    for (int i = 0; i < kNumChainVariants; ++i) {
      cudaError_t e = cudaFuncSetAttribute(reinterpret_cast<const void*>(kChainVariants[i].fn),
                                           cudaFuncAttributeMaxDynamicSharedMemorySize, GemmCfg<256, 2>::kSmemBytes);
      if (e != cudaSuccess) {
        rc = cuda_error(e, "cudaFuncSetAttribute(MaxDynamicSharedMemorySize)");
        break;
      }
    }
  });
  return rc;
}

static double unit_cost(const PreparedGemm& g) {
  const double mma = (double)g.params.kb_per_split * g.params.num_passes;
  const double epi = (g.epi == EPI_DRELU || g.epi == EPI_OUT) ? 11.0 : 8.0;
  if (g.epi == EPI_DLATENT) return mma + 22.0 + 2.0;
  return (mma > epi ? mma : epi) + 2.0;
}

int gemm_prepare_chain(const Ctx* ctx, const PreparedGemm* const* g, int count, int pairs, int* sched_dev,
                       PreparedChain* out, unsigned int* dep_flags) {
  RVAE_REQUIRE(count >= 2 && count <= kMaxChain, RVAE_ERR_INVALID, "chain gemm: %d problems", count);
  for (int i = 0; i < count; ++i)
    RVAE_REQUIRE(g[i]->block_n == 256 && g[i]->cg == 2, RVAE_ERR_UNSUPPORTED,
                 "chain gemm: every problem must use 256-wide pair tiles");
  RVAE_REQUIRE(sched_dev != nullptr && pairs >= 1 && 2 * pairs <= ctx->num_sms_total, RVAE_ERR_INVALID,
               "chain gemm: bad schedule buffer / pair count %d", pairs);
  RVAE_CHECK(configure_chain_variants());
  int variant = -1;
  for (int v = 0; v < kNumChainVariants && variant < 0; ++v) {
    const ChainVariant& cv = kChainVariants[v];
    if (cv.count != count) continue;
    bool match = true;
    for (int i = 0; i < count; ++i)
      match = match && cv.k[i].a == g[i]->a_major && cv.k[i].b == g[i]->b_major && cv.k[i].e == g[i]->epi;
    if (match) variant = v;
  }
  RVAE_REQUIRE(variant >= 0, RVAE_ERR_UNSUPPORTED, "chain gemm: no fused kernel for this combination of problems");
  int nunits[kMaxChain], base[kMaxChain + 1];
  base[0] = 0;
  for (int i = 0; i < kMaxChain; ++i) {
    nunits[i] = i < count ? g[i]->params.m_blocks * g[i]->params.n_blocks * g[i]->params.k_splits : 0;
    base[i + 1] = base[i] + nunits[i];
  }
  RVAE_REQUIRE(base[kMaxChain] <= pairs * kSchedMax, RVAE_ERR_UNSUPPORTED, "chain gemm: %d units exceed the schedule",
               base[kMaxChain]);
  struct U { int id; double cost; };
  std::vector<U> units;
  units.reserve(base[kMaxChain]);
  if (dep_flags == nullptr) {
    for (int i = 0; i < count; ++i)
      for (int u = 0; u < nunits[i]; ++u) units.push_back({base[i] + u, unit_cost(*g[i])});
    std::stable_sort(units.begin(), units.end(), [](const U& a, const U& b) { return a.cost > b.cost; });
  } else {
    for (int i = 0; i < count; ++i) {
      const int mb = g[i]->params.m_blocks, nb = g[i]->params.n_blocks;
      RVAE_REQUIRE(g[i]->params.k_splits == 1 && mb == g[0]->params.m_blocks && g[i]->params.M == g[0]->params.M &&
                       mb <= 256,
                   RVAE_ERR_UNSUPPORTED, "chain gemm: chained problems must share the row blocking");
      for (int m = 0; m < mb; ++m)
        for (int n = 0; n < nb; ++n) units.push_back({base[i] + n * mb + m, unit_cost(*g[i])});
    }
  }
  std::vector<double> load(pairs, 0.0);
  std::vector<int> cnt(pairs, 0);
  std::vector<int> sched((size_t)pairs * kSchedMax, -1);
  for (const U& u : units) {
    int best = -1;
    for (int pidx = 0; pidx < pairs; ++pidx)
      if (cnt[pidx] < kSchedMax && (best < 0 || load[pidx] < load[best] - 1e-9)) best = pidx;
    RVAE_REQUIRE(best >= 0, RVAE_ERR_UNSUPPORTED, "chain gemm: schedule overflow");
    sched[(size_t)best * kSchedMax + cnt[best]++] = u.id;
    load[best] += u.cost;
  }
  if (dep_flags == nullptr) {
    static const int order_mode = getenv("RVAE_CHAIN_ORDER") ? atoi(getenv("RVAE_CHAIN_ORDER")) : 1;
    auto prob_of = [&](int id) { int q = 0; while (q + 1 < count && id >= base[q + 1]) ++q; return q; };
    for (int pidx = 0; pidx < pairs && order_mode == 1; ++pidx) {
      int* row = &sched[(size_t)pidx * kSchedMax];
      std::vector<int> heavy, light;
      double min_mma = 1e30;
      for (int k = 0; k < cnt[pidx]; ++k) {
        const PreparedGemm& gq = *g[prob_of(row[k])];
        min_mma = std::min(min_mma, (double)gq.params.kb_per_split * gq.params.num_passes);
      }
      for (int k = 0; k < cnt[pidx]; ++k) {
        const PreparedGemm& gq = *g[prob_of(row[k])];
        const double mma = (double)gq.params.kb_per_split * gq.params.num_passes;
        (mma > 1.5 * min_mma ? heavy : light).push_back(row[k]);
      }
      if (heavy.empty() || light.size() < 2) continue;
      std::vector<int> merged;
      const size_t nh = heavy.size(), nl = light.size();
      size_t li = 0;
      for (size_t h = 0; h < nh; ++h) {
        size_t upto = (h + 1) * nl / (nh + 1);
        if (h == 0 && upto < 2 && nl >= 3) upto = 2;
        if (upto < li + (h == 0 ? 1 : 0)) upto = li + (h == 0 ? 1 : 0);
        if (upto > nl) upto = nl;
        while (li < upto) merged.push_back(light[li++]);
        merged.push_back(heavy[h]);
      }
      while (li < nl) merged.push_back(light[li++]);
      for (size_t k = 0; k < merged.size(); ++k) row[k] = merged[k];
    }
  }
  RVAE_CUDA(cudaMemcpy(sched_dev, sched.data(), sched.size() * sizeof(int), cudaMemcpyHostToDevice));
  PreparedChain& d = *out;
  memset(&d, 0, sizeof(d));
  for (int i = 0; i < kMaxChain; ++i) d.params.p[i] = g[i < count ? i : 0]->params;
  for (int i = 0; i <= kMaxChain; ++i) d.params.base[i] = base[i];
  d.params.sched = sched_dev;
  RVAE_REQUIRE(dep_flags == nullptr || RVAE_EXPERIMENTS, RVAE_ERR_UNSUPPORTED,
               "chain gemm: dependent problems need a build with RVAE_EXPERIMENTS=1");
  if (dep_flags != nullptr) {
    for (int i = 0; i + 1 < count; ++i) {
      unsigned int* flags = dep_flags + 256 * i;
      d.params.p[i].dep_signal = flags;
      d.params.p[i + 1].dep_wait = flags;
      d.params.p[i + 1].dep_target = (unsigned)(g[i]->params.n_blocks * 2 * kEpiTeams);
    }
  }
  d.count = count;
  d.variant = variant;
  d.grid = 2 * pairs;
  d.smem_bytes = GemmCfg<256, 2>::kSmemBytes;
  return RVAE_OK;
}

int gemm_run_chain(Ctx* ctx, const PreparedChain& g, cudaStream_t stream) {
  if (ctx->trace != nullptr) {
    ChainParams p = g.params;
    const uint64_t slab = ctx->trace_launches > 1 ? ctx->trace_seq % (uint64_t)ctx->trace_launches : 0;
    for (int i = 0; i < kMaxChain; ++i) p.p[i].trace = ctx->trace + slab * (uint64_t)ctx->num_sms_total * kTraceCtaWords;
    ctx->trace_seq++;
    RVAE_CUDA(launch_kernel(ctx, kChainVariants[g.variant].fn, dim3(g.grid), dim3(kGemmThreads), (size_t)g.smem_bytes,
                            stream, p));
    ctx->launches++;
    return RVAE_OK;
  }
  RVAE_CUDA(launch_kernel(ctx, kChainVariants[g.variant].fn, dim3(g.grid), dim3(kGemmThreads), (size_t)g.smem_bytes,
                          stream, g.params));
  ctx->launches++;
  return RVAE_OK;
}

int gemm_launch(Ctx* ctx, const GemmDesc& d, cudaStream_t stream) {
  PreparedGemm g;
  RVAE_CHECK(gemm_prepare(ctx, d, &g));
  return gemm_run(ctx, g, stream);
}

}
```

Baseline: 25.93 million.

## Add stream-K work decomposition for reduce-add wgrad GEMMs and chain schedules

Schedule entries now carry explicit K-block ranges (tile, kb_begin, kb_count), so a unit of work can be any slice of a tile's K loop. For chains, reduce-add (accumulating) wgrad problems are split stream-K style and water-filled onto the pairs to even out per-pair load left by the whole-tile problems. When a capped grid is too small for the tile/split count, a standalone accumulating wgrad GEMM switches to a stream-K iterator. The aim is to remove load imbalance and tail idling from fixed k-splits, at the cost of more atomic partial-sum traffic, larger schedule entries, and a forced TMEM drain in the dual epilogue.

```diff
diff --git a/rawaudiovae_kelsey_b200/csrc/capi.cu b/rawaudiovae_kelsey_b200/csrc/capi.cu
--- a/rawaudiovae_kelsey_b200/csrc/capi.cu
+++ b/rawaudiovae_kelsey_b200/csrc/capi.cu
@@ -569,7 +569,7 @@
   float* eps_alt;
   int cur;
   int x_pitch, x_pitch_alt;
-  int* sched_dev;
+  SchedEntry* sched_dev;
   int sched_batch;
   unsigned int* dep_flags;
   bool fuse_forward;
@@ -666,7 +666,7 @@
   p->eps = reinterpret_cast<float*>(take(B * L * 4));
   p->eps_alt = reinterpret_cast<float*>(take(B * L * 4));
   p->ticket = reinterpret_cast<unsigned int*>(take(256));
-  p->sched_dev = reinterpret_cast<int*>(take(sizeof(int) * 2 * 6 * 128 * kSchedMax));
+  p->sched_dev = reinterpret_cast<SchedEntry*>(take(sizeof(SchedEntry) * 2 * 6 * 128 * kSchedMax));
   p->dep_flags = reinterpret_cast<unsigned int*>(take(sizeof(unsigned int) * 3 * 256));
   p->norm_parts = reinterpret_cast<double*>(take(sizeof(double) * kNormGroups * kNormMaxBlocks));
   p->clip_coef = reinterpret_cast<float*>(take(sizeof(float)));
@@ -1028,7 +1028,7 @@
     if (gs->dual_lat_state == 0) {
       RVAE_CHECK(prepare(p, *gs, G_B3D_LAT));
       RVAE_CHECK(prepare(p, *gs, G_B3W));
-      int* sched = p->sched_dev + ((size_t)p->cur * 6 + 4) * 128 * kSchedMax;
+      SchedEntry* sched = p->sched_dev + ((size_t)p->cur * 6 + 4) * 128 * kSchedMax;
       const PreparedGemm* both[2] = {&gs->g[G_B3D_LAT], &gs->g[G_B3W]};
       const int rc = gemm_prepare_chain(&p->ctx->c, both, 2, pairs, sched, &gs->dual_lat);
       gs->dual_lat_state = rc == RVAE_OK ? 1 : -1;
@@ -1078,7 +1078,7 @@
       RVAE_CHECK(prepare(p, *gs, G_B2D));
       RVAE_CHECK(prepare(p, *gs, G_B2W));
       RVAE_CHECK(prepare(p, *gs, G_B3W));
-      int* sched = p->sched_dev + ((size_t)p->cur * 6 + 5) * 128 * kSchedMax;
+      SchedEntry* sched = p->sched_dev + ((size_t)p->cur * 6 + 5) * 128 * kSchedMax;
       const PreparedGemm* three[3] = {&gs->g[G_B2D], &gs->g[G_B2W], &gs->g[G_B3W]};
       const int rc = gemm_prepare_chain(&p->ctx->c, three, 3, stage_pairs(2), sched, &gs->tri);
       gs->tri_state = rc == RVAE_OK ? 1 : -1;
@@ -1122,7 +1122,7 @@
       TimedScope ts(p, G_B3W, st);
       PreparedGemm w = gs->g[G_B3W];
       p->t_flops[G_B3W] = 2.0 * w.params.M * w.params.N * w.params.K;
-      if (w.grid > p->s1_wgrad_ctas) w.grid = p->s1_wgrad_ctas;
+      gemm_limit_grid(&w, p->s1_wgrad_ctas);
       RVAE_CHECK(gemm_run(&p->ctx->c, w, st));
     }
     TimedScope ts(p, T_LATENT, st);
@@ -1147,7 +1147,7 @@
     auto run_wgrad = [&]() -> int {
       PreparedGemm w = gs->g[G_B3W];
       const int cap = (p->dp_enabled && p->ctx->dp_world > 1 && p->s1_wgrad_ctas > 64) ? 64 : p->s1_wgrad_ctas;
-      if (w.grid > cap) w.grid = cap;
+      gemm_limit_grid(&w, cap);
       return gemm_run(&p->ctx->c, w, s_w);
     };
     auto run_latent = [&]() -> int {
@@ -1172,7 +1172,7 @@
     if (gs->dual_state[stage] == 0) {
       RVAE_CHECK(prepare(p, *gs, kDgrad[stage]));
       RVAE_CHECK(prepare(p, *gs, kWgrad[stage]));
-      int* sched = p->sched_dev + ((size_t)p->cur * 6 + stage) * 128 * kSchedMax;
+      SchedEntry* sched = p->sched_dev + ((size_t)p->cur * 6 + stage) * 128 * kSchedMax;
       const PreparedGemm* both[2] = {&gs->g[kDgrad[stage]], &gs->g[kWgrad[stage]]};
       const int rc = gemm_prepare_chain(&p->ctx->c, both, 2, pairs, sched, &gs->dual[stage]);
       gs->dual_state[stage] = rc == RVAE_OK ? 1 : -1;
@@ -1514,7 +1514,7 @@
         RVAE_CHECK(prepare(p, *gs, kLayers[k]));
         layers[k] = &gs->g[kLayers[k]];
       }
-      int* sched = p->sched_dev + ((size_t)p->cur * 6 + 3) * 128 * kSchedMax;
+      SchedEntry* sched = p->sched_dev + ((size_t)p->cur * 6 + 3) * 128 * kSchedMax;
       int fpairs = p->dual_pairs;
       if (const char* e = getenv("RVAE_DUAL_PAIRS_F")) {
         const int v = atoi(e);
diff --git a/rawaudiovae_kelsey_b200/csrc/common.h b/rawaudiovae_kelsey_b200/csrc/common.h
--- a/rawaudiovae_kelsey_b200/csrc/common.h
+++ b/rawaudiovae_kelsey_b200/csrc/common.h
@@ -127,12 +127,13 @@
   int grid;
   int smem_bytes;
 };
-int gemm_prepare_chain(const Ctx* ctx, const PreparedGemm* const* g, int count, int pairs, int* sched_dev,
+int gemm_prepare_chain(const Ctx* ctx, const PreparedGemm* const* g, int count, int pairs, SchedEntry* sched_dev,
                        PreparedChain* out, unsigned int* dep_flags = nullptr);
 int gemm_run_chain(Ctx* ctx, const PreparedChain& g, cudaStream_t stream);
 
 int gemm_prepare(const Ctx* ctx, const GemmDesc& d, PreparedGemm* out);
 int gemm_run(Ctx* ctx, const PreparedGemm& g, cudaStream_t stream);
+void gemm_limit_grid(PreparedGemm* g, int ctas);
 int gemm_launch(Ctx* ctx, const GemmDesc& d, cudaStream_t stream);
 
 int launch_frame_gather(Ctx* ctx, const void* audio, int audio_is_i16, int64_t n_samples, const int64_t* frame_idx,
diff --git a/rawaudiovae_kelsey_b200/csrc/gemm.cuh b/rawaudiovae_kelsey_b200/csrc/gemm.cuh
--- a/rawaudiovae_kelsey_b200/csrc/gemm.cuh
+++ b/rawaudiovae_kelsey_b200/csrc/gemm.cuh
@@ -272,30 +272,74 @@
   static constexpr int A = A_MAJOR_, B = B_MAJOR_, EPI = EPI_;
 };
 
-constexpr int kSchedMax = 16;
+struct Work {
+  int u, kb_begin, kb_count;
+};
+
+typedef int4 SchedEntry;
+constexpr int kSchedMax = 24;
+
+__host__ __device__ __forceinline__ long long streamk_bound(long long T, int g, int P) { return T * g / P; }
 
 constexpr int kMaxChain = 4;
 struct alignas(64) ChainParams {
   GemmParams p[kMaxChain];
-  const int* sched;
+  const SchedEntry* sched;
   int base[kMaxChain + 1];
 };
 
 struct UnitIter {
-  const int* sched;
-  int pos, u, stride, total;
-  __device__ __forceinline__ UnitIter(const int* sched_, int group_id, int num_groups, int total_)
-      : sched(sched_ ? sched_ + group_id * kSchedMax : nullptr), pos(0), u(group_id), stride(num_groups), total(total_) {}
-  __device__ __forceinline__ bool next(int& unit) {
+  const SchedEntry* sched;
+  int pos;
+  bool streamk;
+  long long cur, end;
+  long long tail;
+  int v, stride, total, tiles, kbt, kbps;
+  __device__ __forceinline__ UnitIter(const SchedEntry* sched_, const GemmParams& p, int group_id, int num_groups)
+      : sched(sched_ ? sched_ + group_id * kSchedMax : nullptr), pos(0), streamk(sched_ == nullptr && p.k_splits == 0),
+        cur(0), end(0), tail(-1), v(group_id), stride(num_groups), total(0), tiles(p.m_blocks * p.n_blocks),
+        kbt(p.kb_total), kbps(p.kb_per_split) {
+    if (streamk) {
+      const long long T = static_cast<long long>(tiles) * kbt;
+      cur = streamk_bound(T, group_id, num_groups);
+      end = streamk_bound(T, group_id + 1, num_groups);
+      if (end > cur) {
+        const long long last0 = (end - 1) / kbt * kbt;
+        const long long first_end = min(end, (cur / kbt + 1) * kbt);
+        if (last0 > cur && end - last0 < first_end - cur) tail = last0;
+      }
+    } else {
+      total = tiles * p.k_splits;
+    }
+  }
+  __device__ __forceinline__ bool next(Work& w) {
     if (sched) {
       if (pos >= kSchedMax) return false;
-      unit = __ldg(sched + pos);
+      const SchedEntry e = __ldg(sched + pos);
       ++pos;
-      return unit >= 0;
-    }
-    if (u >= total) return false;
-    unit = u;
-    u += stride;
+      w = Work{e.x, e.y, e.z};
+      return e.x >= 0;
+    }
+    if (streamk) {
+      if (tail >= 0) {
+        const int tile = static_cast<int>(tail / kbt);
+        w = Work{tile, static_cast<int>(tail - static_cast<long long>(tile) * kbt), static_cast<int>(end - tail)};
+        end = tail;
+        tail = -1;
+        return true;
+      }
+      if (cur >= end) return false;
+      const int tile = static_cast<int>(cur / kbt);
+      const int kb0 = static_cast<int>(cur - static_cast<long long>(tile) * kbt);
+      const int n = static_cast<int>(min(end - cur, static_cast<long long>(kbt - kb0)));
+      w = Work{tile, kb0, n};
+      cur += n;
+      return true;
+    }
+    if (v >= total) return false;
+    const int ks = v / tiles;
+    w = Work{v - ks * tiles, ks * kbps, min(kbps, kbt - ks * kbps)};
+    v += stride;
     return true;
   }
 };
@@ -316,19 +360,16 @@
 };
 
 struct TileCoord {
-  int ks, n_blk, m_blk, m0, kb_begin, kb_count;
+  int n_blk, m_blk, m0, kb_begin, kb_count;
 };
 template <int CG>
-__device__ __forceinline__ TileCoord decode_unit(const GemmParams& p, int u, uint32_t cta_rank) {
+__device__ __forceinline__ TileCoord decode_unit(const GemmParams& p, const Work& w, uint32_t cta_rank) {
   TileCoord t;
-  const int tiles = p.m_blocks * p.n_blocks;
-  t.ks = u / tiles;
-  const int tile = u - t.ks * tiles;
-  t.n_blk = tile / p.m_blocks;
-  t.m_blk = tile - t.n_blk * p.m_blocks;
+  t.n_blk = w.u / p.m_blocks;
+  t.m_blk = w.u - t.n_blk * p.m_blocks;
   t.m0 = (t.m_blk * CG + static_cast<int>(cta_rank)) * kBlockM;
-  t.kb_begin = t.ks * p.kb_per_split;
-  t.kb_count = min(p.kb_per_split, p.kb_total - t.kb_begin);
+  t.kb_begin = w.kb_begin;
+  t.kb_count = w.kb_count;
   return t;
 }
 
@@ -338,12 +379,12 @@
 };
 
 template <class KD, int BLOCK_N, int CG>
-__device__ __forceinline__ void produce_unit(const GemmParams& p, int u, ProdState& ps, const Shared& sh, int titer) {
+__device__ __forceinline__ void produce_unit(const GemmParams& p, const Work& w, ProdState& ps, const Shared& sh, int titer) {
   using Cfg = GemmCfg<BLOCK_N, CG>;
   constexpr int kStages = Cfg::kStages;
   constexpr int A_MAJOR = KD::A, B_MAJOR = KD::B;
   trace_ev(p.trace, titer, 0);
-  const TileCoord t = decode_unit<CG>(p, u, sh.cta_rank);
+  const TileCoord t = decode_unit<CG>(p, w, sh.cta_rank);
   uint32_t stage = ps.stage, phase = ps.phase;
   bool slot_free = ps.slot_free;
 #if RVAE_EXPERIMENTS
@@ -422,12 +463,12 @@
 };
 
 template <class KD, int BLOCK_N, int CG>
-__device__ __forceinline__ void mma_unit(const GemmParams& p, int u, MmaState& ms, const Shared& sh, int titer) {
+__device__ __forceinline__ void mma_unit(const GemmParams& p, const Work& w, MmaState& ms, const Shared& sh, int titer) {
   using Cfg = GemmCfg<BLOCK_N, CG>;
   constexpr int kStages = Cfg::kStages;
   constexpr int A_MAJOR = KD::A, B_MAJOR = KD::B;
   constexpr uint32_t kIdesc = ptx::umma_idesc_bf16(kBlockM * CG, BLOCK_N, A_MAJOR, B_MAJOR);
-  const TileCoord t = decode_unit<CG>(p, u, sh.cta_rank);
+  const TileCoord t = decode_unit<CG>(p, w, sh.cta_rank);
   const int iters = t.kb_count * p.num_passes;
   uint32_t stage = ms.stage, phase = ms.phase;
   bool data_ready = ms.data_ready;
@@ -484,7 +525,7 @@
 };
 
 template <class KD, int BLOCK_N, int CG>
-__device__ __forceinline__ void epilogue_unit(const GemmParams& p, int u, EpiState& es, const Shared& sh, int titer) {
+__device__ __forceinline__ void epilogue_unit(const GemmParams& p, const Work& w, EpiState& es, const Shared& sh, int titer) {
   using Cfg = GemmCfg<BLOCK_N, CG>;
   constexpr int EPI = KD::EPI;
   const EpiArgs& e = p.epi;
@@ -496,7 +537,7 @@
   float& loss_local = es.loss_local;
   const bool dual = e.out_lo != nullptr;
   const bool tr = team_tid == 0 && team == 0;
-  const TileCoord tc = decode_unit<CG>(p, u, sh.cta_rank);
+  const TileCoord tc = decode_unit<CG>(p, w, sh.cta_rank);
   const int n_blk = tc.n_blk, m0 = tc.m0;
   const int m = m0 + row;
   const bool row_ok = m < p.M;
@@ -839,9 +880,9 @@
             ++tm.use;
           }
         }
+        if (dual) { tm.drain(); tm.use = 0; }
         if constexpr (kBias) {
           if (e.out_f32) {
-            if (dual) { tm.drain(); tm.use = 0; }
 #pragma unroll 1
             for (int jp = 0; jp < 2 * kUnitsPerTeam; ++jp) {
               const int j = jp >> 1, hf = jp & 1;
@@ -905,19 +946,23 @@
 struct ProblemSet {
   const GemmParams* p[kMaxChain];
   int base[kMaxChain + 1];
-  const int* sched;
+  const SchedEntry* sched;
 };
 
 #define RVAE_DISPATCH(FN, STATE)                                                                                  \
   do {                                                                                                            \
+    const int u = w.u;                                                                                            \
     if (u < ps.base[1]) {                                                                                         \
-      FN<K0, BLOCK_N, CG>(*ps.p[0], u, STATE, sh, titer);                                                         \
+      FN<K0, BLOCK_N, CG>(*ps.p[0], w, STATE, sh, titer);                                                         \
     } else if (u < ps.base[2]) {                                                                                  \
-      if constexpr (is_kind<K1>::value) FN<K1, BLOCK_N, CG>(*ps.p[1], u - ps.base[1], STATE, sh, titer);          \
+      if constexpr (is_kind<K1>::value)                                                                           \
+        FN<K1, BLOCK_N, CG>(*ps.p[1], Work{u - ps.base[1], w.kb_begin, w.kb_count}, STATE, sh, titer);            \
     } else if (u < ps.base[3]) {                                                                                  \
-      if constexpr (is_kind<K2>::value) FN<K2, BLOCK_N, CG>(*ps.p[2], u - ps.base[2], STATE, sh, titer);          \
+      if constexpr (is_kind<K2>::value)                                                                           \
+        FN<K2, BLOCK_N, CG>(*ps.p[2], Work{u - ps.base[2], w.kb_begin, w.kb_count}, STATE, sh, titer);            \
     } else {                                                                                                      \
-      if constexpr (is_kind<K3>::value) FN<K3, BLOCK_N, CG>(*ps.p[3], u - ps.base[3], STATE, sh, titer);          \
+      if constexpr (is_kind<K3>::value)                                                                           \
+        FN<K3, BLOCK_N, CG>(*ps.p[3], Work{u - ps.base[3], w.kb_begin, w.kb_count}, STATE, sh, titer);            \
     }                                                                                                             \
   } while (0)
 
@@ -992,13 +1037,14 @@
   ptx::pdl_wait();
   if (threadIdx.x == 0) trace_hdr(p.trace, 3, clock64());
 
-  UnitIter it(ps.sched, group_id, num_groups, ps.base[1]);
+  UnitIter it(ps.sched, p, group_id, num_groups);
 
   if (warp == 0) {
     if (lane == 0) {
       ProdState st{0u, 0u, ptx::mbar_try_wait(&sh.empty_bar[0], 1)};
-      int titer = 0, u;
-      while (it.next(u)) {
+      int titer = 0;
+      Work w;
+      while (it.next(w)) {
         RVAE_DISPATCH(produce_unit, st);
         ++titer;
       }
@@ -1007,8 +1053,9 @@
   } else if (warp == 1) {
     if (lane == 0 && sh.leader) {
       MmaState st{0u, 0u, 0u, 0u, false};
-      int titer = 0, u;
-      while (it.next(u)) {
+      int titer = 0;
+      Work w;
+      while (it.next(w)) {
         RVAE_DISPATCH(mma_unit, st);
         ++titer;
       }
@@ -1026,10 +1073,11 @@
                  es.team_tid == 0};
     es.as = 0; es.aphase = 0; es.loss_local = 0.f;
     float loss[kMaxChain] = {0.f, 0.f, 0.f, 0.f};
-    int titer = 0, u;
-    while (it.next(u)) {
+    int titer = 0;
+    Work w;
+    while (it.next(w)) {
       RVAE_DISPATCH(epilogue_unit, es);
-      const int q = (u >= ps.base[1]) + (u >= ps.base[2]) + (u >= ps.base[3]);
+      const int q = (w.u >= ps.base[1]) + (w.u >= ps.base[2]) + (w.u >= ps.base[3]);
 #pragma unroll
       for (int i = 0; i < kMaxChain; ++i)
         if (i == q) loss[i] += es.loss_local;
@@ -1065,10 +1113,10 @@
 
 __device__ __forceinline__ ProblemSet single_problem(const GemmParams& p) {
   ProblemSet ps;
-  const int total = p.m_blocks * p.n_blocks * p.k_splits;
+  const int tiles = p.m_blocks * p.n_blocks;
   ps.p[0] = ps.p[1] = ps.p[2] = ps.p[3] = &p;
   ps.base[0] = 0;
-  ps.base[1] = ps.base[2] = ps.base[3] = ps.base[4] = total;
+  ps.base[1] = ps.base[2] = ps.base[3] = ps.base[4] = tiles;
   ps.sched = nullptr;
   return ps;
 }
diff --git a/rawaudiovae_kelsey_b200/csrc/gemm_host.cu b/rawaudiovae_kelsey_b200/csrc/gemm_host.cu
--- a/rawaudiovae_kelsey_b200/csrc/gemm_host.cu
+++ b/rawaudiovae_kelsey_b200/csrc/gemm_host.cu
@@ -198,11 +198,8 @@
   int splits = 1;
   if (d.epi == EPI_REDUCE) {
     const int tiles = p.m_blocks * p.n_blocks;
-    static const int env_splits = getenv("RVAE_WGRAD_SPLITS") ? atoi(getenv("RVAE_WGRAD_SPLITS")) : 0;
     if (d.k_splits > 0) {
       splits = d.k_splits;
-    } else if (env_splits > 0 && d.A.major == MAJOR_MN) {
-      splits = env_splits;
     } else {
       double best = 0.0;
       for (int s = 1; s <= 8 && p.kb_total / s >= 8; ++s) {
@@ -273,6 +270,13 @@
   g.grid = cg * (units < slots_eff ? units : slots_eff);
   g.smem_bytes = kVariants[g.variant].smem;
   return RVAE_OK;
+}
+
+void gemm_limit_grid(PreparedGemm* g, int ctas) {
+  if (g->grid <= ctas) return;
+  g->grid = ctas;
+  GemmParams& p = g->params;
+  if (g->epi == EPI_REDUCE && p.epi.accumulate && p.m_blocks * p.n_blocks * p.k_splits > ctas / g->cg) p.k_splits = 0;
 }
 
 int gemm_run(Ctx* ctx, const PreparedGemm& g, cudaStream_t stream) {
@@ -341,19 +345,21 @@
   return rc;
 }
 
-static double unit_cost(const PreparedGemm& g) {
-  const double mma = (double)g.params.kb_per_split * g.params.num_passes;
+constexpr double kHandover = 2.0;
+static double unit_cost(const PreparedGemm& g, int kb) {
+  const double mma = (double)kb * g.params.num_passes;
   const double epi = (g.epi == EPI_DRELU || g.epi == EPI_OUT) ? 11.0 : 8.0;
-  if (g.epi == EPI_DLATENT) return mma + 22.0 + 2.0;
-  return (mma > epi ? mma : epi) + 2.0;
-}
-
-int gemm_prepare_chain(const Ctx* ctx, const PreparedGemm* const* g, int count, int pairs, int* sched_dev,
+  if (g.epi == EPI_DLATENT) return mma + 22.0 + kHandover;
+  return (mma > epi ? mma : epi) + kHandover;
+}
+
+int gemm_prepare_chain(const Ctx* ctx, const PreparedGemm* const* g, int count, int pairs, SchedEntry* sched_dev,
                        PreparedChain* out, unsigned int* dep_flags) {
   RVAE_REQUIRE(count >= 2 && count <= kMaxChain, RVAE_ERR_INVALID, "chain gemm: %d problems", count);
+  auto by_k = [&](int i) { return g[i]->epi == EPI_REDUCE && g[i]->params.epi.accumulate != 0; };
   for (int i = 0; i < count; ++i)
-    RVAE_REQUIRE(g[i]->block_n == 256 && g[i]->cg == 2, RVAE_ERR_UNSUPPORTED,
-                 "chain gemm: every problem must use 256-wide pair tiles");
+    RVAE_REQUIRE(g[i]->block_n == 256 && g[i]->cg == 2 && (by_k(i) || g[i]->params.k_splits == 1), RVAE_ERR_UNSUPPORTED,
+                 "chain gemm: every problem must use 256-wide pair tiles and whole-K units or a reduce-add epilogue");
   RVAE_REQUIRE(sched_dev != nullptr && pairs >= 1 && 2 * pairs <= ctx->num_sms_total, RVAE_ERR_INVALID,
                "chain gemm: bad schedule buffer / pair count %d", pairs);
   RVAE_CHECK(configure_chain_variants());
@@ -367,20 +373,27 @@
     if (match) variant = v;
   }
   RVAE_REQUIRE(variant >= 0, RVAE_ERR_UNSUPPORTED, "chain gemm: no fused kernel for this combination of problems");
-  int nunits[kMaxChain], base[kMaxChain + 1];
+  int ntiles[kMaxChain], base[kMaxChain + 1];
   base[0] = 0;
   for (int i = 0; i < kMaxChain; ++i) {
-    nunits[i] = i < count ? g[i]->params.m_blocks * g[i]->params.n_blocks * g[i]->params.k_splits : 0;
-    base[i + 1] = base[i] + nunits[i];
-  }
-  RVAE_REQUIRE(base[kMaxChain] <= pairs * kSchedMax, RVAE_ERR_UNSUPPORTED, "chain gemm: %d units exceed the schedule",
-               base[kMaxChain]);
-  struct U { int id; double cost; };
+    ntiles[i] = i < count ? g[i]->params.m_blocks * g[i]->params.n_blocks : 0;
+    base[i + 1] = base[i] + ntiles[i];
+  }
+  std::vector<double> load(pairs, 0.0);
+  std::vector<int> cnt(pairs, 0);
+  std::vector<SchedEntry> sched((size_t)pairs * kSchedMax, SchedEntry{-1, 0, 0, 0});
+  auto place = [&](int pidx, int id, int kb0, int kb, double cost) -> int {
+    RVAE_REQUIRE(cnt[pidx] < kSchedMax, RVAE_ERR_UNSUPPORTED, "chain gemm: more than %d units for a pair", kSchedMax);
+    sched[(size_t)pidx * kSchedMax + cnt[pidx]++] = SchedEntry{id, kb0, kb, 0};
+    load[pidx] += cost;
+    return RVAE_OK;
+  };
+  struct U { int id, prob; double cost; };
   std::vector<U> units;
-  units.reserve(base[kMaxChain]);
   if (dep_flags == nullptr) {
     for (int i = 0; i < count; ++i)
-      for (int u = 0; u < nunits[i]; ++u) units.push_back({base[i] + u, unit_cost(*g[i])});
+      if (!by_k(i))
+        for (int u = 0; u < ntiles[i]; ++u) units.push_back({base[i] + u, i, unit_cost(*g[i], g[i]->params.kb_total)});
     std::stable_sort(units.begin(), units.end(), [](const U& a, const U& b) { return a.cost > b.cost; });
   } else {
     for (int i = 0; i < count; ++i) {
@@ -389,38 +402,66 @@
                        mb <= 256,
                    RVAE_ERR_UNSUPPORTED, "chain gemm: chained problems must share the row blocking");
       for (int m = 0; m < mb; ++m)
-        for (int n = 0; n < nb; ++n) units.push_back({base[i] + n * mb + m, unit_cost(*g[i])});
-    }
-  }
-  std::vector<double> load(pairs, 0.0);
-  std::vector<int> cnt(pairs, 0);
-  std::vector<int> sched((size_t)pairs * kSchedMax, -1);
+        for (int n = 0; n < nb; ++n) units.push_back({base[i] + n * mb + m, i, unit_cost(*g[i], g[i]->params.kb_total)});
+    }
+  }
   for (const U& u : units) {
     int best = -1;
     for (int pidx = 0; pidx < pairs; ++pidx)
       if (cnt[pidx] < kSchedMax && (best < 0 || load[pidx] < load[best] - 1e-9)) best = pidx;
     RVAE_REQUIRE(best >= 0, RVAE_ERR_UNSUPPORTED, "chain gemm: schedule overflow");
-    sched[(size_t)best * kSchedMax + cnt[best]++] = u.id;
-    load[best] += u.cost;
+    RVAE_CHECK(place(best, u.id, 0, g[u.prob]->params.kb_total, u.cost));
+  }
+  long long off[kMaxChain + 1];
+  off[0] = 0;
+  double work = 0.0;
+  for (int i = 0; i < kMaxChain; ++i) {
+    const bool sk = i < count && by_k(i);
+    off[i + 1] = off[i] + (sk ? (long long)ntiles[i] * g[i]->params.kb_total : 0);
+    if (sk) work += (double)(off[i + 1] - off[i]) * g[i]->params.num_passes;
+  }
+  const long long T = off[kMaxChain];
+  if (T > 0) {
+    auto fill_at = [&](double level, int pidx) { return std::max(0.0, level - load[pidx] - kHandover); };
+    double lo = *std::min_element(load.begin(), load.end()), hi = *std::max_element(load.begin(), load.end()) + work + kHandover;
+    for (int it = 0; it < 100; ++it) {
+      const double mid = 0.5 * (lo + hi);
+      double f = 0.0;
+      for (int pidx = 0; pidx < pairs; ++pidx) f += fill_at(mid, pidx);
+      (f < work ? lo : hi) = mid;
+    }
+    double total = 0.0;
+    for (int pidx = 0; pidx < pairs; ++pidx) total += fill_at(hi, pidx);
+    auto prob_at = [&](long long b) { int i = 0; while (i + 1 < kMaxChain && b >= off[i + 1]) ++i; return i; };
+    double cum = 0.0;
+    long long begin = 0;
+    for (int pidx = 0; pidx < pairs; ++pidx) {
+      cum += fill_at(hi, pidx);
+      const long long end = pidx + 1 == pairs ? T : std::min(T, std::llround((double)T * cum / total));
+      for (long long cur = begin; cur < end;) {
+        const int i = prob_at(cur);
+        const int kbt = g[i]->params.kb_total;
+        const long long local = cur - off[i];
+        const int tile = (int)(local / kbt), kb0 = (int)(local % kbt);
+        const int kb = (int)std::min<long long>(end - cur, kbt - kb0);
+        RVAE_CHECK(place(pidx, base[i] + tile, kb0, kb, unit_cost(*g[i], kb)));
+        cur += kb;
+      }
+      begin = end > begin ? end : begin;
+    }
   }
   if (dep_flags == nullptr) {
     static const int order_mode = getenv("RVAE_CHAIN_ORDER") ? atoi(getenv("RVAE_CHAIN_ORDER")) : 1;
     auto prob_of = [&](int id) { int q = 0; while (q + 1 < count && id >= base[q + 1]) ++q; return q; };
+    auto mma_of = [&](const SchedEntry& e) { return (double)e.z * g[prob_of(e.x)]->params.num_passes; };
     for (int pidx = 0; pidx < pairs && order_mode == 1; ++pidx) {
-      int* row = &sched[(size_t)pidx * kSchedMax];
-      std::vector<int> heavy, light;
+      SchedEntry* row = &sched[(size_t)pidx * kSchedMax];
+      std::vector<SchedEntry> heavy, light;
       double min_mma = 1e30;
-      for (int k = 0; k < cnt[pidx]; ++k) {
-        const PreparedGemm& gq = *g[prob_of(row[k])];
-        min_mma = std::min(min_mma, (double)gq.params.kb_per_split * gq.params.num_passes);
-      }
-      for (int k = 0; k < cnt[pidx]; ++k) {
-        const PreparedGemm& gq = *g[prob_of(row[k])];
-        const double mma = (double)gq.params.kb_per_split * gq.params.num_passes;
-        (mma > 1.5 * min_mma ? heavy : light).push_back(row[k]);
-      }
+      for (int k = 0; k < cnt[pidx]; ++k) min_mma = std::min(min_mma, mma_of(row[k]));
+      for (int k = 0; k < cnt[pidx]; ++k) (mma_of(row[k]) > 1.5 * min_mma ? heavy : light).push_back(row[k]);
       if (heavy.empty() || light.size() < 2) continue;
-      std::vector<int> merged;
+      std::vector<SchedEntry> merged;
       const size_t nh = heavy.size(), nl = light.size();
       size_t li = 0;
       for (size_t h = 0; h < nh; ++h) {
@@ -435,7 +476,7 @@
       for (size_t k = 0; k < merged.size(); ++k) row[k] = merged[k];
     }
   }
-  RVAE_CUDA(cudaMemcpy(sched_dev, sched.data(), sched.size() * sizeof(int), cudaMemcpyHostToDevice));
+  RVAE_CUDA(cudaMemcpy(sched_dev, sched.data(), sched.size() * sizeof(SchedEntry), cudaMemcpyHostToDevice));
   PreparedChain& d = *out;
   memset(&d, 0, sizeof(d));
   for (int i = 0; i < kMaxChain; ++i) d.params.p[i] = g[i < count ? i : 0]->params;
```

Result: slower. 25.27 million (median of 6 runs) (-2.5%).
